# yzGuu830/efficient-speech-codec

Measured on AMD Instinct MI355X. Metric: audio-seconds/sec encode+decode, ESC-Base 9kbps 3s@16kHz, higher is better.
Workload: dtype f32 (fp32 storage and accumulation everywhere; the K = C contractions of the MLPs, of the attention's Q / K / V projections, of PatchMerge / PatchSplit and of the de-embedding run on the fp16 matrix cores with every fp32 operand split into two fp16 terms under power-of-two scales (range-safe by cons

## Files before the change

efficient-speech-codec_amd/csrc/escx_api.cpp:

```cpp
#include <hip/hip_runtime.h>

#include <algorithm>
#include <cmath>
#include <cstdlib>
#include <cstring>
#include <map>
#include <mutex>
#include <tuple>
#include <utility>
#include <vector>

#include "escx_internal.h"
#include "launchers.h"

using namespace escx;

static void part_layout(escx_handle_s* h, int B, int T, int* k, int* per, int* pass) {
    *k = std::min(n_parts(h, B), h->n_sets);
    *pass = std::max(1, std::min(pass_clips(h, B, T), h->sets[0].shp.B));
    *per = *k <= 1 ? B : (B + *k - 1) / *k;
}

template <class F>
static int run_halves(escx_handle_s* h, int B, int T, hipStream_t st, F part) {
// ... 311 lines not shown
        L.sub_x3 = nullptr; L.sub_x3s = nullptr;
        if (!want || !grab(&L.sub_x3_buf, rowgemm_x3_bytes(KP, Np))) continue;
        if (rowgemm_x3_pack(L.sub_wf, L.sub_x3_buf, KP, Np, st, nt, L.sub_g, L.sub_b, (L.scale == 1 ? 2 : 1) * L.C) == 0) L.sub_x3 = L.sub_x3_buf;
        if (L.scale == 2 && (L.Cp == 80 || L.Cp == 96 || L.Cp == 144) && L.Cp <= x3_max && grab(&L.sub_x3s_buf, mlp_x3_split_bytes(L.Cp, Np)) &&
            mlp_x3_split_pack(L.sub_wf, L.sub_x3s_buf, L.Cp, Np, st, nt, L.sub_g, L.sub_b, L.C) == 0) L.sub_x3s = L.sub_x3s_buf;
    }
    h->pvq_tab_stale = false;
    return launch_ok("derived images");
}

extern "C" int escx_set_precision(escx_handle h, int mode) {
    if (!h) ESCX_FAIL(ESCX_ERR_INVALID_ARG, "null handle");
    if (mode != ESCX_PRECISION_FP32 && mode != ESCX_PRECISION_BF16X3 && mode != ESCX_PRECISION_F16X2)
        ESCX_FAIL(ESCX_ERR_INVALID_ARG, "precision mode %d (0 = fp32 MFMA, 3 = three bf16 terms, 2 = two fp16 terms)", mode);
    if (mode != h->prec) { h->prec = mode; h->pvq_tab_stale = true; }
    return ESCX_OK;
}
extern "C" int escx_get_precision(escx_handle h) { return h ? h->prec : ESCX_ERR_INVALID_ARG; }

static float pvq_loss_scale(const escx_handle_s* h, const Quant& q, int Tq) {
    if (h->len) return 1.0f / ((float)q.d * h->cfg.group_size);
    return 1.0f / ((float)Tq * q.d * h->cfg.group_size);
}

static int run_pvq_encode(escx_handle_s* h, const Quant& q, const float* enc, const float* dec, int B, int W, long long* codes,
                          long long bstride, float* loss, hipStream_t st) {
    const escx_config& c = h->cfg;
    const int Tq = W / c.overlap, M = B * Tq;
    const int splits = pvq_down_splits(M, q.Kq, q.Cp);
    if ((size_t)splits * M * q.Nz > h->zpart_cap) ESCX_FAIL(ESCX_ERR_STATE, "split-K scratch too small");
    const double vec = (double)c.overlap * q.Hq * q.C;
    PROF("pvq_down_gemm", 2.0 * M * vec * q.d, (double)M * vec * (dec ? 2 : 1) * 4,
         gemm_pvq_down(enc, dec, B, q.Hq, W, q.Cp, c.overlap, q.wd, q.Nz, q.Kq, h->zpart, splits, st));
    int src_rc = 0;
    PROF("pvq_search", 2.0 * M * c.group_size * c.codebook_size * q.d, ((double)c.group_size * c.codebook_size * q.d + (double)M * c.group_size * q.d) * 4,
         src_rc = pvq_search(h->zpart, splits, M, q.Nz, q.cbn, q.c2, q.cbraw, c.group_size, c.codebook_size, q.d, q.dt, Tq, codes, bstride,
                             loss, pvq_loss_scale(h, q, Tq), c.l2norm, st));
    if (src_rc) ESCX_FAIL(ESCX_ERR_UNSUPPORTED, "codebook_dim %d unsupported by the search kernel", q.d);
    return launch_ok("pvq_encode");
}

static int run_pvq_decode(escx_handle_s* h, const Quant& q, const long long* codes, long long bstride, const float* dec, int B, int W,
                          float* out, hipStream_t st) {
    const escx_config& c = h->cfg;
    const double vec = (double)c.overlap * q.Hq * q.C, Mv = (double)B * (W / c.overlap);
    const bool special = h->pvq_up_kernel;
    if (q.tab && special) {
        PROF("pvq_tab_add", 0, Mv * vec * (dec ? 3 : 2) * 4,
             pvq_tab_add(codes, bstride, q.tab, q.gq, c.group_size, c.codebook_size, B, q.Hq, W, q.Cp, c.overlap, dec, out, st));
        return launch_ok("pvq_decode");
    }
    int urc = -1;
    if (special)
        PROF("pvq_up_gemm", 2.0 * Mv * vec * q.d, Mv * vec * (dec ? 2 : 1) * 4,
             urc = pvq_up(codes, bstride, q.cbraw, c.group_size, c.codebook_size, q.dt, B, q.Hq, W, q.Cp, c.overlap, q.wup, q.Kq, q.Kup, dec, out, st));
    if (urc != 0) {
        if (special && h->prof && !h->prof_recs.empty()) h->prof_recs.pop_back();
    PROF("pvq_up_gemm", 2.0 * Mv * vec * q.d, Mv * vec * (dec ? 2 : 1) * 4,
         gemm_pvq_up(codes, bstride, q.cbraw, c.group_size, c.codebook_size, q.dt, B, q.Hq, W, q.Cp, c.overlap, q.wup, q.Kq, q.Kup, dec, out, st));
    }
    return launch_ok("pvq_decode");
}

static int run_pvq_quantize(escx_handle_s* h, const Quant& q, const float* enc, const float* dec, int B, int W, long long* codes, long long bstride,
                            float* loss, float* out, hipStream_t st) {
    const escx_config& c = h->cfg;
    if (h->pvq_fused) {
        const int Tq = W / c.overlap, M = B * Tq;
        const double vec = (double)c.overlap * q.Hq * q.C;
        int frc = -1;
        PROF(out ? "pvq_fused" : "pvq_fused_codes", 2.0 * M * vec * q.d * (out ? 2 : 1) + 2.0 * M * c.group_size * c.codebook_size * q.d,
             (double)M * vec * ((dec ? 2 : 1) + (out ? (dec ? 2 : 1) : 0)) * 4,
             frc = pvq_fused(enc, dec, B, q.Hq, W, q.Cp, c.overlap, q.wdf, q.Nz, q.Kq, pvq_down_splits(M, q.Kq, q.Cp), pvq_down_bk(q.Cp), q.cbn, q.c2, q.cbraw,
                             c.group_size, c.codebook_size, q.d, q.dt, q.wup, q.tab, q.gq, out, codes, bstride, loss, pvq_loss_scale(h, q, Tq), c.l2norm, st));
        if (frc == 0) return launch_ok("pvq_quantize");
        if (h->prof && !h->prof_recs.empty()) h->prof_recs.pop_back();
    }
    int rc;
    if ((rc = run_pvq_encode(h, q, enc, dec, B, W, codes, bstride, loss, st))) return rc;
    if (out && (rc = run_pvq_decode(h, q, codes, bstride, dec, B, W, out, st))) return rc;
    return 0;
}

static int run_deembed(escx_handle_s* h, const float* tok, int B, int W, float* rspec, hipStream_t st) {
    const escx_config& c = h->cfg;
    const int H0 = c.in_freq / c.patch_f;
    if (h->len) {
        if (h->deembed_two_stage || c.in_dim * h->Q > 16) ESCX_FAIL(ESCX_ERR_UNSUPPORTED, "mixed-length batches run the composed de-embedding only (in_dim * patch area <= 16, ESCX_DEEMBED_TWO_STAGE unset)");
        const double tk = (double)B * H0 * W;
        PROF("deembed_zero_dead", 0, tk * h->C0p * 4, zero_dead_cols(const_cast<float*>(tok), h->len->d_W, B, H0, W, h->C0p, st));
        int hrc = -1;
        if (h->deembed_halo)
            PROF("deembed_composed7x7", 2.0 * tk * 49 * h->C0 * c.in_dim * h->Q, (tk * h->C0 + tk * c.in_dim * h->Q) * 4,
                 hrc = deembed7_fused(tok, B, H0, W, h->C0p, h->dch_w, h->dcc_b, rspec, c.patch_f, c.patch_t, c.in_dim, h->Fp, st, h->dch_x2));
        if (hrc != 0)
        PROF("deembed_composed7x7", 2.0 * tk * 49 * h->C0 * c.in_dim * h->Q, (tk * h->C0 + tk * c.in_dim * h->Q) * 4,
             gemm_deembed_composed(tok, B, H0, W, h->C0p, h->dcc_w, rspec, h->dcc_b, c.patch_f, c.patch_t, c.in_dim, h->Fp, st));
        int brc = 0;
        PROF("deembed_border_len", 0, 0,
             brc = deembed_border_len(tok, h->dcv_w, h->dcv_b, rspec, h->len->d_W, B, H0, W, h->C0, h->C0p, c.patch_f, c.patch_t, c.in_dim, h->Fp, st));
        if (brc != 0) ESCX_FAIL(ESCX_ERR_UNSUPPORTED, "mixed-length batches: no border kernel for %d de-embedding outputs", c.in_dim * h->Q);
        return launch_ok("patch_deembed");
    }
    if (!h->deembed_two_stage && c.in_dim * h->Q <= 16) {
        const double tk = (double)B * H0 * W;
        int hrc = -1;
        if (h->deembed_halo)
            PROF("deembed_composed7x7", 2.0 * tk * 49 * h->C0 * c.in_dim * h->Q, (tk * h->C0 + tk * c.in_dim * h->Q) * 4,
                 hrc = deembed7_fused(tok, B, H0, W, h->C0p, h->dch_w, h->dcc_b, rspec, c.patch_f, c.patch_t, c.in_dim, h->Fp, st, h->dch_x2));
        if (hrc != 0)
        PROF("deembed_composed7x7", 2.0 * tk * 49 * h->C0 * c.in_dim * h->Q, (tk * h->C0 + tk * c.in_dim * h->Q) * 4,
             gemm_deembed_composed(tok, B, H0, W, h->C0p, h->dcc_w, rspec, h->dcc_b, c.patch_f, c.patch_t, c.in_dim, h->Fp, st));
        int brc = 0;
        PROF("deembed_border", 0, 0,
             brc = deembed_border(tok, h->dcv_w, h->dcv_b, rspec, B, H0, W, h->C0, h->C0p, c.patch_f, c.patch_t, c.in_dim, h->Fp, st));
        if (brc == 0) return launch_ok("patch_deembed");
    }
    const double toks = (double)B * H0 * W, pix = toks * h->Q;
    PROF("deembed_conv5x5", 2.0 * toks * 25 * h->C0 * h->C0 * h->Q, (toks * h->C0 + pix * h->C0) * 4,
         gemm_conv_deembed1(tok, B, H0, W, h->C0p, h->dc1_w, h->Q * h->C0p, h->deemb, h->dc1_b, c.patch_f, c.patch_t, st));
    PROF("deembed_conv3x3", 2.0 * pix * 9 * h->C0 * c.in_dim, (pix * h->C0 + pix * c.in_dim) * 4,
         gemm_conv_spec(h->deemb, B, c.patch_t * W, c.patch_f * H0, h->C0p, h->dc2_w, rspec, h->dc2_b, h->Fp, c.in_dim, st));
    return launch_ok("patch_deembed");
}

static int run_istft(escx_handle_s* h, const float* rspec, int B, int T2, float* wave, hipStream_t st) {
    const escx_config& c = h->cfg;
    PROF("istft_idft_gemm", 2.0 * B * T2 * c.win_length * 2 * h->F, (double)B * T2 * (2 * h->F + c.win_length) * 4,
         gemm_store(rspec, c.in_dim * h->Fp, B * T2, h->idft_w, h->winP, c.in_dim * h->Fp, h->frames, h->winP, nullptr, st));
    if (h->len) {
        PROF("istft_overlap_add_len", 0, (double)B * T2 * c.win_length * 4 + (double)B * c.hop_length * (T2 - 1) * 4,
             istft_ola_len(h->frames, h->win2, wave, h->len->d_W, c.patch_t, B, T2, h->winP, c.win_length, c.hop_length, h->left, h->n_fft / 2, c.hop_length * (T2 - 1), st));
        return launch_ok("istft");
    }
    PROF("istft_overlap_add", 0, (double)B * T2 * c.win_length * 4 + (double)B * c.hop_length * (T2 - 1) * 4,
         istft_ola(h->frames, h->win2, wave, B, T2, h->winP, c.win_length, c.hop_length, h->left, h->n_fft / 2, c.hop_length * (T2 - 1), st));
    return launch_ok("istft");
}

static void spec_unpad(escx_handle_s* h, const float* src, float* dst, long long rows, hipStream_t st) {
    unpad_rows(src, dst, rows * h->cfg.in_dim, h->F, h->Fp, st);
}
static void spec_pad(escx_handle_s* h, const float* src, float* dst, long long rows, hipStream_t st) {
    pad_rows(src, dst, rows * h->cfg.in_dim, h->F, h->Fp, st);
}

extern "C" int escx_num_frames(escx_handle h, int n_samples) { return h ? 1 + n_samples / h->cfg.hop_length : 0; }
extern "C" int escx_output_samples(escx_handle h, int feat_w) { return h ? h->cfg.hop_length * (h->cfg.patch_t * feat_w - 1) : 0; }

static int rvq_encode(escx_handle_s* h, const float* wave, int B, int L, const int32_t* streams, int S, int64_t* codes, int* fh, int* fw, void* stream);
static int rvq_decode(escx_handle_s* h, const int64_t* codes, int B, int S, const int32_t* streams, int fh, int fw, float* wave_out, float* recon_feat, void* stream);
static int rvq_forward(escx_handle_s* h, const float* wave, const float* feat, int B, int LT, const int32_t* streams, int S, int64_t* codes, float* wave_out,
                       float* raw_feat, float* recon_feat, float* cm_loss, void* stream);

static int run_csvq_encode(escx_handle_s* h, const Shapes& s, int S, long long* codes, hipStream_t st) {
    const escx_config& c = h->cfg;
    const int n = h->n, G = c.group_size;
    const long long bstride = (long long)S * G * s.Tq, sstride = (long long)G * s.Tq;
    int rc, H = s.encH[n - 1], Hn;
    float* dec = h->decA; float* other = h->decB;
    if ((rc = run_pvq_quantize(h, h->quants[0], h->enc_hs[n - 1], nullptr, s.B, s.W, codes, bstride, nullptr, S == 1 ? nullptr : dec, st))) return rc;
    if (S == 1) return 0;
    for (int i = 0; i < S - 1; ++i) {
        const Quant& q = h->quants[i + 1];
        const bool last = (i + 2 == S);
        if ((rc = run_pvq_quantize(h, q, h->enc_hs[n - 1 - i], dec, s.B, s.W, codes + (i + 1) * sstride, bstride, nullptr, last ? nullptr : dec, st))) return rc;
        if (last) break;
        if ((rc = run_layer(h, h->layers[n + i], dec, other, s.B, H, s.W, &Hn, st))) return rc;
        std::swap(dec, other); H = Hn;
    }
    return 0;
}

extern "C" int escx_encode(escx_handle h, const float* wave, int B, int L, int S, int64_t* codes, int* fh, int* fw, void* stream) {
    if (h && h->kind == 1) return rvq_encode(h, wave, B, L, nullptr, S, codes, fh, fw, stream);
    int rc = check_ready(h); if (rc) return rc;
    if (!wave || !codes) ESCX_FAIL(ESCX_ERR_INVALID_ARG, "null pointer");
    if (S < 1 || S > h->cfg.max_streams) ESCX_FAIL(ESCX_ERR_INVALID_ARG, "num_streams=%d outside [1, %d]", S, h->cfg.max_streams);
    if (L <= h->n_fft / 2) ESCX_FAIL(ESCX_ERR_INVALID_ARG, "n_samples=%d too short for reflect padding of %d", L, h->n_fft / 2);
    Shapes s; if ((rc = ensure_ws(h, B, frames_of(h, L), &s))) return rc;
    const long long cstride = (long long)S * h->cfg.group_size * s.Tq;
    if ((rc = ensure_pvq_tables(h, (hipStream_t)stream))) return rc;
    rc = run_halves(h, B, s.T, (hipStream_t)stream, [&](int b0, int nb, hipStream_t st) -> int {
        Shapes sp = s; sp.B = nb; int r;
        if ((r = run_stft(h, wave + (size_t)b0 * L, nb, L, sp.T, h->spec, st))) return r;
        if ((r = run_encoder(h, sp, st))) return r;
        return run_csvq_encode(h, sp, S, (long long*)codes + b0 * cstride, st);
    });
    if (rc) return rc;
    if (fh) *fh = s.encH[h->n - 1];
    if (fw) *fw = s.W;
    return ESCX_OK;
}

static int run_csvq_decode(escx_handle_s* h, const long long* codes, int B, int S, int Hb, int W, float* rspec, hipStream_t st) {
    const escx_config& c = h->cfg;
    const int n = h->n, G = c.group_size, Tq = W / c.overlap;
    const long long bstride = (long long)S * G * Tq, sstride = (long long)G * Tq;
    int rc, H = Hb, Hn;
    float* dec = h->decA; float* other = h->decB;
    if ((rc = run_pvq_decode(h, h->quants[0], codes, bstride, nullptr, B, W, dec, st))) return rc;
    for (int i = 0; i + 1 < n; ++i) {
        if (i < S - 1 && (rc = run_pvq_decode(h, h->quants[i + 1], codes + (i + 1) * sstride, bstride, dec, B, W, dec, st))) return rc;
        if ((rc = run_layer(h, h->layers[n + i], dec, other, B, H, W, &Hn, st))) return rc;
        std::swap(dec, other); H = Hn;
    }
    if ((rc = run_layer(h, h->layers[2 * n - 1], dec, other, B, H, W, &Hn, st))) return rc;
    return run_deembed(h, other, B, W, rspec, st);
}

extern "C" int escx_decode(escx_handle h, const int64_t* codes, int B, int S, int fh, int fw, float* wave_out, float* recon_feat,
                           void* stream) {
    if (h && h->kind == 1) return rvq_decode(h, codes, B, S, nullptr, fh, fw, wave_out, recon_feat, stream);
    int rc = check_infer_ready(h); if (rc) return rc;
    if (!codes || !wave_out) ESCX_FAIL(ESCX_ERR_INVALID_ARG, "null pointer");
    const escx_config& c = h->cfg;
    if (S < 1 || S > c.max_streams) ESCX_FAIL(ESCX_ERR_INVALID_ARG, "codes.size(1)=%d outside [1, %d]", S, c.max_streams);
    if (fw < 1 || fw % c.overlap) ESCX_FAIL(ESCX_ERR_ASSERT, "Time dimension must be multiple of overlap");
    Shapes s; if ((rc = ensure_ws(h, B, frames_for_width(h, fw), &s))) return rc;
    if (s.W != fw || s.encH[h->n - 1] != fh) ESCX_FAIL(ESCX_ERR_INVALID_ARG, "feat_shape (%d,%d) does not match the model (%d,%d)", fh, fw, s.encH[h->n - 1], s.W);
    const int T2 = c.patch_t * fw, out_len = c.hop_length * (T2 - 1);
    const long long cstride = (long long)S * c.group_size * (fw / c.overlap);
    if ((rc = ensure_pvq_tables(h, (hipStream_t)stream))) return rc;
    rc = run_halves(h, B, s.T, (hipStream_t)stream, [&](int b0, int nb, hipStream_t st) -> int {
        int r;
        if ((r = run_csvq_decode(h, (const long long*)codes + b0 * cstride, nb, S, fh, fw, h->rspec, st))) return r;
        if ((r = run_istft(h, h->rspec, nb, T2, wave_out + (size_t)b0 * out_len, st))) return r;
        if (recon_feat) spec_unpad(h, h->rspec, recon_feat + (size_t)b0 * T2 * c.in_dim * h->F, (long long)nb * T2, st);
        return launch_ok("decode");
    });
    return rc;
}

static int forward_impl(escx_handle h, const float* wave, const float* feat, int B, int L, int T, int S, int64_t* codes, float* wave_out,
                        float* raw_feat, float* recon_feat, float* cm_loss, void* stream) {
    if (h && h->kind == 1) return rvq_forward(h, wave, feat, B, wave ? L : T, nullptr, S, codes, wave_out, raw_feat, recon_feat, cm_loss, stream);
    int rc = check_infer_ready(h); if (rc) return rc;
    if ((!wave && !feat) || !codes || !wave_out) ESCX_FAIL(ESCX_ERR_INVALID_ARG, "null pointer");
    const escx_config& c = h->cfg;
    if (S < 1 || S > c.max_streams) ESCX_FAIL(ESCX_ERR_INVALID_ARG, "num_streams=%d outside [1, %d]", S, c.max_streams);
    if (wave && L <= h->n_fft / 2) ESCX_FAIL(ESCX_ERR_INVALID_ARG, "n_samples=%d too short for reflect padding of %d", L, h->n_fft / 2);
    if (!wave && T < c.patch_t) ESCX_FAIL(ESCX_ERR_INVALID_ARG, "n_frames=%d shorter than one patch", T);
    if (wave) T = frames_of(h, L);
    Shapes s; if ((rc = ensure_ws(h, B, T, &s))) return rc;
    if (s.W % c.overlap) ESCX_FAIL(ESCX_ERR_ASSERT, "Time dimension must be multiple of overlap");
    const int n = h->n, G = c.group_size;
    const long long bstride = (long long)S * G * s.Tq, sstride = (long long)G * s.Tq;
    const int T2 = c.patch_t * s.W, out_len = c.hop_length * (T2 - 1);
    if ((rc = ensure_pvq_tables(h, (hipStream_t)stream))) return rc;
    return run_halves(h, B, s.T, (hipStream_t)stream, [&](int b0, int nb, hipStream_t st) -> int {
        Shapes sp = s; sp.B = nb; int r;
        long long* cd = (long long*)codes + b0 * bstride;
        if (wave) { if ((r = run_stft(h, wave + (size_t)b0 * L, nb, L, sp.T, h->spec, st))) return r; }
        else spec_pad(h, feat + (size_t)b0 * sp.T * c.in_dim * h->F, h->spec, (long long)nb * sp.T, st);
        if (raw_feat) spec_unpad(h, h->spec, raw_feat + (size_t)b0 * sp.T * c.in_dim * h->F, (long long)nb * sp.T, st);
        if ((r = run_encoder(h, sp, st))) return r;
        const size_t lslot = (size_t)G * nb * sp.Tq;
        float* loss = cm_loss ? h->loss_terms : nullptr;
        int n_slots = 1;
        int H = sp.encH[n - 1], Hn;
        float* dec = h->decA; float* other = h->decB;
        if ((r = run_pvq_quantize(h, h->quants[0], h->enc_hs[n - 1], nullptr, nb, sp.W, cd, bstride, loss, dec, st))) return r;
        for (int i = 0; i + 1 < n; ++i) {
            if (i < S - 1) {
                const Quant& q = h->quants[i + 1];
                if ((r = run_pvq_quantize(h, q, h->enc_hs[n - 1 - i], dec, nb, sp.W, cd + (i + 1) * sstride, bstride, loss ? loss + (size_t)(i + 1) * lslot : nullptr, dec, st))) return r;
                n_slots = i + 2;
            }
            if ((r = run_layer(h, h->layers[n + i], dec, other, nb, H, sp.W, &Hn, st))) return r;
            std::swap(dec, other); H = Hn;
        }
        if ((r = run_layer(h, h->layers[2 * n - 1], dec, other, nb, H, sp.W, &Hn, st))) return r;
        if ((r = run_deembed(h, other, nb, sp.W, h->rspec, st))) return r;
        if ((r = run_istft(h, h->rspec, nb, T2, wave_out + (size_t)b0 * out_len, st))) return r;
        if (recon_feat) spec_unpad(h, h->rspec, recon_feat + (size_t)b0 * T2 * c.in_dim * h->F, (long long)nb * T2, st);
        if (cm_loss) loss_reduce(loss, n_slots, G, nb * sp.Tq, sp.Tq, cm_loss + b0, st);
        return launch_ok("forward");
    });
}

extern "C" int escx_forward(escx_handle h, const float* wave, int B, int L, int S, int64_t* codes, float* wave_out, float* raw_feat,
                            float* recon_feat, float* cm_loss, void* stream) {
    if (!wave) ESCX_FAIL(ESCX_ERR_INVALID_ARG, "null pointer");
    return forward_impl(h, wave, nullptr, B, L, 0, S, codes, wave_out, raw_feat, recon_feat, cm_loss, stream);
}

extern "C" int escx_forward_feat(escx_handle h, const float* feat, int B, int T, int S, int64_t* codes, float* wave_out, float* recon_feat,
                                 float* cm_loss, void* stream) {
    if (!feat) ESCX_FAIL(ESCX_ERR_INVALID_ARG, "null pointer");
    return forward_impl(h, nullptr, feat, B, 0, T, S, codes, wave_out, nullptr, recon_feat, cm_loss, stream);
}

namespace {
struct MixPlan {
    int B = 0, Smax = 0;
    std::vector<int32_t> ints;
    const int32_t* S_ws() const { return ints.data() + 2 * B; }
};
}

static int check_streams(escx_handle_s* h, int B, const int32_t* streams, int* Smax) {
    if (!streams) ESCX_FAIL(ESCX_ERR_INVALID_ARG, "null streams pointer");
    if (B < 1) ESCX_FAIL(ESCX_ERR_INVALID_ARG, "batch=%d: the per-clip stream counts need at least one clip", B);
    int m = 0;
    for (int b = 0; b < B; ++b) {
        if (streams[b] < 1 || streams[b] > h->cfg.max_streams)
            ESCX_FAIL(ESCX_ERR_INVALID_ARG, "streams[%d]=%d outside [1, %d]", b, streams[b], h->cfg.max_streams);
        m = std::max(m, (int)streams[b]);
    }
    *Smax = m;
    return 0;
}

static void plan_streams(escx_handle_s* h, int B, int T, const int32_t* streams, int Smax, MixPlan* p) {
    int k, per, pass;
    part_layout(h, B, T, &k, &per, &pass);
    std::vector<std::pair<int, int>> groups;
    for (int off = 0; off < per; off += pass)
        for (int i = 0; i < std::max(k, 1); ++i) {
            const int b0 = i * per, nb = std::min(per, B - b0);
            if (nb <= off) continue;
            groups.push_back({b0 + off, std::min(pass, nb - off)});
        }
    std::vector<int> order(B);
    for (int b = 0; b < B; ++b) order[b] = b;
    std::stable_sort(order.begin(), order.end(), [&](int a, int b) { return streams[a] > streams[b]; });
    p->B = B; p->Smax = Smax;
    p->ints.assign((size_t)4 * B, 0);
    int32_t *ws2b = p->ints.data(), *b2ws = ws2b + B, *Sws = ws2b + 2 * B, *Sb = ws2b + 3 * B;
    int next = 0;
    for (int r = 0; next < B; ++r)
        for (const auto& g : groups)
            if (r < g.second && next < B) ws2b[g.first + r] = order[next++];
    for (int w = 0; w < B; ++w) { b2ws[ws2b[w]] = w; Sws[w] = streams[ws2b[w]]; }
    for (int b = 0; b < B; ++b) Sb[b] = streams[b];
}

namespace {
struct MixBufs {
    size_t used = 0;
    std::vector<std::pair<void**, size_t>> want;
    template <class T> void add(T** p, size_t n) { want.push_back({reinterpret_cast<void**>(p), n * sizeof(T)}); }
};
}
static int mix_alloc(escx_handle_s* h, MixBufs& m) {
    size_t total = 0;
    for (auto& w : m.want) total += (w.second + 255) / 256 * 256;
    if (total > h->mix_cap) {
        ESCX_HIP(hipDeviceSynchronize());
        if (h->mix_buf) { (void)hipFree(h->mix_buf); h->mix_buf = nullptr; h->mix_cap = 0; }
        ESCX_HIP(hipMalloc(&h->mix_buf, total));
        h->mix_cap = total;
    }
    char* base = static_cast<char*>(h->mix_buf);
    for (auto& w : m.want) { *w.first = w.second ? base : nullptr; base += (w.second + 255) / 256 * 256; }
    return 0;
}

static int upload_plan(escx_handle_s* h, const MixPlan& p, int32_t* dev, hipStream_t st) {
    ESCX_HIP(hipMemcpyAsync(dev, p.ints.data(), p.ints.size() * sizeof(int32_t), hipMemcpyHostToDevice, st));
    return 0;
}

static int clips_over(const int* S, int B, int j) { int c = 0; while (c < B && S[c] > j) ++c; return c; }

static int run_csvq_encode_streams(escx_handle_s* h, const Shapes& s, const int* S, long long* codes, long long bstride, hipStream_t st) {
    const int n = h->n;
    const long long sstride = (long long)h->cfg.group_size * s.Tq;
    int rc, H = s.encH[n - 1], Hn;
    float* dec = h->decA; float* other = h->decB;
    int nref = clips_over(S, s.B, 1);
    if ((rc = run_pvq_quantize(h, h->quants[0], h->enc_hs[n - 1], nullptr, s.B, s.W, codes, bstride, nullptr, nref ? dec : nullptr, st))) return rc;
    for (int i = 0; nref > 0; ++i) {
        const int nq = nref;
        nref = clips_over(S, nq, i + 2);
        if ((rc = run_pvq_quantize(h, h->quants[i + 1], h->enc_hs[n - 1 - i], dec, nq, s.W, codes + (i + 1) * sstride, bstride, nullptr, nref ? dec : nullptr, st))) return rc;
        if (!nref) break;
        if ((rc = run_layer(h, h->layers[n + i], dec, other, nref, H, s.W, &Hn, st))) return rc;
        std::swap(dec, other); H = Hn;
    }
    return 0;
}

static int run_csvq_decode_streams(escx_handle_s* h, const long long* codes, long long bstride, int B, const int* S, int Hb, int W, float* rspec, hipStream_t st) {
    const int n = h->n;
    const long long sstride = (long long)h->cfg.group_size * (W / h->cfg.overlap);
    int rc, H = Hb, Hn;
    float* dec = h->decA; float* other = h->decB;
    if ((rc = run_pvq_decode(h, h->quants[0], codes, bstride, nullptr, B, W, dec, st))) return rc;
    for (int i = 0; i + 1 < n; ++i) {
        const int nq = clips_over(S, B, i + 1);
        if (nq && (rc = run_pvq_decode(h, h->quants[i + 1], codes + (i + 1) * sstride, bstride, dec, nq, W, dec, st))) return rc;
        if ((rc = run_layer(h, h->layers[n + i], dec, other, B, H, W, &Hn, st))) return rc;
        std::swap(dec, other); H = Hn;
    }
    if ((rc = run_layer(h, h->layers[2 * n - 1], dec, other, B, H, W, &Hn, st))) return rc;
    return run_deembed(h, other, B, W, rspec, st);
}

extern "C" int escx_encode_streams(escx_handle h, const float* wave, int B, int L, const int32_t* streams, int64_t* codes, int* fh, int* fw,
                                   void* stream) {
    if (h && h->kind == 1) return rvq_encode(h, wave, B, L, streams, 0, codes, fh, fw, stream);
    int rc = check_ready(h); if (rc) return rc;
    if (!wave || !codes) ESCX_FAIL(ESCX_ERR_INVALID_ARG, "null pointer");
    int Smax = 0; if ((rc = check_streams(h, B, streams, &Smax))) return rc;
    if (L <= h->n_fft / 2) ESCX_FAIL(ESCX_ERR_INVALID_ARG, "n_samples=%d too short for reflect padding of %d", L, h->n_fft / 2);
    Shapes s; if ((rc = ensure_ws(h, B, frames_of(h, L), &s))) return rc;
    MixPlan p; plan_streams(h, B, s.T, streams, Smax, &p);
    const int GT = h->cfg.group_size * s.Tq;
    const long long cstride = (long long)Smax * GT;
    int32_t* maps; float* wave_ws; long long* codes_ws;
    MixBufs mb; mb.add(&maps, p.ints.size()); mb.add(&wave_ws, (size_t)B * L); mb.add(&codes_ws, (size_t)B * cstride);
    if ((rc = mix_alloc(h, mb))) return rc;
    hipStream_t st = (hipStream_t)stream;
    if ((rc = ensure_pvq_tables(h, st))) return rc;
    if ((rc = upload_plan(h, p, maps, st))) return rc;
    PROF("mix_gather", 0, 2.0 * B * L * 4, rows_permute(wave, wave_ws, maps, B, L, st));
    rc = run_halves(h, B, s.T, st, [&](int b0, int nb, hipStream_t sti) -> int {
        Shapes sp = s; sp.B = nb; int r;
        if ((r = run_stft(h, wave_ws + (size_t)b0 * L, nb, L, sp.T, h->spec, sti))) return r;
        if ((r = run_encoder(h, sp, sti))) return r;
        return run_csvq_encode_streams(h, sp, p.S_ws() + b0, codes_ws + b0 * cstride, cstride, sti);
    });
    if (rc) return rc;
    PROF("mix_scatter", 0, 2.0 * B * cstride * 8, codes_permute(codes_ws, cstride, (long long*)codes, maps + B, maps + 3 * B, B, Smax, GT, st));
    if ((rc = launch_ok("encode_streams"))) return rc;
    if (fh) *fh = s.encH[h->n - 1];
    if (fw) *fw = s.W;
    return ESCX_OK;
}

extern "C" int escx_decode_streams(escx_handle h, const int64_t* codes, int B, int Smax_in, const int32_t* streams, int fh, int fw, float* wave_out,
                                   float* recon_feat, void* stream) {
    if (h && h->kind == 1) return rvq_decode(h, codes, B, Smax_in, streams, fh, fw, wave_out, recon_feat, stream);
    int rc = check_infer_ready(h); if (rc) return rc;
    if (!codes || !wave_out) ESCX_FAIL(ESCX_ERR_INVALID_ARG, "null pointer");
    const escx_config& c = h->cfg;
    int Smax = 0; if ((rc = check_streams(h, B, streams, &Smax))) return rc;
    if (Smax_in < Smax || Smax_in > c.max_streams) ESCX_FAIL(ESCX_ERR_INVALID_ARG, "codes.size(1)=%d: must lie in [max(streams)=%d, %d]", Smax_in, Smax, c.max_streams);
    if (fw < 1 || fw % c.overlap) ESCX_FAIL(ESCX_ERR_ASSERT, "Time dimension must be multiple of overlap");
    Shapes s; if ((rc = ensure_ws(h, B, frames_for_width(h, fw), &s))) return rc;
    if (s.W != fw || s.encH[h->n - 1] != fh) ESCX_FAIL(ESCX_ERR_INVALID_ARG, "feat_shape (%d,%d) does not match the model (%d,%d)", fh, fw, s.encH[h->n - 1], s.W);
    MixPlan p; plan_streams(h, B, s.T, streams, Smax, &p);
    const int T2 = c.patch_t * fw, out_len = c.hop_length * (T2 - 1), GT = c.group_size * (fw / c.overlap);
    const long long in_stride = (long long)Smax_in * GT, cstride = (long long)Smax * GT, frow = (long long)T2 * c.in_dim * h->F;
    int32_t* maps; long long* codes_ws; float *wave_ws, *recon_ws = nullptr;
    MixBufs mb; mb.add(&maps, p.ints.size()); mb.add(&codes_ws, (size_t)B * cstride); mb.add(&wave_ws, (size_t)B * out_len);
    if (recon_feat) mb.add(&recon_ws, (size_t)B * frow);
    if ((rc = mix_alloc(h, mb))) return rc;
    hipStream_t st = (hipStream_t)stream;
    if ((rc = ensure_pvq_tables(h, st))) return rc;
    if ((rc = upload_plan(h, p, maps, st))) return rc;
    PROF("mix_gather", 0, 2.0 * B * cstride * 8, codes_permute((const long long*)codes, in_stride, codes_ws, maps, maps + 2 * B, B, Smax, GT, st));
    rc = run_halves(h, B, s.T, st, [&](int b0, int nb, hipStream_t sti) -> int {
        int r;
        if ((r = run_csvq_decode_streams(h, codes_ws + b0 * cstride, cstride, nb, p.S_ws() + b0, fh, fw, h->rspec, sti))) return r;
        if ((r = run_istft(h, h->rspec, nb, T2, wave_ws + (size_t)b0 * out_len, sti))) return r;
        if (recon_ws) spec_unpad(h, h->rspec, recon_ws + (size_t)b0 * frow, (long long)nb * T2, sti);
        return launch_ok("decode_streams");
    });
    if (rc) return rc;
    PROF("mix_scatter", 0, 2.0 * B * out_len * 4, rows_permute(wave_ws, wave_out, maps + B, B, out_len, st));
    if (recon_feat) PROF("mix_scatter", 0, 2.0 * B * frow * 4, rows_permute(recon_ws, recon_feat, maps + B, B, frow, st));
    return launch_ok("decode_streams");
}

extern "C" int escx_forward_streams(escx_handle h, const float* wave, const float* feat, int B, int LT, const int32_t* streams, int64_t* codes,
                                    float* wave_out, float* raw_feat, float* recon_feat, float* cm_loss, void* stream) {
    if (h && h->kind == 1) return rvq_forward(h, wave, feat, B, LT, streams, 0, codes, wave_out, raw_feat, recon_feat, cm_loss, stream);
    int rc = check_infer_ready(h); if (rc) return rc;
    if ((!wave == !feat) || !codes || !wave_out) ESCX_FAIL(ESCX_ERR_INVALID_ARG, "null pointer (exactly one of wave / feat, codes and wave_out are required)");
    const escx_config& c = h->cfg;
    int Smax = 0; if ((rc = check_streams(h, B, streams, &Smax))) return rc;
    const int L = wave ? LT : 0;
    int T = wave ? 0 : LT;
    if (wave && L <= h->n_fft / 2) ESCX_FAIL(ESCX_ERR_INVALID_ARG, "n_samples=%d too short for reflect padding of %d", L, h->n_fft / 2);
    if (!wave && T < c.patch_t) ESCX_FAIL(ESCX_ERR_INVALID_ARG, "n_frames=%d shorter than one patch", T);
    if (wave) T = frames_of(h, L);
    Shapes s; if ((rc = ensure_ws(h, B, T, &s))) return rc;
    if (s.W % c.overlap) ESCX_FAIL(ESCX_ERR_ASSERT, "Time dimension must be multiple of overlap");
    MixPlan p; plan_streams(h, B, s.T, streams, Smax, &p);
    const int n = h->n, G = c.group_size, GT = G * s.Tq;
    const long long cstride = (long long)Smax * GT, sstride = GT;
    const int T2 = c.patch_t * s.W, out_len = c.hop_length * (T2 - 1);
    const long long in_row = wave ? (long long)L : (long long)s.T * c.in_dim * h->F, raw_row = (long long)s.T * c.in_dim * h->F, rec_row = (long long)T2 * c.in_dim * h->F;
    int32_t* maps; float *in_ws, *wave_ws, *raw_ws = nullptr, *recon_ws = nullptr, *loss_ws = nullptr; long long* codes_ws;
    MixBufs mb; mb.add(&maps, p.ints.size()); mb.add(&in_ws, (size_t)B * in_row); mb.add(&codes_ws, (size_t)B * cstride); mb.add(&wave_ws, (size_t)B * out_len);
    if (raw_feat) mb.add(&raw_ws, (size_t)B * raw_row);
    if (recon_feat) mb.add(&recon_ws, (size_t)B * rec_row);
    if (cm_loss) mb.add(&loss_ws, (size_t)B);
    if ((rc = mix_alloc(h, mb))) return rc;
    hipStream_t st = (hipStream_t)stream;
    if ((rc = ensure_pvq_tables(h, st))) return rc;
    if ((rc = upload_plan(h, p, maps, st))) return rc;
    PROF("mix_gather", 0, 2.0 * B * in_row * 4, rows_permute(wave ? wave : feat, in_ws, maps, B, in_row, st));
    const int32_t* Sdev = maps + 2 * B;
    rc = run_halves(h, B, s.T, st, [&](int b0, int nb, hipStream_t st) -> int {
        Shapes sp = s; sp.B = nb; int r;
        const int* S = p.S_ws() + b0;
        long long* cd = codes_ws + b0 * cstride;
        if (wave) { if ((r = run_stft(h, in_ws + (size_t)b0 * L, nb, L, sp.T, h->spec, st))) return r; }
        else spec_pad(h, in_ws + (size_t)b0 * in_row, h->spec, (long long)nb * sp.T, st);
        if (raw_ws) spec_unpad(h, h->spec, raw_ws + (size_t)b0 * raw_row, (long long)nb * sp.T, st);
        if ((r = run_encoder(h, sp, st))) return r;
        const size_t lslot = (size_t)G * nb * sp.Tq;
        float* loss = cm_loss ? h->loss_terms : nullptr;
        int slot_clips[8] = {nb};
        int H = sp.encH[n - 1], Hn;
        float* dec = h->decA; float* other = h->decB;
        if ((r = run_pvq_quantize(h, h->quants[0], h->enc_hs[n - 1], nullptr, nb, sp.W, cd, cstride, loss, dec, st))) return r;
        for (int i = 0; i + 1 < n; ++i) {
            const int nq = clips_over(S, nb, i + 1);
            if (nq) {
                if ((r = run_pvq_quantize(h, h->quants[i + 1], h->enc_hs[n - 1 - i], dec, nq, sp.W, cd + (i + 1) * sstride, cstride, loss ? loss + (size_t)(i + 1) * lslot : nullptr, dec, st))) return r;
                slot_clips[i + 1] = nq;
            }
            if ((r = run_layer(h, h->layers[n + i], dec, other, nb, H, sp.W, &Hn, st))) return r;
            std::swap(dec, other); H = Hn;
        }
        if ((r = run_layer(h, h->layers[2 * n - 1], dec, other, nb, H, sp.W, &Hn, st))) return r;
        if ((r = run_deembed(h, other, nb, sp.W, h->rspec, st))) return r;
        if ((r = run_istft(h, h->rspec, nb, T2, wave_ws + (size_t)b0 * out_len, st))) return r;
        if (recon_ws) spec_unpad(h, h->rspec, recon_ws + (size_t)b0 * rec_row, (long long)nb * T2, st);
        if (cm_loss) PROF("loss_reduce_streams", 0, (double)nb * Smax * GT * 4, loss_reduce_streams(loss, (long long)lslot, Sdev + b0, n, slot_clips, G, sp.Tq, nb, loss_ws + b0, st));
        return launch_ok("forward_streams");
    });
    if (rc) return rc;
    PROF("mix_scatter", 0, 2.0 * B * cstride * 8, codes_permute(codes_ws, cstride, (long long*)codes, maps + B, maps + 3 * B, B, Smax, GT, st));
    PROF("mix_scatter", 0, 2.0 * B * out_len * 4, rows_permute(wave_ws, wave_out, maps + B, B, out_len, st));
    if (raw_feat) PROF("mix_scatter", 0, 2.0 * B * raw_row * 4, rows_permute(raw_ws, raw_feat, maps + B, B, raw_row, st));
    if (recon_feat) PROF("mix_scatter", 0, 2.0 * B * rec_row * 4, rows_permute(recon_ws, recon_feat, maps + B, B, rec_row, st));
    if (cm_loss) PROF("mix_scatter", 0, 8.0 * B, rows_permute(loss_ws, cm_loss, maps + B, B, 1, st));
    return launch_ok("forward_streams");
}

namespace {
struct LenGuard {
    escx_handle_s* h;
    LenGuard(escx_handle_s* h_, const LenCtx* c) : h(h_) { h->len = c; }
    ~LenGuard() { h->len = nullptr; }
};
}

static int len_common_checks(escx_handle_s* h, int B, const int32_t* v, const char* what) {
    if (h->kind == 1) ESCX_FAIL(ESCX_ERR_UNSUPPORTED, "mixed-length batches are not implemented for the rvq+swinT codec (RVQCodecs)");
    if (h->ws != 4) ESCX_FAIL(ESCX_ERR_UNSUPPORTED, "mixed-length batches are implemented for window_size 4 only (this model: %d)", h->ws);
    if (!v) ESCX_FAIL(ESCX_ERR_INVALID_ARG, "null %s pointer", what);
    if (B < 1) ESCX_FAIL(ESCX_ERR_INVALID_ARG, "batch=%d: the per-clip %s need at least one clip", B, what);
    return 0;
}

static int plan_lengths(escx_handle_s* h, int B, int Lx, const int32_t* lengths, LenCtx* lc, int* Lmax) {
    const escx_config& c = h->cfg;
    lc->B = B; lc->W.assign(B, 0); lc->Wmax = 0; *Lmax = 0;
    for (int b = 0; b < B; ++b) {
        const int L = lengths[b];
        if (L <= h->n_fft / 2 || L > Lx) ESCX_FAIL(ESCX_ERR_INVALID_ARG, "lengths[%d]=%d outside (%d, %d] (reflect padding of %d, row length %d)", b, L, h->n_fft / 2, Lx, h->n_fft / 2, Lx);
        const int W = frames_of(h, L) / c.patch_t;
        if (W < 1 || W % c.overlap) ESCX_FAIL(ESCX_ERR_ASSERT, "Time dimension must be multiple of overlap (clip %d: %d samples give %d latent frames)", b, L, W);
        lc->W[b] = W; lc->Wmax = std::max(lc->Wmax, W); *Lmax = std::max(*Lmax, L);
    }
    return 0;
}

static int upload_lengths(escx_handle_s* h, MixBufs& mb, LenCtx* lc, const int32_t* lengths, hipStream_t st) {
    int32_t* tab = nullptr;
    mb.add(&tab, (size_t)2 * lc->B);
    int rc = mix_alloc(h, mb); if (rc) return rc;
    ESCX_HIP(hipMemcpyAsync(tab, lc->W.data(), (size_t)lc->B * sizeof(int32_t), hipMemcpyHostToDevice, st));
    lc->d_W = tab;
    if (lengths) { ESCX_HIP(hipMemcpyAsync(tab + lc->B, lengths, (size_t)lc->B * sizeof(int32_t), hipMemcpyHostToDevice, st)); lc->d_L = tab + lc->B; }
    return 0;
}

extern "C" int escx_encode_lengths(escx_handle h, const float* wave, int B, int Lx, const int32_t* lengths, int S, int64_t* codes, int* fh, int* fw, void* stream) {
    int rc = check_ready(h); if (rc) return rc;
    if ((rc = len_common_checks(h, B, lengths, "lengths"))) return rc;
    if (!wave || !codes) ESCX_FAIL(ESCX_ERR_INVALID_ARG, "null pointer");
    const escx_config& c = h->cfg;
    if (S < 1 || S > c.max_streams) ESCX_FAIL(ESCX_ERR_INVALID_ARG, "num_streams=%d outside [1, %d]", S, c.max_streams);
    LenCtx lc; int Lmax = 0;
    if ((rc = plan_lengths(h, B, Lx, lengths, &lc, &Lmax))) return rc;
    Shapes s; if ((rc = ensure_ws(h, B, frames_of(h, Lmax), &s, B))) return rc;
    if (h->sets[0].shp.B < B || h->sets[0].shp.T < s.T) ESCX_FAIL(ESCX_ERR_STATE, "workspace set holds %d clips of %d frames, the batch needs %d of %d", h->sets[0].shp.B, h->sets[0].shp.T, B, s.T);
    hipStream_t st = (hipStream_t)stream;
    MixBufs mb; if ((rc = upload_lengths(h, mb, &lc, lengths, st))) return rc;
    if ((rc = ensure_pvq_tables(h, st))) return rc;
    use_set(h, 0);
    LenGuard guard(h, &lc);
    if ((rc = run_stft(h, wave, B, Lx, s.T, h->spec, st))) return rc;
    if ((rc = run_encoder(h, s, st))) return rc;
    if ((rc = run_csvq_encode(h, s, S, (long long*)codes, st))) return rc;
    PROF("codes_mask_len", 0, 8.0 * B * S * c.group_size * s.Tq, codes_mask_len((const long long*)codes, (long long*)codes, lc.d_W, c.overlap, B, S * c.group_size, s.Tq, -1, st));
    if ((rc = launch_ok("encode_lengths"))) return rc;
    if (fh) *fh = s.encH[h->n - 1];
    if (fw) *fw = s.W;
    return ESCX_OK;
}

static int plan_widths(escx_handle_s* h, int B, int fw, const int32_t* widths, LenCtx* lc) {
    lc->B = B; lc->W.assign(widths, widths + B); lc->Wmax = fw;
    for (int b = 0; b < B; ++b) {
        if (widths[b] < 1 || widths[b] > fw) ESCX_FAIL(ESCX_ERR_INVALID_ARG, "frame_lengths[%d]=%d outside [1, %d]", b, widths[b], fw);
        if (widths[b] % h->cfg.overlap) ESCX_FAIL(ESCX_ERR_ASSERT, "Time dimension must be multiple of overlap (clip %d: %d latent frames)", b, widths[b]);
    }
    return 0;
}

extern "C" int escx_decode_lengths(escx_handle h, const int64_t* codes, int B, int S, const int32_t* widths, int fh, int fw, float* wave_out, float* recon_feat,
                                   void* stream) {
    int rc = check_infer_ready(h); if (rc) return rc;
    if ((rc = len_common_checks(h, B, widths, "frame_lengths"))) return rc;
    if (!codes || !wave_out) ESCX_FAIL(ESCX_ERR_INVALID_ARG, "null pointer");
    const escx_config& c = h->cfg;
    if (S < 1 || S > c.max_streams) ESCX_FAIL(ESCX_ERR_INVALID_ARG, "codes.size(1)=%d outside [1, %d]", S, c.max_streams);
    if (fw < 1 || fw % c.overlap) ESCX_FAIL(ESCX_ERR_ASSERT, "Time dimension must be multiple of overlap");
    LenCtx lc;
    if ((rc = plan_widths(h, B, fw, widths, &lc))) return rc;
    Shapes s; if ((rc = ensure_ws(h, B, frames_for_width(h, fw), &s, B))) return rc;
    if (h->sets[0].shp.B < B || h->sets[0].shp.T < s.T) ESCX_FAIL(ESCX_ERR_STATE, "workspace set holds %d clips of %d frames, the batch needs %d of %d", h->sets[0].shp.B, h->sets[0].shp.T, B, s.T);
    if (s.W != fw || s.encH[h->n - 1] != fh) ESCX_FAIL(ESCX_ERR_INVALID_ARG, "feat_shape (%d,%d) does not match the model (%d,%d)", fh, fw, s.encH[h->n - 1], s.W);
    const int T2 = c.patch_t * fw, Tq = fw / c.overlap;
    hipStream_t st = (hipStream_t)stream;
    long long* codes_ws = nullptr;
    MixBufs mb; mb.add(&codes_ws, (size_t)B * S * c.group_size * Tq);
    if ((rc = upload_lengths(h, mb, &lc, nullptr, st))) return rc;
    if ((rc = ensure_pvq_tables(h, st))) return rc;
    use_set(h, 0);
    LenGuard guard(h, &lc);
    PROF("codes_mask_len", 0, 16.0 * B * S * c.group_size * Tq, codes_mask_len((const long long*)codes, codes_ws, lc.d_W, c.overlap, B, S * c.group_size, Tq, 0, st));
    if ((rc = run_csvq_decode(h, codes_ws, B, S, fh, fw, h->rspec, st))) return rc;
    if ((rc = run_istft(h, h->rspec, B, T2, wave_out, st))) return rc;
    if (recon_feat) PROF("unpad_len", 0, 2.0 * B * T2 * c.in_dim * h->F * 4, unpad_rows_len(h->rspec, recon_feat, lc.d_W, 1, c.patch_t, c.hop_length, B, T2, c.in_dim, h->F, h->Fp, st));
    return launch_ok("decode_lengths");
}

extern "C" int escx_forward_lengths(escx_handle h, const float* wave, int B, int Lx, const int32_t* lengths, int S, int64_t* codes, float* wave_out,
                                    float* raw_feat, float* recon_feat, float* cm_loss, void* stream) {
    int rc = check_infer_ready(h); if (rc) return rc;
    if ((rc = len_common_checks(h, B, lengths, "lengths"))) return rc;
    if (!wave || !codes || !wave_out) ESCX_FAIL(ESCX_ERR_INVALID_ARG, "null pointer");
    const escx_config& c = h->cfg;
    if (S < 1 || S > c.max_streams) ESCX_FAIL(ESCX_ERR_INVALID_ARG, "num_streams=%d outside [1, %d]", S, c.max_streams);
    LenCtx lc; int Lmax = 0;
    if ((rc = plan_lengths(h, B, Lx, lengths, &lc, &Lmax))) return rc;
    Shapes s; if ((rc = ensure_ws(h, B, frames_of(h, Lmax), &s, B))) return rc;
    if (h->sets[0].shp.B < B || h->sets[0].shp.T < s.T) ESCX_FAIL(ESCX_ERR_STATE, "workspace set holds %d clips of %d frames, the batch needs %d of %d", h->sets[0].shp.B, h->sets[0].shp.T, B, s.T);
    hipStream_t st = (hipStream_t)stream;
    MixBufs mb; if ((rc = upload_lengths(h, mb, &lc, lengths, st))) return rc;
    if ((rc = ensure_pvq_tables(h, st))) return rc;
    use_set(h, 0);
    LenGuard guard(h, &lc);
    const int n = h->n, G = c.group_size;
    const long long bstride = (long long)S * G * s.Tq, sstride = (long long)G * s.Tq;
    const int T2 = c.patch_t * s.W;
    long long* cd = (long long*)codes;
    if ((rc = run_stft(h, wave, B, Lx, s.T, h->spec, st))) return rc;
    if (raw_feat) PROF("unpad_len", 0, 2.0 * B * s.T * c.in_dim * h->F * 4, unpad_rows_len(h->spec, raw_feat, lc.d_L, 0, c.patch_t, c.hop_length, B, s.T, c.in_dim, h->F, h->Fp, st));
    if ((rc = run_encoder(h, s, st))) return rc;
    const size_t lslot = (size_t)G * B * s.Tq;
    float* loss = cm_loss ? h->loss_terms : nullptr;
    int n_slots = 1;
    int H = s.encH[n - 1], Hn;
    float* dec = h->decA; float* other = h->decB;
    if ((rc = run_pvq_quantize(h, h->quants[0], h->enc_hs[n - 1], nullptr, B, s.W, cd, bstride, loss, dec, st))) return rc;
    for (int i = 0; i + 1 < n; ++i) {
        if (i < S - 1) {
            if ((rc = run_pvq_quantize(h, h->quants[i + 1], h->enc_hs[n - 1 - i], dec, B, s.W, cd + (i + 1) * sstride, bstride, loss ? loss + (size_t)(i + 1) * lslot : nullptr, dec, st))) return rc;
            n_slots = i + 2;
        }
        if ((rc = run_layer(h, h->layers[n + i], dec, other, B, H, s.W, &Hn, st))) return rc;
        std::swap(dec, other); H = Hn;
    }
    if ((rc = run_layer(h, h->layers[2 * n - 1], dec, other, B, H, s.W, &Hn, st))) return rc;
    if ((rc = run_deembed(h, other, B, s.W, h->rspec, st))) return rc;
    if ((rc = run_istft(h, h->rspec, B, T2, wave_out, st))) return rc;
    if (recon_feat) PROF("unpad_len", 0, 2.0 * B * T2 * c.in_dim * h->F * 4, unpad_rows_len(h->rspec, recon_feat, lc.d_W, 1, c.patch_t, c.hop_length, B, T2, c.in_dim, h->F, h->Fp, st));
    if (cm_loss) PROF("loss_reduce_len", 0, (double)n_slots * lslot * 4, loss_reduce_len(loss, lc.d_W, c.overlap, n_slots, G, B, s.Tq, cm_loss, st));
    PROF("codes_mask_len", 0, 8.0 * B * bstride, codes_mask_len(cd, cd, lc.d_W, c.overlap, B, S * G, s.Tq, -1, st));
    return launch_ok("forward_lengths");
}

static int run_prvq(escx_handle_s* h, const float* enc, const long long* codes_in, int B, int W, long long* codes, long long bstride, const int* clip_S,
                    int S, float* loss, long long lslot, float* out, hipStream_t st) {
    const escx_config& c = h->cfg;
    const Quant& q = h->quants[0];
    const int Tq = W / c.overlap, M = B * Tq;
    const double vec = (double)c.overlap * q.Hq * q.C, G = c.group_size;
    int rc = -1;
    PROF(codes_in ? "prvq_decode" : (out ? "prvq_fused" : "prvq_fused_codes"),
         codes_in ? 2.0 * M * vec * q.d : 2.0 * M * vec * q.d * (out ? 2 : 1) + 2.0 * M * S * G * c.codebook_size * q.d,
         (double)M * vec * ((codes_in ? 0 : 1) + (out ? 1 : 0)) * 4,
         rc = prvq_fused(enc, codes_in, B, q.Hq, W, q.Cp, c.overlap, q.wdf, q.Nz, q.Kq, pvq_down_splits(M, q.Kq, q.Cp), pvq_down_bk(q.Cp), q.cbn, q.c2, q.cbraw,
                         c.group_size, c.codebook_size, q.d, q.dt, q.wup, codes, bstride, clip_S, S, S, loss, lslot, 1.0f / ((float)Tq * q.d * c.group_size),
                         c.l2norm, out, st));
    if (rc) ESCX_FAIL(ESCX_ERR_UNSUPPORTED, "rvq quantiser: geometry not covered (codebook_dim %d, %d groups)", q.d, c.group_size);
    return launch_ok("prvq");
}

static int run_plain_decoder(escx_handle_s* h, int B, int Hb, int W, float* rspec, hipStream_t st) {
    const int n = h->n;
    int rc, H = Hb, Hn;
    float* dec = h->decA; float* other = h->decB;
    for (int i = 0; i + 1 < n; ++i) {
        if ((rc = run_layer(h, h->layers[n + i], dec, other, B, H, W, &Hn, st))) return rc;
        std::swap(dec, other); H = Hn;
    }
    if ((rc = run_layer(h, h->layers[2 * n - 1], dec, other, B, H, W, &Hn, st))) return rc;
    return run_deembed(h, other, B, W, rspec, st);
}

static int rvq_counts(escx_handle_s* h, int B, const int32_t* streams, int S, int* Smax) {
    if (!streams) {
        if (S < 1 || S > h->num_rvqs) ESCX_FAIL(ESCX_ERR_INVALID_ARG, "num_streams=%d outside [1, %d] (num_rvqs)", S, h->num_rvqs);
        *Smax = S;
        return 0;
    }
    if (B < 1) ESCX_FAIL(ESCX_ERR_INVALID_ARG, "batch=%d: the per-clip stream counts need at least one clip", B);
    int m = 0;
    for (int b = 0; b < B; ++b) {
        if (streams[b] < 1 || streams[b] > h->num_rvqs) ESCX_FAIL(ESCX_ERR_INVALID_ARG, "streams[%d]=%d outside [1, %d] (num_rvqs)", b, streams[b], h->num_rvqs);
        m = std::max(m, (int)streams[b]);
    }
    *Smax = m;
    return 0;
}

static int rvq_upload(escx_handle_s* h, int B, const int32_t* streams, const int** dev, hipStream_t st) {
    *dev = nullptr;
    if (!streams) return 0;
    int32_t* d = nullptr;
    MixBufs mb; mb.add(&d, (size_t)B);
    int rc = mix_alloc(h, mb); if (rc) return rc;
    ESCX_HIP(hipMemcpyAsync(d, streams, (size_t)B * sizeof(int32_t), hipMemcpyHostToDevice, st));
    *dev = d;
    return 0;
}

static int rvq_encode(escx_handle_s* h, const float* wave, int B, int L, const int32_t* streams, int S, int64_t* codes, int* fh, int* fw, void* stream) {
    int rc = check_ready(h); if (rc) return rc;
    if (!wave || !codes) ESCX_FAIL(ESCX_ERR_INVALID_ARG, "null pointer");
    int Smax = 0; if ((rc = rvq_counts(h, B, streams, S, &Smax))) return rc;
    if (L <= h->n_fft / 2) ESCX_FAIL(ESCX_ERR_INVALID_ARG, "n_samples=%d too short for reflect padding of %d", L, h->n_fft / 2);
    Shapes s; if ((rc = ensure_ws(h, B, frames_of(h, L), &s))) return rc;
    hipStream_t st = (hipStream_t)stream;
    const int* Sdev; if ((rc = rvq_upload(h, B, streams, &Sdev, st))) return rc;
    if ((rc = ensure_pvq_tables(h, st))) return rc;
    const long long cstride = (long long)Smax * h->cfg.group_size * s.Tq;
    rc = run_halves(h, B, s.T, st, [&](int b0, int nb, hipStream_t sti) -> int {
        Shapes sp = s; sp.B = nb; int r;
        if ((r = run_stft(h, wave + (size_t)b0 * L, nb, L, sp.T, h->spec, sti))) return r;
// ... 66 lines not shown
    });
}

extern "C" int escx_spec_transform(escx_handle h, const float* wave, int B, int L, float* spec, void* stream) {
    int rc = check_ready(h); if (rc) return rc;
    if (!wave || !spec || B < 1) ESCX_FAIL(ESCX_ERR_INVALID_ARG, "bad argument");
    if (L <= h->n_fft / 2) ESCX_FAIL(ESCX_ERR_INVALID_ARG, "n_samples=%d too short for reflect padding of %d", L, h->n_fft / 2);
    const int T = frames_of(h, L);
    TmpBuf t; if (t.alloc((size_t)B * T * h->cfg.in_dim * h->Fp)) ESCX_FAIL(ESCX_ERR_HIP, "hipMalloc failed");
    hipStream_t st = (hipStream_t)stream;
    if ((rc = run_stft(h, wave, B, L, T, t.p, st))) return rc;
    spec_unpad(h, t.p, spec, (long long)B * T, st);
    return launch_ok("spec_transform");
}

extern "C" int escx_audio_reconstruct(escx_handle h, const float* spec, int B, int T, float* wave, void* stream) {
    int rc = check_ready(h); if (rc) return rc;
    if (!spec || !wave || B < 1 || T < 2) ESCX_FAIL(ESCX_ERR_INVALID_ARG, "bad argument (need at least 2 frames)");
    TmpBuf ts, tf;
    if (ts.alloc((size_t)B * T * h->cfg.in_dim * h->Fp) || tf.alloc((size_t)B * T * h->winP)) ESCX_FAIL(ESCX_ERR_HIP, "hipMalloc failed");
    hipStream_t st = (hipStream_t)stream;
    const escx_config& c = h->cfg;
    spec_pad(h, spec, ts.p, (long long)B * T, st);
    gemm_store(ts.p, c.in_dim * h->Fp, B * T, h->idft_w, h->winP, c.in_dim * h->Fp, tf.p, h->winP, nullptr, st);
    istft_ola(tf.p, h->win2, wave, B, T, h->winP, c.win_length, c.hop_length, h->left, h->n_fft / 2, c.hop_length * (T - 1), st);
    return launch_ok("audio_reconstruct");
}

extern "C" int escx_patch_embed(escx_handle h, const float* spec, int B, int T, float* tokens, void* stream) {
    int rc = check_ready(h); if (rc) return rc;
    const escx_config& c = h->cfg;
    const int W = T / c.patch_t, H0 = c.in_freq / c.patch_f;
    if (!spec || !tokens || B < 1 || W < 1) ESCX_FAIL(ESCX_ERR_INVALID_ARG, "bad argument");
    TmpBuf ts, tt;
    if (ts.alloc((size_t)B * T * c.in_dim * h->Fp) || tt.alloc((size_t)B * H0 * W * h->C0p)) ESCX_FAIL(ESCX_ERR_HIP, "hipMalloc failed");
    hipStream_t st = (hipStream_t)stream;
    spec_pad(h, spec, ts.p, (long long)B * T, st);
    if ((rc = run_patch_embed(h, ts.p, B, T, W, tt.p, st))) return rc;
    unpad_rows(tt.p, tokens, (long long)B * H0 * W, h->C0, h->C0p, st);
    return launch_ok("patch_embed");
}

static int stage_ws_for_w(escx_handle_s* h, int B, int W, Shapes* s) {
    int rc = ensure_ws(h, h->parts * B, frames_for_width(h, W), s, B);
    if (!rc) s->B = B;
    return rc;
}

extern "C" int escx_transformer_layer(escx_handle h, int layer_id, const float* x, int B, int H, int W, float* y, int* H_out, void* stream) {
    int rc = check_ready(h); if (rc) return rc;
    if (layer_id < 0 || layer_id >= 2 * h->n) ESCX_FAIL(ESCX_ERR_INVALID_ARG, "layer_id out of range");
    const Layer& L = h->layers[layer_id];
    Shapes s; if ((rc = stage_ws_for_w(h, B, W, &s))) return rc;
    if ((size_t)H > (size_t)2 * s.H0) ESCX_FAIL(ESCX_ERR_INVALID_ARG, "H too large for this model");
    hipStream_t st = (hipStream_t)stream;
    if ((rc = ensure_pvq_tables(h, st))) return rc;
    int Hn;
    const size_t need = (size_t)B * H * W * L.Cp, cap = std::max<size_t>((size_t)B * s.H0 * s.W * h->C0p, 1);
    size_t big = 0; for (int i = 0; i < h->n; ++i) big = std::max(big, (size_t)B * s.encH[i] * s.W * rup(h->cfg.h_dims[i], 16));
    if (need > std::max(cap, big)) ESCX_FAIL(ESCX_ERR_INVALID_ARG, "(H=%d, W=%d) is larger than any map of this layer", H, W);
    pad_rows(x, h->stageA, (long long)B * H * W, L.C, L.Cp, st);
    if ((rc = run_layer(h, L, h->stageA, h->stageB, B, H, W, &Hn, st))) return rc;
    unpad_rows(h->stageB, y, (long long)B * Hn * W, L.scale ? L.Cout : L.C, L.scale ? L.CoutP : L.Cp, st);
    if (H_out) *H_out = Hn;
    return launch_ok("transformer_layer");
}

extern "C" int escx_pvq_encode(escx_handle h, int sid, const float* enc, const float* dec, int B, int W, int64_t* codes, int64_t bstride,
                               void* stream) {
    int rc = check_ready(h); if (rc) return rc;
    if (h->kind != 0) ESCX_FAIL(ESCX_ERR_UNSUPPORTED, "escx_pvq_encode: the cross-scale quantisers do not exist on an rvq handle (escx_rvq_encode / escx_rvq_decode)");
    if (sid < 0 || sid >= h->cfg.max_streams) ESCX_FAIL(ESCX_ERR_INVALID_ARG, "stream_id out of range");
    if (W % h->cfg.overlap) ESCX_FAIL(ESCX_ERR_ASSERT, "Time dimension must be multiple of overlap");
    const Quant& q = h->quants[sid];
    Shapes s; if ((rc = stage_ws_for_w(h, B, W, &s))) return rc;
    hipStream_t st = (hipStream_t)stream;
    const long long rows = (long long)B * q.Hq * W;
    if ((rc = ensure_pvq_tables(h, st))) return rc;
    pad_rows(enc, h->stageA, rows, q.C, q.Cp, st);
    if (dec) pad_rows(dec, h->stageB, rows, q.C, q.Cp, st);
    return run_pvq_quantize(h, q, h->stageA, dec ? h->stageB : nullptr, B, W, (long long*)codes, bstride, nullptr, nullptr, st);
}

extern "C" int escx_pvq_decode(escx_handle h, int sid, const int64_t* codes, int64_t bstride, const float* dec, int B, int W, float* out,
                               void* stream) {
    int rc = check_ready(h); if (rc) return rc;
    if (h->kind != 0) ESCX_FAIL(ESCX_ERR_UNSUPPORTED, "escx_pvq_decode: the cross-scale quantisers do not exist on an rvq handle (escx_rvq_encode / escx_rvq_decode)");
    if (sid < 0 || sid >= h->cfg.max_streams) ESCX_FAIL(ESCX_ERR_INVALID_ARG, "stream_id out of range");
    if (W % h->cfg.overlap) ESCX_FAIL(ESCX_ERR_ASSERT, "Time dimension must be multiple of overlap");
    const Quant& q = h->quants[sid];
    Shapes s; if ((rc = stage_ws_for_w(h, B, W, &s))) return rc;
    hipStream_t st = (hipStream_t)stream;
    const long long rows = (long long)B * q.Hq * W;
    if ((rc = ensure_pvq_tables(h, st))) return rc;
    if (dec) pad_rows(dec, h->stageB, rows, q.C, q.Cp, st);
    if ((rc = run_pvq_decode(h, q, (const long long*)codes, bstride, dec ? h->stageB : nullptr, B, W, h->stageA, st))) return rc;
    unpad_rows(h->stageA, out, rows, q.C, q.Cp, st);
    return launch_ok("pvq_decode");
}

extern "C" int escx_rvq_encode(escx_handle h, const float* tokens, int B, int W, int S, int64_t* codes, float* zq_out, void* stream) {
    int rc = check_ready(h); if (rc) return rc;
    if (h->kind != 1) ESCX_FAIL(ESCX_ERR_UNSUPPORTED, "escx_rvq_encode needs an rvq handle (escx_create_rvq)");
    if (!tokens || !codes) ESCX_FAIL(ESCX_ERR_INVALID_ARG, "null pointer");
    if (B < 1 || W < 1) ESCX_FAIL(ESCX_ERR_INVALID_ARG, "batch and W must be positive");
    if (S < 1 || S > h->num_rvqs) ESCX_FAIL(ESCX_ERR_INVALID_ARG, "num_streams=%d outside [1, %d] (num_rvqs)", S, h->num_rvqs);
    if (W % h->cfg.overlap) ESCX_FAIL(ESCX_ERR_ASSERT, "Time dimension must be multiple of overlap");
    const Quant& q = h->quants[0];
    Shapes s; if ((rc = stage_ws_for_w(h, B, W, &s))) return rc;
    hipStream_t st = (hipStream_t)stream;
    const long long rows = (long long)B * q.Hq * W;
    pad_rows(tokens, h->stageA, rows, q.C, q.Cp, st);
    if ((rc = run_prvq(h, h->stageA, nullptr, B, W, (long long*)codes, (long long)S * h->cfg.group_size * (W / h->cfg.overlap), nullptr, S, nullptr, 0,
                       zq_out ? h->stageB : nullptr, st))) return rc;
    if (zq_out) unpad_rows(h->stageB, zq_out, rows, q.C, q.Cp, st);
    return launch_ok("rvq_encode");
}

extern "C" int escx_rvq_decode(escx_handle h, const int64_t* codes, int B, int S, int W, float* tokens_out, void* stream) {
    int rc = check_ready(h); if (rc) return rc;
    if (h->kind != 1) ESCX_FAIL(ESCX_ERR_UNSUPPORTED, "escx_rvq_decode needs an rvq handle (escx_create_rvq)");
    if (!codes || !tokens_out) ESCX_FAIL(ESCX_ERR_INVALID_ARG, "null pointer");
    if (B < 1 || W < 1) ESCX_FAIL(ESCX_ERR_INVALID_ARG, "batch and W must be positive");
    if (S < 1 || S > h->num_rvqs) ESCX_FAIL(ESCX_ERR_INVALID_ARG, "codes.size(1)=%d outside [1, %d] (num_rvqs)", S, h->num_rvqs);
    if (W % h->cfg.overlap) ESCX_FAIL(ESCX_ERR_ASSERT, "Time dimension must be multiple of overlap");
    const Quant& q = h->quants[0];
    Shapes s; if ((rc = stage_ws_for_w(h, B, W, &s))) return rc;
    hipStream_t st = (hipStream_t)stream;
    if ((rc = run_prvq(h, nullptr, (const long long*)codes, B, W, nullptr, (long long)S * h->cfg.group_size * (W / h->cfg.overlap), nullptr, S, nullptr, 0,
                       h->stageA, st))) return rc;
    unpad_rows(h->stageA, tokens_out, (long long)B * q.Hq * W, q.C, q.Cp, st);
    return launch_ok("rvq_decode");
}

extern "C" int escx_patch_deembed(escx_handle h, const float* tokens, int B, int W, float* spec, void* stream) {
    int rc = check_infer_ready(h); if (rc) return rc;
    Shapes s; if ((rc = stage_ws_for_w(h, B, W, &s))) return rc;
    hipStream_t st = (hipStream_t)stream;
    pad_rows(tokens, h->stageA, (long long)B * s.H0 * W, h->C0, h->C0p, st);
    if ((rc = run_deembed(h, h->stageA, B, W, h->rspec, st))) return rc;
    spec_unpad(h, h->rspec, spec, (long long)B * h->cfg.patch_t * W, st);
    return launch_ok("patch_deembed");
}

extern "C" int escx_debug_mlp_trace(unsigned long long* dev_buf) { mlp_set_trace(dev_buf); return 0; }
extern "C" int escx_test_fastdiv(int n, int d) { return test_fastdiv(n, d); }
extern "C" int escx_test_math(const float* x, float* y, int64_t n, int which, void* stream) {
    test_math(x, y, n, which, (hipStream_t)stream);
    return launch_ok("test_math");
}
extern "C" int escx_test_copy_rows(const float* src, float* dst, int64_t rows, int row_floats, void* stream) {
    if (!src || !dst || rows < 1 || row_floats < 4 || row_floats % 4) ESCX_FAIL(ESCX_ERR_INVALID_ARG, "bad argument");
    test_copy_rows(src, dst, rows, row_floats, (hipStream_t)stream);
    return launch_ok("test_copy_rows");
}
extern "C" int escx_codes_pack10(const int64_t* codes, uint8_t* out, int64_t n, void* stream) {
    if (!codes || !out || n < 0) ESCX_FAIL(ESCX_ERR_INVALID_ARG, "bad argument");
    codes_pack10((const long long*)codes, out, n, (hipStream_t)stream);
    return launch_ok("codes_pack10");
}
extern "C" int escx_codes_unpack10(const uint8_t* in, int64_t* codes, int64_t n, void* stream) {
    if (!codes || !in || n < 0) ESCX_FAIL(ESCX_ERR_INVALID_ARG, "bad argument");
    codes_unpack10(in, (long long*)codes, n, (hipStream_t)stream);
    return launch_ok("codes_unpack10");
}
static int ragged_offsets(int B, int Smax, int64_t gt, const int32_t* streams, hipStream_t st, const long long** off_dev, long long* n) {
// ... 38 lines not shown
```

efficient-speech-codec_amd/csrc/escx_internal.h:

```cpp
#pragma once
#include <hip/hip_runtime.h>
#include <cstdarg>
#include <cstdint>
#include <cstdio>
#include <map>
#include <string>
#include <tuple>
#include <vector>

#include "../../include/escx.h"

namespace escx {

inline int rup(int x, int m) { return (x + m - 1) / m * m; }

void set_error(const char* fmt, ...);

#define ESCX_FAIL(code, ...) do { ::escx::set_error(__VA_ARGS__); return (code); } while (0)
#define ESCX_HIP(expr) do { hipError_t _e = (expr); if (_e != hipSuccess) { \
        ::escx::set_error("%s failed: %s (%s:%d)", #expr, hipGetErrorString(_e), __FILE__, __LINE__); return ESCX_ERR_HIP; } } while (0)

struct Param { std::vector<float> data; std::vector<int64_t> shape; };

struct Arena {
// ... 25 lines not shown
    int scale;
    int Cout, CoutP;
    std::vector<BlockW> blocks;
    float *sub_g = nullptr, *sub_b = nullptr, *sub_w = nullptr;
    float *sub_wf = nullptr;
    void* sub_x3 = nullptr;
    void* sub_x3s = nullptr;
    void *sub_x3_buf = nullptr, *sub_x3s_buf = nullptr;
    float *sub_wT = nullptr;
};

struct Quant {
    std::string prefix;
    int C, Cp, Hq, d, dt, Nz, Kq, Kup;
    float *wd, *cbn, *c2, *cbraw, *wup;
    float *wdT = nullptr, *wupT = nullptr;
    float *wdf = nullptr, *gq = nullptr, *tab = nullptr;
    bool tab_ok = false;
    bool rvq = false;
    int stages = 1;
};

struct Shapes {
    int B = 0, L = 0, T = 0, W = 0, H0 = 0, Tq = 0;
    std::vector<int> encH;
};

struct WsFields {
    Arena ws;
    Shapes shp;
    float *spec = nullptr, *work = nullptr, *xn = nullptr, *qkv = nullptr, *obuf = nullptr, *hid = nullptr;
    float *decA = nullptr, *decB = nullptr, *zpart = nullptr, *deemb = nullptr, *rspec = nullptr, *frames = nullptr;
    float *stageA = nullptr, *stageB = nullptr, *loss = nullptr, *loss_terms = nullptr;
    long long* codes_tmp = nullptr;
    std::vector<float*> enc_hs;
    size_t zpart_cap = 0;
};

struct LenCtx {
    int B = 0, Wmax = 0;
    std::vector<int32_t> W;
    const int* d_W = nullptr;
    const int* d_L = nullptr;
};
struct LenMap { int* dev = nullptr; int n_windows = 0; };

}

struct escx_handle_s;
namespace escx {
int get_len_map(escx_handle_s* h, const LenCtx& lc, int H, int shift, LenMap* out);
int make_shapes(escx_handle_s* h, int B, int T, Shapes* out);
int check_infer_ready(escx_handle_s* h);
void free_train_state(escx_handle_s* h);
int get_map(escx_handle_s* h, int H, int W, int shift, const int** out);
int check_ready(escx_handle_s* h);
float* stream_scratch(hipStream_t st, int slot, size_t floats);
int launch_ok(const char* what);
int build_gather_map(escx_handle_s* h);
void use_set(escx_handle_s* h, int i);
int n_parts(escx_handle_s* h, int B);
int ensure_ws(escx_handle_s* h, int B, int T, Shapes* s, int min_set_clips = 0);
int pass_clips(escx_handle_s* h, int B, int T);
}

struct escx_handle_s : escx::WsFields {
    escx_config cfg;
    int kind = 0;
    int num_rvqs = 0;
    int device = 0;
    int n = 0;
    int F = 0, Fp = 0, n_fft = 0, left = 0, winP = 0, Kpe = 0, C0 = 0, C0p = 0, Q = 0;
    std::map<std::string, escx::Param> params;
    std::vector<std::string> required;
    bool finalized = false;
    bool use_fused = true;
    bool use_fused_attn = true;
    int prec = 2;
    int mlp_x3_max = 384, attn_x3_max = 384;
    bool rowgemm_x3 = true, pvq_table = true;
    int attn_gs_tokens = 600;
    bool mlp_split_fold = true;
    bool pvq_fused = true, pvq_up_kernel = true;
    bool prof_serial = false;
    int ws = 4;

    escx::Arena wts;
    std::vector<escx::Layer> layers;
    std::vector<escx::Quant> quants;
    float *pe_w = nullptr, *pe_b = nullptr, *pe_g = nullptr, *pe_beta = nullptr;
    float *dc1_w = nullptr, *dc1_b = nullptr, *dc2_w = nullptr, *dc2_b = nullptr;
    float *dft_w = nullptr, *idft_w = nullptr, *win2 = nullptr;
    float *dcc_w = nullptr, *dcc_b = nullptr, *dcv_w = nullptr, *dcv_b = nullptr;
    float* dch_w = nullptr;
    void* dch_x2 = nullptr;
    void* dch_x2_buf = nullptr;
    float *dc1_wT = nullptr, *idft_wT = nullptr;
    float* dft_wT = nullptr;
    double* dft_w64 = nullptr;

    std::vector<std::string> flat_keys;
    std::vector<size_t> flat_off, flat_numel;
    size_t flat_total = 0;
    int* gmap = nullptr;
    float* garena = nullptr;
    std::vector<std::pair<size_t, size_t>> grad_regions;
    long long* grad_seg = nullptr; int grad_nseg = 0; long long grad_seg_total = 0;
    escx::Arena tape;
    void* train_state = nullptr;
    bool train_x3_stale = true;
    bool pvq_tab_stale = true;
    long long* iota_codes = nullptr;
    bool composed_stale = false;
    bool deembed_halo = true;
    bool deembed_two_stage = false;

    static constexpr int MAX_PARTS = 4;
    escx::WsFields sets[MAX_PARTS];
    int n_sets = 1;
    int cap_clips = 0;
    int parts = 2;
    bool parts_forced = false;
    int chunk_frames = 10818;
    hipStream_t sx[MAX_PARTS] = {nullptr, nullptr, nullptr, nullptr};
    hipEvent_t ev_fork = nullptr, ev_join[MAX_PARTS] = {nullptr, nullptr, nullptr, nullptr};

    void* coll_buf = nullptr; size_t coll_cap = 0;
    void* mix_buf = nullptr; size_t mix_cap = 0;

    std::map<std::tuple<int, int, int>, int*> maps;
    const escx::LenCtx* len = nullptr;
    std::map<std::pair<std::vector<int32_t>, std::pair<int, int>>, escx::LenMap> len_maps;

    bool prof = false, prof_isolated = false;
    struct ProfRec { std::string name; double flops, bytes; hipEvent_t a, b; };
    std::vector<ProfRec> prof_recs;
    std::vector<hipEvent_t> prof_pool;
    std::string prof_json;
};

#include "launch_prof.h"
namespace escx {
hipEvent_t prof_event(escx_handle_s* h);
struct ProfScope {
    escx_handle_s* h; hipStream_t st; LaunchTimer lt; LaunchTimer* prev = nullptr; hipEvent_t m_start = nullptr;
    ProfScope(escx_handle_s* h_, hipStream_t s) : h(h_), st(s) {
        if (h->prof) { m_start = prof_event(h); (void)hipEventRecord(m_start, st); lt.start = prof_event(h); lt.stop = prof_event(h); prev = g_launch_timer; g_launch_timer = &lt; }
    }
    ~ProfScope() { if (lt.start && g_launch_timer == &lt) g_launch_timer = prev; }
    void end(const std::string& name, double flops, double bytes) {
        if (!lt.start) return;
        g_launch_timer = prev;
        if (lt.launches != 1) (void)hipEventRecord(lt.stop, st);
        const bool dispatch_timed = lt.launches >= 1;
        h->prof_recs.push_back({name, flops, bytes, dispatch_timed ? lt.start : m_start, lt.stop});
        h->prof_pool.push_back(dispatch_timed ? m_start : lt.start);
        lt.start = nullptr;
    }
};
}
#define PROF(name, flops, bytes, stmt) do { ::escx::ProfScope _ps(h, st); stmt; if (h->prof) _ps.end(name, flops, bytes); } while (0)
```

efficient-speech-codec_amd/csrc/escx_params.cpp:

```cpp
#include <hip/hip_runtime.h>

#include <algorithm>
#include <cmath>
#include <cstdlib>
#include <cstring>
#include <map>
#include <mutex>
#include <tuple>

#include "escx_internal.h"
#include "launchers.h"

using namespace escx;

namespace escx {
static thread_local std::string g_err;
void set_error(const char* fmt, ...) {
    char buf[1024];
    va_list ap; va_start(ap, fmt); vsnprintf(buf, sizeof(buf), fmt, ap); va_end(ap);
    g_err = buf;
}
}

extern "C" const char* escx_last_error(void) { return g_err.c_str(); }
// ... 51 lines not shown
    for (int j = 0; j + 1 < n; ++j)
        if ((rc = make_layer("decoder.blocks." + std::to_string(j) + ".", c.h_dims[n - 1 - j], c.swin_heads[n - 2 - j], 2,
                             c.h_dims[n - 2 - j]))) return rc;
    if ((rc = make_layer("decoder.post_nn.", c.h_dims[0], c.swin_heads[0], 0, c.h_dims[0]))) return rc;

    const int H0 = c.in_freq / c.patch_f;
    if (h->kind == 1) {
        Quant q; q.prefix = "quantizers."; q.rvq = true; q.stages = h->num_rvqs;
        q.C = c.h_dims[n - 1]; q.Cp = rup(q.C, 16);
        q.Hq = H0 >> (n - 1);
        if (q.Hq < 1) ESCX_FAIL(ESCX_ERR_UNSUPPORTED, "the bottleneck quantiser has in_freq 0");
        q.d = c.codebook_dims[0]; q.dt = roundup4(q.d);
        q.Nz = rup(c.group_size * q.dt, 16); q.Kup = q.Nz;
        q.Kq = c.overlap * q.Hq * q.Cp;
        const int D = c.overlap * q.Hq * q.C;
        for (int g = 0; g < c.group_size; ++g) {
            const int dg = g + 1 < c.group_size ? D / c.group_size : D - (D / c.group_size) * (c.group_size - 1);
            if (dg == q.d) ESCX_FAIL(ESCX_ERR_UNSUPPORTED, "rvq group %d has width %d == codebook_dim: the reference skips the projections there", g, dg);
            if (dg < 1) ESCX_FAIL(ESCX_ERR_UNSUPPORTED, "rvq group %d is empty", g);
        }
        if (!prvq_geometry_ok(q.Nz, q.dt, c.group_size, q.Kq, q.Cp, pvq_down_splits(0, q.Kq, q.Cp), pvq_down_bk(q.Cp)))
            ESCX_FAIL(ESCX_ERR_UNSUPPORTED, "rvq quantiser: codebook_dim %d with %d groups (bottleneck vector %d) is not covered by the fused kernel "
                                            "(fused_prvq.h: codebook_dim 5..8 with 3 or 4 groups, codebook_dim <= 4 with up to 4 groups)", q.d, c.group_size, D);
        h->quants.push_back(q);
    }
    for (int s = 0; s < c.max_streams && h->kind == 0; ++s) {
        Quant q; q.prefix = "quantizers." + std::to_string(s) + ".";
        q.C = c.h_dims[n - 1 - std::max(s - 1, 0)]; q.Cp = rup(q.C, 16);
        q.Hq = (s == 0) ? H0 >> (c.max_streams - 1) : H0 >> (c.max_streams - s);
        if (q.Hq < 1) ESCX_FAIL(ESCX_ERR_UNSUPPORTED, "quantizer %d has in_freq 0", s);
        q.d = c.codebook_dims[s]; q.dt = roundup4(q.d);
        if (q.d < 1 || q.dt > 64) ESCX_FAIL(ESCX_ERR_UNSUPPORTED, "codebook_dim %d unsupported", q.d);
        q.Nz = rup(c.group_size * q.dt, 16); q.Kup = q.Nz;
        q.Kq = c.overlap * q.Hq * q.Cp;
        h->quants.push_back(q);
    }

    auto& K = h->required;
    if (h->kind == 1)
        for (int g = 0; g < c.group_size; ++g) {
            const std::string p = "quantizers.vqs." + std::to_string(g) + ".";
            K.push_back(p + "proj_down.weight");
            K.push_back(p + "proj_up.weight");
            for (int i = 0; i < h->num_rvqs; ++i) K.push_back(p + "vqs." + std::to_string(i) + ".embedding.weight");
        }
    for (int s = 0; s < c.max_streams && h->kind == 0; ++s)
        for (int g = 0; g < c.group_size; ++g) {
            const std::string p = "quantizers." + std::to_string(s) + ".";
            K.push_back(p + "vqs." + std::to_string(g) + ".embedding.weight");
            K.push_back(p + "down_projs." + std::to_string(g) + ".weight");
            K.push_back(p + "up_projs." + std::to_string(g) + ".weight");
        }
    for (const char* k : {"proj.weight", "proj.bias", "norm.weight", "norm.bias"}) K.push_back(std::string("encoder.patch_embed.") + k);
    for (const Layer& L : h->layers) {
        for (int j = 0; j < c.swin_depth; ++j) add_block_keys(K, L.prefix + "swint_blocks." + std::to_string(j) + ".");
        if (L.scale) {
            K.push_back(L.prefix + "subsample.norm.weight"); K.push_back(L.prefix + "subsample.norm.bias");
            K.push_back(L.prefix + (L.scale == 1 ? "subsample.down.weight" : "subsample.up.weight"));
        }
    }
    for (const char* k : {"de_proj1.weight", "de_proj1.bias", "de_proj2.weight", "de_proj2.bias"})
        K.push_back(std::string("decoder.patch_deembed.") + k);
    return 0;
}

static int env_defaults(escx_handle_s* h) {
    auto flag = [](const char* name, bool dflt) { const char* e = getenv(name); return (e && e[0]) ? e[0] == '1' : dflt; };
    auto off = [](const char* name) { const char* e = getenv(name); return e && e[0] == '0'; };
    auto num = [](const char* name, int dflt) { const char* e = getenv(name); return (e && e[0]) ? atoi(e) : dflt; };
    h->use_fused = !flag("ESCX_NO_FUSED", false);
    h->use_fused_attn = !flag("ESCX_NO_FUSED_ATTN", false);
    h->deembed_two_stage = flag("ESCX_DEEMBED_TWO_STAGE", false);
    h->deembed_halo = !flag("ESCX_DEEMBED_GEMM", false);
    if (getenv("ESCX_STREAMS") && getenv("ESCX_STREAMS")[0]) { h->parts = std::min(std::max(num("ESCX_STREAMS", 2), 1), (int)escx_handle_s::MAX_PARTS); h->parts_forced = true; }
    h->chunk_frames = num("ESCX_CHUNK_FRAMES", h->chunk_frames);
    h->mlp_x3_max = num("ESCX_MLP_X3", h->mlp_x3_max);
    h->attn_x3_max = num("ESCX_ATTN_X3", h->attn_x3_max);
    h->rowgemm_x3 = !off("ESCX_ROWGEMM_X3");
    h->pvq_table = !off("ESCX_PVQ_TABLE");
    h->attn_gs_tokens = num("ESCX_ATTN_GS_TOKENS", h->attn_gs_tokens);
    h->mlp_split_fold = !off("ESCX_MLP_SPLIT_FOLD");
    h->pvq_fused = !off("ESCX_PVQ_FUSED");
    h->pvq_up_kernel = !off("ESCX_PVQ_UP_KERNEL");
    h->prof_serial = flag("ESCX_PROF_SERIAL", false);
    if (num("ESCX_X3_TERMS", 2) == 3) h->prec = 3;
    if (const char* e = getenv("ESCX_PRECISION")) {
        if (e[0]) {
            const std::string v(e);
            if (v == "fp32" || v == "0") h->prec = 0; else if (v == "bf16x3" || v == "3") h->prec = 3; else if (v == "f16x2" || v == "2") h->prec = 2;
            else ESCX_FAIL(ESCX_ERR_INVALID_ARG, "ESCX_PRECISION=%s (fp32 | bf16x3 | f16x2)", e);
        }
    }
    return 0;
}

static int create_impl(const escx_config* cfg, int kind, int num_rvqs, int device, escx_handle* out) {
    int ndev = 0;
    ESCX_HIP(hipGetDeviceCount(&ndev));
    if (device < 0 || device >= ndev) ESCX_FAIL(ESCX_ERR_INVALID_ARG, "device %d out of range (%d visible)", device, ndev);
    escx_handle_s* h = new escx_handle_s();
    h->cfg = *cfg; h->device = device;
    h->kind = kind; h->num_rvqs = num_rvqs;
    int erc = env_defaults(h);
    if (erc) { delete h; return erc; }
    int rc = build_geometry(h);
    if (rc) { delete h; return rc; }
    *out = h;
    return ESCX_OK;
}

extern "C" int escx_create(const escx_config* cfg, int device, escx_handle* out) {
    if (!cfg || !out) ESCX_FAIL(ESCX_ERR_INVALID_ARG, "null argument");
    return create_impl(cfg, 0, 0, device, out);
}

extern "C" int escx_create_rvq(const escx_rvq_config* cfg, int device, escx_handle* out) {
    if (!cfg || !out) ESCX_FAIL(ESCX_ERR_INVALID_ARG, "null argument");
    if (cfg->num_rvqs < 1 || cfg->num_rvqs > 16) ESCX_FAIL(ESCX_ERR_UNSUPPORTED, "num_rvqs=%d outside [1, 16]", cfg->num_rvqs);
    if (cfg->codebook_dim < 1 || cfg->codebook_dim > 64) ESCX_FAIL(ESCX_ERR_UNSUPPORTED, "codebook_dim=%d outside [1, 64]", cfg->codebook_dim);
    escx_config c = cfg->base;
    for (int i = 0; i < ESCX_MAX_SCALES; ++i) c.codebook_dims[i] = cfg->codebook_dim;
    return create_impl(&c, 1, cfg->num_rvqs, device, out);
}

extern "C" int escx_quantizer_kind(escx_handle h) { return h ? h->kind : ESCX_ERR_INVALID_ARG; }

extern "C" void escx_destroy(escx_handle h) {
    if (!h) return;
    (void)hipSetDevice(h->device);
    if (h->wts.base) (void)hipFree(h->wts.base);
    for (auto& S : h->sets) if (S.ws.base) (void)hipFree(S.ws.base);
    for (int i = 0; i < escx_handle_s::MAX_PARTS; ++i) {
        if (h->sx[i]) (void)hipStreamDestroy(h->sx[i]);
        if (h->ev_join[i]) (void)hipEventDestroy(h->ev_join[i]);
    }
    if (h->ev_fork) (void)hipEventDestroy(h->ev_fork);
    for (auto& kv : h->maps) (void)hipFree(kv.second);
    for (auto& kv : h->len_maps) (void)hipFree(kv.second.dev);
    if (h->coll_buf) (void)hipFree(h->coll_buf);
    if (h->mix_buf) (void)hipFree(h->mix_buf);
    for (Quant& q : h->quants) if (q.tab) (void)hipFree(q.tab);
    for (Layer& L : h->layers) { if (L.sub_x3_buf) (void)hipFree(L.sub_x3_buf); if (L.sub_x3s_buf) (void)hipFree(L.sub_x3s_buf); }
    if (h->dch_x2_buf) (void)hipFree(h->dch_x2_buf);
    for (Layer& L : h->layers) for (BlockW& bw : L.blocks) { if (bw.x3w_buf) (void)hipFree(bw.x3w_buf); if (bw.x3a_buf) (void)hipFree(bw.x3a_buf); if (bw.x3w_train) (void)hipFree(bw.x3w_train); }
    if (h->iota_codes) (void)hipFree(h->iota_codes);
    if (h->gmap) (void)hipFree(h->gmap);
    if (h->garena) (void)hipFree(h->garena);
    if (h->grad_seg) (void)hipFree(h->grad_seg);
    if (h->tape.base) (void)hipFree(h->tape.base);
    if (h->dft_w64) (void)hipFree(h->dft_w64);
    free_train_state(h);
    delete h;
}

extern "C" int escx_num_required_keys(escx_handle h) { return h ? (int)h->required.size() : 0; }
extern "C" const char* escx_required_key(escx_handle h, int i) {
    return (h && i >= 0 && i < (int)h->required.size()) ? h->required[i].c_str() : nullptr;
}

extern "C" int escx_set_param(escx_handle h, const char* key, const float* host, const int64_t* shape, int ndim) {
    if (!h || !key || !host || (ndim > 0 && !shape)) ESCX_FAIL(ESCX_ERR_INVALID_ARG, "null argument");
    Param p; size_t n = 1;
    for (int i = 0; i < ndim; ++i) { p.shape.push_back(shape[i]); n *= (size_t)shape[i]; }
    p.data.assign(host, host + n);
    h->params[key] = std::move(p);
    h->finalized = false;
// ... 729 lines not shown
```

efficient-speech-codec_amd/csrc/fused_pvq.h:

```cpp
#pragma once
#include <hip/hip_runtime.h>
#include "gemm_engine.h"
#include "kernels.h"

namespace escx {

struct PvqFusedArgs {
    const float* enc; const float* dec;
    const float* wd;
    const float* cbn; const float* c2; const float* cbraw;
    const float* wup;
    const float* tab; const float* gq;
    float* out;
    long long* codes; long long bstride;
    float* loss; float loss_scale;
    int M, Tq, Hq, Wd, Cp, ov, Kq, k_per_z, splits;
    int G, Ksz, d, l2norm;
    unsigned long long* trace;
};

constexpr int PVQF_WAVES = 16;
constexpr int PVQF_GMAX = 4;
template <int NT> constexpr int pvqf_lds_floats() { return PVQF_WAVES * 16 * (16 * NT + 4); }

// ... 6 lines not shown
    const int kbeg = wave * k_per_z, kend = min(Kq, kbeg + k_per_z);
    if (wave < splits && kbeg < kend) {
        const int nch = (kend - kbeg) >> 4;
        const float* wfrag = wd + (size_t)lane * 4;
        f32x4 er[PF], dr[PF], wr[PF][NT];
        auto issue = [&](int ci, f32x4& e, f32x4& dd, f32x4 (&wf)[NT]) {
            const int k0 = kbeg + 16 * min(ci, nch - 1);
            const int oh = k0 / Cp, cc = k0 - oh * Cp, o = oh / Hq, h = oh - o * Hq;
            const size_t idx = vecbase + (size_t)(h * Wd + o) * Cp + cc;
            e = ld4(enc + idx);
            if constexpr (DEC) dd = ld4(dec + idx);
#pragma unroll
            for (int n = 0; n < NT; ++n) wf[n] = ld4(wfrag + ((size_t)(k0 >> 4) * NT + n) * 256);
        };
        f32x4 acc[NT];
#pragma unroll
        for (int n = 0; n < NT; ++n) acc[n] = zero4();
        auto consume = [&](const f32x4& e, const f32x4& dd, const f32x4 (&wf)[NT]) {
            f32x4 af = e;
            if constexpr (DEC) af -= dd;
            if (!live) af = zero4();
#pragma unroll
            for (int r = 0; r < 4; ++r)
#pragma unroll
                for (int n = 0; n < NT; ++n) acc[n] = __builtin_amdgcn_mfma_f32_16x16x4f32(wf[n][r], af[r], acc[n], 0, 0, 0);
        };
#pragma unroll
        for (int j = 0; j < PF; ++j) issue(j, er[j], dr[j], wr[j]);
        const int rounds = nch / PF, tail = nch - rounds * PF;
        for (int rd = 0; rd < rounds; ++rd) {
#pragma unroll
            for (int j = 0; j < PF; ++j) {
                consume(er[j], dr[j], wr[j]);
                issue((rd + 1) * PF + j, er[j], dr[j], wr[j]);
            }
        }
#pragma unroll
        for (int j = 0; j < PF - 1; ++j)
            if (j < tail) consume(er[j], dr[j], wr[j]);
        float* pr = part + ((size_t)wave * 16 + (lane & 15)) * NPS + 4 * (lane >> 4);
#pragma unroll
        for (int n = 0; n < NT; ++n) st4(pr + 16 * n, acc[n]);
    }
}

template <int NT>
__device__ __forceinline__ void pvq_sum_slices(const float* part, int splits, int tid, float (&zs)[16][16 * NT + 1]) {
#pragma clang fp contract(off)
    constexpr int NP = 16 * NT, NPS = NP + 4;
    for (int e = tid; e < 16 * NP; e += 64 * PVQF_WAVES) {
        const int r = e / NP, n = e - r * NP;
        float z = 0.f;
#pragma unroll
        for (int s = 0; s < 16; ++s) z += (s < splits) ? part[((size_t)s * 16 + r) * NPS + n] : 0.f;
        zs[r][n] = z;
    }
}

template <int NT, int STEPS>
__device__ __forceinline__ void pvq_normalise(const float (&zs)[16][16 * NT + 1], int tid, int G, int d, int l2norm,
                                              float (&zn2)[PVQF_GMAX][16][4 * STEPS], float (&asum)[PVQF_GMAX][16]) {
#pragma clang fp contract(off)
    constexpr int DT = 4 * STEPS;
    if (tid < 16 * G) {
        const int g = tid >> 4, vi = tid & 15;
        float zr[DT];
#pragma unroll
        for (int j = 0; j < DT; ++j) zr[j] = zs[vi][g * DT + j];
        float ss = 0.f;
#pragma unroll
        for (int j = 0; j < DT; ++j) ss = (j < d) ? __builtin_fmaf(zr[j], zr[j], ss) : ss;
        const float den = l2norm ? fmaxf(sqrtf(ss), 1e-12f) : 1.0f;
        float s2 = 0.f;
#pragma unroll
        for (int j = 0; j < DT; ++j) {
            const float zn = (j < d) ? zr[j] / den : 0.f;
            s2 = __builtin_fmaf(zn, zn, s2);
            zn2[g][vi][j] = 2.0f * zn;
        }
        asum[g][vi] = s2;
    }
}

template <int STEPS>
__device__ __forceinline__ void pvq_search_group(const float* cb, const float* c2, int Ksz, int g, int wave, int l15, int lg,
                                                 const float (&zn2)[PVQF_GMAX][16][4 * STEPS], const float (&asum)[PVQF_GMAX][16],
                                                 float (&bestd)[PVQF_WAVES][PVQF_GMAX][16], int (&besti)[PVQF_WAVES][PVQF_GMAX][16]) {
#pragma clang fp contract(off)
    constexpr int TB = 4, DT = 4 * STEPS;
    const int per_wave = ((Ksz + PVQF_WAVES - 1) / PVQF_WAVES + 15) & ~15;
    const int cbeg = wave * per_wave, cend = min(Ksz, cbeg + per_wave);
    float zf[STEPS];
#pragma unroll
    for (int r = 0; r < STEPS; ++r) zf[r] = zn2[g][l15][STEPS * lg + r];
    const float av = asum[g][l15];
    float bd = __builtin_inff();
    int bi = 0x7fffffff;
    bool have = false;
    for (int cb0 = cbeg; cb0 < cend; cb0 += 16 * TB) {
        float cf[TB][STEPS], c2v[TB][4];
#pragma unroll
        for (int u = 0; u < TB; ++u) {
            const int c0 = cb0 + 16 * u;
            const float* p = cb + (size_t)min(c0 + l15, Ksz - 1) * DT + STEPS * lg;
#pragma unroll
            for (int r = 0; r < STEPS; ++r) cf[u][r] = p[r];
#pragma unroll
            for (int r = 0; r < 4; ++r) c2v[u][r] = c2[min(c0 + 4 * lg + r, Ksz - 1)];
        }
#pragma unroll
        for (int u = 0; u < TB; ++u) {
            const int c0 = cb0 + 16 * u;
            f32x4 dot = zero4();
#pragma unroll
            for (int r = 0; r < STEPS; ++r) dot = __builtin_amdgcn_mfma_f32_16x16x4f32(cf[u][r], zf[r], dot, 0, 0, 0);
#pragma unroll
            for (int r = 0; r < 4; ++r) {
                const int code = c0 + 4 * lg + r;
                const float dist = (av - dot[r]) + c2v[u][r];
                const bool in = code < cend;
                const bool take = in & (!have | (!(dist >= bd) & (bd == bd)));
                bd = take ? dist : bd; bi = take ? code : bi; have = have | in;
            }
        }
    }
#pragma unroll
    for (int o = 16; o <= 32; o <<= 1) {
        const float od = __shfl_xor(bd, o);
        const int oi = __shfl_xor(bi, o);
        const bool better = arg_better_sel(od, oi, bd, bi);
        bd = better ? od : bd; bi = better ? oi : bi;
    }
    if (lg == 0) { bestd[wave][g][l15] = bd; besti[wave][g][l15] = bi; }
}

__device__ __forceinline__ int pvq_combine_waves(const float (&bestd)[PVQF_WAVES][PVQF_GMAX][16], const int (&besti)[PVQF_WAVES][PVQF_GMAX][16], int g, int vi) {
#pragma clang fp contract(off)
    float wd_[PVQF_WAVES]; int wi_[PVQF_WAVES];
#pragma unroll
    for (int w = 0; w < PVQF_WAVES; ++w) { wd_[w] = bestd[w][g][vi]; wi_[w] = besti[w][g][vi]; }
    float d0 = wd_[0]; int i0 = wi_[0];
#pragma unroll
    for (int w = 1; w < PVQF_WAVES; ++w) {
        const bool better = arg_better_sel(wd_[w], wi_[w], d0, i0);
        d0 = better ? wd_[w] : d0; i0 = better ? wi_[w] : i0;
    }
    return i0;
}

template <int NT, bool DEC>
__device__ __forceinline__ void pvq_up_mfma(const f32x4 (&zf)[NT], const float* wup, const float* dec, float* out, size_t vecbase, bool live,
                                            int wave, int l15, int lg, int Kq, int Hq, int Wd, int Cp) {
#pragma clang fp contract(off)
    constexpr int NP = 16 * NT, KC = NT;
    constexpr int UNR = KC >= 6 ? 2 : (KC >= 4 ? 3 : (KC == 3 ? 4 : 6));
    const int NTo = Kq / 16;
    const float* wrow = wup + (size_t)l15 * NP + 4 * lg;
    for (int nt0 = wave * UNR; nt0 < NTo; nt0 += PVQF_WAVES * UNR) {
        f32x4 wf[UNR][KC], dv[UNR];
        size_t idx[UNR];
#pragma unroll
        for (int u = 0; u < UNR; ++u) {
            const int nt = min(nt0 + u, NTo - 1);
#pragma unroll
            for (int c = 0; c < KC; ++c) wf[u][c] = ld4(wrow + (size_t)(16 * nt) * NP + 16 * c);
            const int n0 = 16 * nt, oh = n0 / Cp, c0 = n0 - oh * Cp, o = oh / Hq, h = oh - o * Hq;
            idx[u] = vecbase + (size_t)(h * Wd + o) * Cp + c0;
            if constexpr (DEC) dv[u] = ld4(dec + idx[u]);
        }
#pragma unroll
        for (int u = 0; u < UNR; ++u) {
            f32x4 acc = zero4();
#pragma unroll
            for (int c = 0; c < KC; ++c)
#pragma unroll
                for (int r = 0; r < 4; ++r) acc = __builtin_amdgcn_mfma_f32_16x16x4f32(wf[u][c][r], zf[c][r], acc, 0, 0, 0);
            if constexpr (DEC) acc += dv[u];
            if (live && nt0 + u < NTo) st4(out + idx[u], acc);
        }
    }
}

template <int NT, int STEPS, bool DEC>
__global__ __launch_bounds__(64 * PVQF_WAVES) void pvq_fused_kernel(PvqFusedArgs a) {
#pragma clang fp contract(off)
    ESCX_SET_PRIO_SMALL();
    constexpr int NP = 16 * NT, DT = 4 * STEPS, KC = NT;
    extern __shared__ __attribute__((aligned(16))) float pvqf_part[];
    __shared__ float zs[16][NP + 1];
    __shared__ float zn2[PVQF_GMAX][16][DT];
    __shared__ float asum[PVQF_GMAX][16];
    __shared__ float bestd[PVQF_WAVES][PVQF_GMAX][16];
    __shared__ int besti[PVQF_WAVES][PVQF_GMAX][16];
    __shared__ int code_s[PVQF_GMAX][16];
    const int tid = threadIdx.x;
    const int lane = tid & 63, l15 = lane & 15, lg = lane >> 4;
    const int wave = __builtin_amdgcn_readfirstlane(tid >> 6);
    const int m0 = blockIdx.x * 16;
    const int m = m0 + l15;
    const bool live = m < a.M;
    const int b = live ? m / a.Tq : 0, t = live ? m - b * a.Tq : 0;
    const size_t vecbase = ((size_t)b * a.Hq * a.Wd + (size_t)a.ov * t) * a.Cp + 4 * lg;
#ifdef ESCX_PVQ_TRACE
#define PVQ_TS(i) if (a.trace && tid == 0) { __builtin_amdgcn_sched_barrier(0); a.trace[(size_t)blockIdx.x * 8 + (i)] = __builtin_amdgcn_s_memtime(); __builtin_amdgcn_sched_barrier(0); }
#else
#define PVQ_TS(i)
#endif
    PVQ_TS(0)

    pvq_down_slice<NT, DEC>(a.enc, a.dec, a.wd, vecbase, live, lane, wave, a.Kq, a.k_per_z, a.splits, a.Hq, a.Wd, a.Cp, pvqf_part);
    __syncthreads();
    PVQ_TS(1)
    pvq_sum_slices<NT>(pvqf_part, a.splits, tid, zs);
    __syncthreads();
    pvq_normalise<NT, STEPS>(zs, tid, a.G, a.d, a.l2norm, zn2, asum);
    __syncthreads();
    PVQ_TS(2)
    for (int g = 0; g < a.G; ++g)
        pvq_search_group<STEPS>(a.cbn + (size_t)g * a.Ksz * DT, a.c2 + (size_t)g * a.Ksz, a.Ksz, g, wave, l15, lg, zn2, asum, bestd, besti);
    __syncthreads();
    PVQ_TS(3)
    if (tid < 16 * a.G) {
        const int g = tid >> 4, vi = tid & 15;
        const int i0 = pvq_combine_waves(bestd, besti, g, vi);
        code_s[g][vi] = i0;
        const int mm = m0 + vi;
        if (mm < a.M) {
            const int bb = mm / a.Tq, tt = mm - bb * a.Tq;
            a.codes[(size_t)bb * a.bstride + (size_t)g * a.Tq + tt] = (long long)i0;
            if (a.loss) {
                const float* q = a.cbraw + ((size_t)g * a.Ksz + i0) * DT;
                float e = 0.f;
                for (int j = 0; j < a.d; ++j) { const float df = q[j] - zs[vi][g * DT + j]; e = __builtin_fmaf(df, df, e); }
                a.loss[(size_t)g * a.M + mm] = e * a.loss_scale;
            }
        }
    }
    if (!a.out) return;
    __syncthreads();
    PVQ_TS(4)

    if (a.tab) {
        constexpr int UNR = 8;
        const int NTo = a.Kq / 16;
        const int tabw = a.ov * a.Ksz;
        int cs[PVQF_GMAX];
#pragma unroll
        for (int g = 0; g < PVQF_GMAX; ++g) cs[g] = code_s[g < a.G ? g : 0][l15];
        for (int nt0 = wave * UNR; nt0 < NTo; nt0 += PVQF_WAVES * UNR) {
            f32x4 tv[UNR], dv[UNR];
            size_t idx[UNR];
            int gsel[UNR];
#pragma unroll
            for (int u = 0; u < UNR; ++u) {
                const int nt = min(nt0 + u, NTo - 1);
                const int n0 = 16 * nt, oh = n0 / a.Cp, c0 = n0 - oh * a.Cp, o = oh / a.Hq, h = oh - o * a.Hq;
                idx[u] = vecbase + (size_t)(h * a.Wd + o) * a.Cp + c0;
                gsel[u] = (int)a.gq[(n0 >> 2) + lg];
                const int gg = gsel[u] < 0 ? 0 : gsel[u];
                const int code = gg == 0 ? cs[0] : (gg == 1 ? cs[1] : (gg == 2 ? cs[2] : cs[3]));
                tv[u] = ld4(a.tab + ((size_t)h * tabw + (size_t)a.ov * code + o) * a.Cp + c0 + 4 * lg);
                if constexpr (DEC) dv[u] = ld4(a.dec + idx[u]);
            }
#pragma unroll
            for (int u = 0; u < UNR; ++u) {
                f32x4 v = gsel[u] >= 0 ? tv[u] : zero4();
                if constexpr (DEC) v += dv[u];
                if (live && nt0 + u < NTo) st4(a.out + idx[u], v);
            }
        }
        PVQ_TS(5)
        return;
    }
    f32x4 zf[KC];
#pragma unroll
    for (int c = 0; c < KC; ++c) {
        const int k = 16 * c + 4 * lg, g = k / DT;
        zf[c] = zero4();
        if (live && g < a.G) zf[c] = ld4(a.cbraw + ((size_t)g * a.Ksz + (size_t)code_s[g][l15]) * DT + (k - g * DT));
    }
    pvq_up_mfma<NT, DEC>(zf, a.wup, a.dec, a.out, vecbase, live, wave, l15, lg, a.Kq, a.Hq, a.Wd, a.Cp);
    PVQ_TS(5)
#undef PVQ_TS
}

struct PvqTabAddArgs {
    const long long* codes; long long bstride; const float* tab; const float* gq; const float* dec; float* out;
    int G, Ksz, Tq, Hq, Wd, Cp, ov; long long n4;
};
__global__ __launch_bounds__(256) void pvq_tab_add_kernel(PvqTabAddArgs a) {
    ESCX_SET_PRIO_SMALL();
    const long long i = (long long)blockIdx.x * 256 + threadIdx.x;
    if (i >= a.n4) return;
    const int c4 = a.Cp >> 2;
    const long long row = i / c4; const int c = (int)(i - row * c4) * 4;
    const int w = (int)(row % a.Wd); const long long bh = row / a.Wd; const int h = (int)(bh % a.Hq); const int b = (int)(bh / a.Hq);
    const int t = w / a.ov, o = w - t * a.ov;
    const int g = (int)a.gq[(((o * a.Hq + h) * a.Cp) + c) >> 2];
    f32x4 v = zero4();
    if (g >= 0) {
        long long code = a.codes[(size_t)b * a.bstride + (size_t)g * a.Tq + t];
        code = code < 0 ? 0 : (code >= a.Ksz ? a.Ksz - 1 : code);
        v = ld4(a.tab + ((size_t)h * a.ov * a.Ksz + (size_t)a.ov * code + o) * a.Cp + c);
    }
    if (a.dec) v += ld4(a.dec + i * 4);
    st4(a.out + i * 4, v);
}

}
```

efficient-speech-codec_amd/csrc/kernels_misc.hip:

```cpp
#include <algorithm>
#include <cstdint>

#include "kernels.h"
#include "fused_pvq.h"
#include "fused_prvq.h"
#include "train_prvq.h"
#include <atomic>
#include "launchers.h"

namespace escx {

static inline int grid_for(long long work_items, int per_block, int cap = 4096) {
    long long g = (work_items + per_block - 1) / per_block;
    if (g < 1) g = 1;
    if (g > cap) g = cap;
    return (int)g;
}

void ln_rows(int mode, const float* src, float* dst, const float* gamma, const float* beta, const int* map, int rows_per_clip,
             int src_rows_per_clip, int total_rows, int C, int Cp, hipStream_t s) {
    const int grid = grid_for(total_rows, 16, 8192);
    const float eps = 1e-5f;
    if (mode == 0)
        ESCX_LAUNCH((ln_rows_kernel<1, 0>), dim3(grid), dim3(256), 0, s, src, dst, gamma, beta, map, rows_per_clip,
// ... 1 lines not shown
    else if (mode == 1)
        ESCX_LAUNCH((ln_rows_kernel<1, 1>), dim3(grid), dim3(256), 0, s, src, dst, gamma, beta, map, rows_per_clip,
                           src_rows_per_clip, total_rows, C, Cp, eps);
    else
        ESCX_LAUNCH((ln_rows_kernel<2, 2>), dim3(grid), dim3(256), 0, s, src, dst, gamma, beta, map, rows_per_clip,
                           src_rows_per_clip, total_rows, C, Cp, eps);
}

int window_attention(const float* qkv, const float* bias, float* out, int total_windows, int nH, int hdp, int ldq, int ldo, int nWh,
                     int nWw, int shifted, hipStream_t s) {
    const long long pairs = (long long)total_windows * nH;
    const int grid = grid_for(pairs, 4, 16384);
#define ESCX_ATT(S) case S: ESCX_LAUNCH((window_attention_kernel<S>), dim3(grid), dim3(256), 0, s, qkv, bias, out, (int)pairs, \
                                               nH, ldq, ldo, nWh, nWw, shifted); return 0;
    switch (hdp / 4) {
        ESCX_ATT(1) ESCX_ATT(2) ESCX_ATT(3) ESCX_ATT(4) ESCX_ATT(5) ESCX_ATT(6) ESCX_ATT(7) ESCX_ATT(8)
        ESCX_ATT(12) ESCX_ATT(16)
        default: return -1;
    }
#undef ESCX_ATT
}

int window_attention_any(const float* qkv, const float* bias, float* out, int total_windows, int ws, int nH, int hd, int hdp, int ldq, int ldo, int nWh, int nWw,
                         int shift, hipStream_t s) {
    if (total_windows < 1 || nH < 1 || nH > 65535 || ws < 1) return -1;
    ESCX_LAUNCH(window_attention_any_kernel, dim3((unsigned)total_windows, (unsigned)nH), dim3(64), 0, s, qkv, bias, out, nH, hd, hdp, ldq, ldo, ws, nWh, nWw, shift);
    return 0;
}

int pvq_search(const float* zpart, int splits, int M, int ldz, const float* cbn, const float* c2, const float* cbraw, int G, int Ksz,
               int d, int dt, int Tq, long long* codes, long long bstride, float* loss, float loss_scale, int l2norm, hipStream_t s) {
    SearchArgs a{zpart, splits, M, ldz, cbn, c2, cbraw, Ksz, d, Tq, codes, bstride, loss, loss_scale, l2norm};
    dim3 grid((M + 15) / 16, G);
#define ESCX_SRCH(S) case S: ESCX_LAUNCH((pvq_search_kernel<S>), grid, dim3(256), 0, s, a); return 0;
    switch (dt / 4) {
        ESCX_SRCH(1) ESCX_SRCH(2) ESCX_SRCH(3) ESCX_SRCH(4) ESCX_SRCH(5) ESCX_SRCH(6) ESCX_SRCH(7) ESCX_SRCH(8)
        ESCX_SRCH(12) ESCX_SRCH(16)
        default: return -1;
    }
#undef ESCX_SRCH
}

void loss_reduce(const float* terms, int n_slots, int G, int M, int Tq, float* out, hipStream_t s) {
    ESCX_LAUNCH(loss_reduce_kernel, dim3(M / Tq), dim3(64), 0, s, terms, n_slots, G, M, Tq, out);
}

static bool pvq_slices(int Kq, int splits, int bk, int* k_per_z) {
    if (bk < 16 || bk % 16 || Kq % bk || splits < 1 || splits > PVQF_WAVES) return false;
    const int kIters = Kq / bk, per = (kIters + splits - 1) / splits;
    if ((kIters + per - 1) / per != splits) return false;
    *k_per_z = per * bk;
    return true;
}
static bool pvq_geometry(int Np, int dt, int G, int Kq, int Cp, int splits, int bk, int* k_per_z) {
    return !(Np % 16 || Kq % 16 || Cp % 16 || dt % 4 || G < 1 || G > PVQF_GMAX || G * dt > Np) && pvq_slices(Kq, splits, bk, k_per_z);
}

template <int NT, int STEPS, bool DEC>
static void launch_pvq_fused_d(const PvqFusedArgs& a, hipStream_t s) {
    auto kern = pvq_fused_kernel<NT, STEPS, DEC>;
    constexpr int lds = pvqf_lds_floats<NT>() * (int)sizeof(float);
    if constexpr (lds > 48 * 1024) {
        static std::atomic<unsigned> done{0};
        int dev = 0; (void)hipGetDevice(&dev);
        const unsigned bit = 1u << (dev & 31);
        if (!(done.load(std::memory_order_relaxed) & bit)) {
            (void)hipFuncSetAttribute((const void*)kern, hipFuncAttributeMaxDynamicSharedMemorySize, lds);
            done.fetch_or(bit, std::memory_order_relaxed);
        }
    }
    ESCX_LAUNCH(kern, dim3((a.M + 15) / 16), dim3(64 * PVQF_WAVES), lds, s, a);
}
template <int NT, int STEPS>
static void launch_pvq_fused(const PvqFusedArgs& a, hipStream_t s) {
    if (a.dec) launch_pvq_fused_d<NT, STEPS, true>(a, s); else launch_pvq_fused_d<NT, STEPS, false>(a, s);
}

void pvq_tab_add(const long long* codes, long long bstride, const float* tab, const float* gq, int G, int Ksz, int B, int Hq, int Wd, int Cp, int ov,
                 const float* dec, float* out, hipStream_t s) {
    PvqTabAddArgs a{codes, bstride, tab, gq, dec, out, G, Ksz, Wd / ov, Hq, Wd, Cp, ov, (long long)B * Hq * Wd * (Cp / 4)};
    ESCX_LAUNCH(pvq_tab_add_kernel, dim3((unsigned)((a.n4 + 255) / 256)), dim3(256), 0, s, a);
}

int pvq_fused(const float* enc, const float* dec, int B, int Hq, int Wd, int Cp, int ov, const float* wd, int Np, int Kq, int splits, int bk,
              const float* cbn, const float* c2, const float* cbraw, int G, int Ksz, int d, int dt, const float* wup, const float* tab, const float* gq,
              float* out, long long* codes, long long bstride, float* loss, float loss_scale, int l2norm, hipStream_t s) {
    const int Tq = Wd / ov, M = B * Tq;
    int k_per_z = 0;
    if (!pvq_geometry(Np, dt, G, Kq, Cp, splits, bk, &k_per_z) || Ksz < 1) return -1;
    PvqFusedArgs a{enc, dec, wd, cbn, c2, cbraw, wup, tab, gq, out, codes, bstride, loss, loss_scale, M, Tq, Hq, Wd, Cp, ov, Kq, k_per_z, splits, G, Ksz, d, l2norm, nullptr};
#ifdef ESCX_PVQ_TRACE
    {
        static unsigned long long* last = nullptr; static int n = 0;
        unsigned long long* p = debug_trace_buffer();
        if (p != last) { last = p; n = 0; }
        a.trace = p ? p + (size_t)(n++ % 16) * 4096 * 8 : nullptr;
    }
#endif
    const int NT = Np / 16, STEPS = dt / 4;
    if (NT == 6 && STEPS == 8) { launch_pvq_fused<6, 8>(a, s); return 0; }
    if (NT == 3 && STEPS == 4) { launch_pvq_fused<3, 4>(a, s); return 0; }
    if (NT == 3 && STEPS == 3) { launch_pvq_fused<3, 3>(a, s); return 0; }
    if (NT == 2 && STEPS == 2) { launch_pvq_fused<2, 2>(a, s); return 0; }
    if (NT == 1 && STEPS == 1) { launch_pvq_fused<1, 1>(a, s); return 0; }
    return -1;
}

int pvq_up(const long long* codes, long long bstride, const float* cbraw, int G, int Ksz, int dt, int B, int Hq, int Wd, int Cp, int ov,
           const float* W, int Np, int Kp, const float* dec, float* out, hipStream_t s) {
    const int Tq = Wd / ov, M = B * Tq;
    if (Np % 16 || Kp % 16 || Cp % 16 || dt % 4) return -1;
    PvqUpArgs a{codes, bstride, cbraw, W, dec, out, G, Ksz, dt, Tq, M, Hq, Wd, Cp, ov, Kp, Np / 16, 0};
    const int mt = (M + 15) / 16;
    int per = 16;
    while (per < a.NT && (long long)mt * ((a.NT + per - 1) / per) > 2048) per += 16;
    a.nt_per_wg = per;
    const dim3 grid(mt, (a.NT + per - 1) / per);
    switch (Kp / 16) {
        case 1: ESCX_LAUNCH(pvq_up_kernel<1>, grid, dim3(256), 0, s, a); return 0;
        case 2: ESCX_LAUNCH(pvq_up_kernel<2>, grid, dim3(256), 0, s, a); return 0;
        case 3: ESCX_LAUNCH(pvq_up_kernel<3>, grid, dim3(256), 0, s, a); return 0;
        case 4: ESCX_LAUNCH(pvq_up_kernel<4>, grid, dim3(256), 0, s, a); return 0;
        case 6: ESCX_LAUNCH(pvq_up_kernel<6>, grid, dim3(256), 0, s, a); return 0;
        default: return -1;
    }
}

void istft_ola(const float* frames, const float* win2, float* wave, int B, int T, int ldf, int win, int hop, int left, int half,
               int out_len, hipStream_t s) {
    const long long n = (long long)B * out_len;
    ESCX_LAUNCH(istft_ola_kernel, dim3((unsigned)((n + 255) / 256)), dim3(256), 0, s, frames, win2, wave, B, T, ldf, win, hop,
                       left, half, out_len);
}

void pad_rows(const float* src, float* dst, long long rows, int C, int Cp, hipStream_t s) {
    const long long n = rows * Cp;
    ESCX_LAUNCH(pad_rows_kernel, dim3((unsigned)((n + 255) / 256)), dim3(256), 0, s, src, dst, rows, C, Cp);
}
void unpad_rows(const float* src, float* dst, long long rows, int C, int Cp, hipStream_t s) {
    const long long n = rows * C;
    ESCX_LAUNCH(unpad_rows_kernel, dim3((unsigned)((n + 255) / 256)), dim3(256), 0, s, src, dst, rows, C, Cp);
}
int deembed_border(const float* x, const float* wv, const float* bv, float* out, int B, int H, int W, int C, int Cp, int pf, int pt,
                   int in_dim, int Fp, hipStream_t s) {
    const int per_clip = 2 * W + 2 * (H > 2 ? H - 2 : 0);
    const long long waves = (long long)B * per_clip;
    const unsigned grid = (unsigned)((waves + 3) / 4);
    const int NO = in_dim * pf * pt;
    if (NO == 12) ESCX_LAUNCH((deembed_border_kernel<12>), dim3(grid), dim3(256), 0, s, x, wv, bv, out, B, H, W, C, Cp, pf, pt, in_dim, Fp);
    else if (NO == 8) ESCX_LAUNCH((deembed_border_kernel<8>), dim3(grid), dim3(256), 0, s, x, wv, bv, out, B, H, W, C, Cp, pf, pt, in_dim, Fp);
    else if (NO == 6) ESCX_LAUNCH((deembed_border_kernel<6>), dim3(grid), dim3(256), 0, s, x, wv, bv, out, B, H, W, C, Cp, pf, pt, in_dim, Fp);
    else if (NO == 4) ESCX_LAUNCH((deembed_border_kernel<4>), dim3(grid), dim3(256), 0, s, x, wv, bv, out, B, H, W, C, Cp, pf, pt, in_dim, Fp);
    else return -1;
    return 0;
}

void codes_pack10(const long long* in, unsigned char* out, long long n, hipStream_t s) {
    const long long q = (n + 3) / 4;
    ESCX_LAUNCH(codes_pack10_kernel, dim3((unsigned)((q + 255) / 256)), dim3(256), 0, s, in, out, n);
}
void codes_unpack10(const unsigned char* in, long long* out, long long n, hipStream_t s) {
    const long long q = (n + 3) / 4;
    ESCX_LAUNCH(codes_unpack10_kernel, dim3((unsigned)((q + 255) / 256)), dim3(256), 0, s, in, out, n);
}
void test_math(const float* x, float* y, long long n, int which, hipStream_t s) {
    ESCX_LAUNCH(test_math_kernel, dim3((unsigned)((n + 255) / 256)), dim3(256), 0, s, x, y, n, which);
}
void test_copy_rows(const float* src, float* dst, long long rows, int Cp, hipStream_t s) {
    ESCX_LAUNCH(test_copy_rows_kernel, dim3(4096), dim3(256), 0, s, src, dst, rows, Cp);
}
void rows_permute(const float* src, float* dst, const int* map, int rows, long long row_len, hipStream_t s) {
    const int vec = (row_len % 4 == 0 && (reinterpret_cast<uintptr_t>(src) | reinterpret_cast<uintptr_t>(dst)) % 16 == 0) ? 1 : 0;
    const long long per_row = vec ? row_len / 4 : row_len;
    const unsigned gx = (unsigned)std::max<long long>(1, std::min<long long>((per_row + 255) / 256, 1024));
    ESCX_LAUNCH(rows_permute_kernel, dim3(gx, (unsigned)std::min(rows, 65535)), dim3(256), 0, s, src, dst, map, rows, row_len, vec);
}
void codes_permute(const long long* src, long long src_stride, long long* dst, const int* map, const int* S, int rows, int Smax, int GT, hipStream_t s) {
    const long long n = (long long)rows * Smax * GT;
    ESCX_LAUNCH(codes_permute_kernel, dim3((unsigned)((n + 255) / 256)), dim3(256), 0, s, src, src_stride, dst, map, S, rows, Smax, GT);
}
void loss_reduce_streams(const float* terms, long long lslot, const int* S, int cap, const int* slot_clips, int G, int Tq, int B, float* out, hipStream_t s) {
    SlotRows r{};
    for (int j = 0; j < cap && j < 8; ++j) r.m[j] = slot_clips[j] * Tq;
    ESCX_LAUNCH(loss_reduce_streams_kernel, dim3(B), dim3(64), 0, s, terms, lslot, S, cap, r, G, Tq, out);
}
void codes_pack10_streams(const long long* in, unsigned char* out, const long long* off, int B, long long clip_stride, long long n, hipStream_t s) {
    const long long q = (n + 3) / 4;
    if (q > 0) ESCX_LAUNCH(codes_pack10_streams_kernel, dim3((unsigned)((q + 255) / 256)), dim3(256), 0, s, in, out, off, B, clip_stride);
// ... 73 lines not shown
```

efficient-speech-codec_amd/csrc/launchers.h:

```cpp
#pragma once
#include <hip/hip_runtime.h>

namespace escx {

void gemm_qkv(const float* A, int lda, int M, const float* W, int Np, int Kp, float* out, const float* bias,
              int nq, float scale, hipStream_t s);
void gemm_proj_scatter(const float* A, int lda, int M, const float* W, int Np, int Kp, float* out, const float* shortcut,
                       const float* bias, const int* map, int slots, int tokens, hipStream_t s);
void gemm_gelu(const float* A, int lda, int M, const float* W, int Np, int Kp, float* out, const float* bias, hipStream_t s);
void gemm_residual(const float* A, int lda, int M, const float* W, int Np, int Kp, float* out, const float* bias,
                   const float* res, hipStream_t s);
void gemm_store(const float* A, int lda, int M, const float* W, int Np, int Kp, float* out, int ldo, const float* bias, hipStream_t s);
void gemm_split(const float* A, int lda, int M, const float* W, int Np, int Kp, float* out, int H, int Wd, int C2p, hipStream_t s);

#ifndef ESCX_MLP_OCC4
#define ESCX_MLP_OCC4 96
#endif
#ifndef ESCX_ATTN_TMW2_MAX
#define ESCX_ATTN_TMW2_MAX 48
#endif
constexpr int attn_windows_per_wave(int Cp) { return Cp <= ESCX_ATTN_TMW2_MAX ? 2 : 1; }

constexpr int ESCX_COMB_UNSUPPORTED = -3;
struct MlpSplit { const float* wf; const float* gamma; const float* beta; float* out; int NT, H, W, C2p; };
int mlp_fused(float* x, int M, int C, int Cp, const float* gamma, const float* beta, const float* w1f, const float* b1,
              const float* w2f, const float* b2, const float* wcf, int hiddenP, int variant, int* hs_io, float* partial, hipStream_t s,
              float* out = nullptr,
              const MlpSplit* split = nullptr);
unsigned long long* debug_trace_buffer();
size_t mlp_x3_bytes(int Cp, int hiddenP, int nt = 3);
int mlp_x3_pack(const float* w1, const float* w2, void* image, int Cp, int hiddenP, hipStream_t s, int nt = 3, const float* gamma = nullptr, const float* beta = nullptr,
                const float* b1 = nullptr, int C = 0);
struct MlpSplit;
int mlp_x3(float* x, int M, int C, int Cp, const float* gamma, const float* beta, const float* b1, const float* b2, const void* image, int hiddenP, int nw, int* hs_io, float* partial,
           hipStream_t s, const MlpSplit* split = nullptr, int nt = 3, float* out = nullptr);
size_t mlp_x3_split_bytes(int Cp, int Np);
int mlp_x3_split_pack(const float* wf, void* image, int Cp, int Np, hipStream_t s, int nt = 3, const float* gamma = nullptr, const float* beta = nullptr, int C = 0);
void rows_combine(float* dst, const float* src, const float* partial, const float* bias, long long M, int Cp, int n, hipStream_t s);

int rowgemm_fused(int segs, const float* x, float* out, const float* gamma, const float* beta, const float* wf, const int* map, int M,
                  int rows_per_clip, int src_rows_per_clip, int C, int Cp, int Np, int split, int H, int W, int C2p, hipStream_t s,
                  const void* x3_wf = nullptr, int x3_nt = 3);
size_t rowgemm_x3_bytes(int KP, int Np);
int rowgemm_x3_pack(const float* wf, void* image, int KP, int Np, hipStream_t s, int nt = 3, const float* gamma = nullptr, const float* beta = nullptr, int C = 0);
void loss_reduce(const float* terms, int n_slots, int G, int M, int Tq, float* out, hipStream_t s);
void mlp_set_trace(unsigned long long* p);
int test_fastdiv(int n, int d);
int deembed7_fused(const float* tok, int B, int H, int W, int Cp, const float* wfrag, const float* bias, float* out, int pf, int pt,
                   int in_dim, int Fp, hipStream_t s, const void* x2_image = nullptr);
size_t deembed7_x2_image_bytes(int Cp);
int deembed7_x2_pack(const float* wfrag, void* image, int Cp, hipStream_t s);
int attn_fused(const float* src, float* dst, int Cp, int C, int mode, int n_groups, const float* gamma, const float* beta,
               const float* wf, const float* bqkv, const float* bias_tab, const float* bproj, const int* map, int slots, int tokens,
               int n_windows, int nWh, int nWw, int shifted, float scale, int nw, int* gs_io, float* partial, int rows, hipStream_t s,
               const struct AttnTape* tape = nullptr,
               const void* x3_wf = nullptr, int x3_nt = 3,
               bool len_tables = false);
size_t attn_x3_bytes(int Cp, int mode, int n_groups);
int attn_x3_pack(const float* waf, void* image, int Cp, int mode, int n_groups, hipStream_t s, int nt = 3, const float* gamma = nullptr, const float* beta = nullptr, int C = 0, const float* bqkv = nullptr);
struct AttnTape { float* xn; float* qkv; float* o; int ldq, ldo, hdp, nH; };

void gemm_frames(const float* wave, int B, int L, int T, int hop, int off, const float* W, int Np, int Kp, float* out, hipStream_t s);
void gemm_patch(const float* spec, int B, int T, int in_dim, int Fp, int H, int Wd, int pf, int pt, const float* W, int Np, int Kp,
                float* out, const float* bias, hipStream_t s);
void gemm_conv_deembed1(const float* x, int B, int H, int Wd, int Cp, const float* W, int Np, float* out, const float* bias,
                        int pf, int pt, hipStream_t s);
void gemm_conv_spec(const float* x, int B, int T, int F, int Cp, const float* W, float* out, const float* bias, int Fp, int in_dim,
                    hipStream_t s);
void gemm_deembed_composed(const float* x, int B, int H, int Wd, int Cp, const float* W, float* out, const float* bias, int pf, int pt,
                           int in_dim, int Fp, hipStream_t s);
int deembed_border(const float* x, const float* wv, const float* bv, float* out, int B, int H, int W, int C, int Cp, int pf, int pt,
                   int in_dim, int Fp, hipStream_t s);
void gemm_pvq_down(const float* enc, const float* dec, int B, int Hq, int Wd, int Cp, int ov, const float* W, int Np, int Kp,
                   float* zpart, int splits, hipStream_t s);
int pvq_down_splits(int M, int Kp, int Cp);
void gemm_pvq_up(const long long* codes, long long bstride, const float* cbraw, int G, int Ksz, int dt, int B, int Hq, int Wd, int Cp,
                 int ov, const float* W, int Np, int Kp, const float* dec, float* out, hipStream_t s);

void ln_rows(int mode, const float* src, float* dst, const float* gamma, const float* beta, const int* map, int rows_per_clip,
             int src_rows_per_clip, int total_rows, int C, int Cp, hipStream_t s);
int window_attention(const float* qkv, const float* bias, float* out, int total_windows, int nH, int hdp, int ldq, int ldo, int nWh,
                     int nWw, int shifted, hipStream_t s);
int window_attention_any(const float* qkv, const float* bias, float* out, int total_windows, int ws, int nH, int hd, int hdp, int ldq, int ldo, int nWh, int nWw,
                         int shift, hipStream_t s);
int pvq_fused(const float* enc, const float* dec, int B, int Hq, int Wd, int Cp, int ov, const float* wdf, int Np, int Kq, int splits, int bk,
              const float* cbn, const float* c2, const float* cbraw, int G, int Ksz, int d, int dt, const float* wup, const float* tab, const float* gq,
              float* out, long long* codes, long long bstride, float* loss, float loss_scale, int l2norm, hipStream_t s);
bool prvq_geometry_ok(int Np, int dt, int G, int Kq, int Cp, int splits, int bk);
int prvq_fused(const float* enc, const long long* codes_in, int B, int Hq, int Wd, int Cp, int ov, const float* wdf, int Np, int Kq, int splits, int bk,
               const float* cbn, const float* c2, const float* cbraw, int G, int Ksz, int d, int dt, const float* wup,
               long long* codes, long long bstride, const int* clip_S, int S, int Smax, float* loss, long long lslot, float loss_scale, int l2norm,
               float* out, hipStream_t s);
int prvq_train_fwd(const float* enc, int B, int Hq, int Wd, int Cp, int ov, const float* wdf, int Np, int Kq, int splits, int bk, const float* cbn, const float* c2,
                   const float* cbraw, int G, int Ksz, int d, int dt, const float* wup, long long* codes, long long bstride, int S, int R, int freeze, float* ze,
                   float* zq, float* terms, long long lslot, float loss_scale, int l2norm, float* out, hipStream_t s);
void pvq_tab_add(const long long* codes, long long bstride, const float* tab, const float* gq, int G, int Ksz, int B, int Hq, int Wd, int Cp, int ov,
                 const float* dec, float* out, hipStream_t s);
int pvq_down_bk(int Cp);
int pvq_up(const long long* codes, long long bstride, const float* cbraw, int G, int Ksz, int dt, int B, int Hq, int Wd, int Cp, int ov,
           const float* W, int Np, int Kp, const float* dec, float* out, hipStream_t s);
int pvq_search(const float* zpart, int splits, int M, int ldz, const float* cbn, const float* c2, const float* cbraw, int G, int Ksz,
               int d, int dt, int Tq, long long* codes, long long bstride, float* loss, float loss_scale, int l2norm, hipStream_t s);
void istft_ola(const float* frames, const float* win2, float* wave, int B, int T, int ldf, int win, int hop, int left, int half,
               int out_len, hipStream_t s);
void pad_rows(const float* src, float* dst, long long rows, int C, int Cp, hipStream_t s);
void unpad_rows(const float* src, float* dst, long long rows, int C, int Cp, hipStream_t s);
void codes_pack10(const long long* in, unsigned char* out, long long n, hipStream_t s);
void codes_unpack10(const unsigned char* in, long long* out, long long n, hipStream_t s);
void test_math(const float* x, float* y, long long n, int which, hipStream_t s);
void test_copy_rows(const float* src, float* dst, long long rows, int Cp, hipStream_t s);
void rows_permute(const float* src, float* dst, const int* map, int rows, long long row_len, hipStream_t s);
void codes_permute(const long long* src, long long src_stride, long long* dst, const int* map, const int* S, int rows, int Smax, int GT, hipStream_t s);
void loss_reduce_streams(const float* terms, long long lslot, const int* S, int cap, const int* slot_clips, int G, int Tq, int B, float* out, hipStream_t s);
void codes_pack10_streams(const long long* in, unsigned char* out, const long long* off, int B, long long clip_stride, long long n, hipStream_t s);
void codes_unpack10_streams(const unsigned char* in, long long* out, const long long* off, int B, long long clip_stride, hipStream_t s);
void gemm_frames_len(const float* wave, const int* len, int B, int L, int T, int hop, int off, const float* W, int Np, int Kp, float* out, hipStream_t s);
int window_attention_len(const float* qkv, const float* bias, float* out, int total_windows, int nH, int hdp, int ldq, int ldo, const int* flags, int shifted,
                         hipStream_t s);
void zero_dead_cols(float* x, const int* wlen, int B, int H, int W, int Cp, hipStream_t s);
int deembed_border_len(const float* x, const float* wv, const float* bv, float* out, const int* wlen, int B, int H, int W, int C, int Cp, int pf, int pt,
                       int in_dim, int Fp, hipStream_t s);
void istft_ola_len(const float* frames, const float* win2, float* wave, const int* wlen, int pt, int B, int T, int ldf, int win, int hop, int left, int half,
                   int out_len, hipStream_t s);
void loss_reduce_len(const float* terms, const int* wlen, int ov, int n_slots, int G, int B, int Tq, float* out, hipStream_t s);
void codes_mask_len(const long long* src, long long* dst, const int* wlen, int ov, int B, int rows, int Tq, long long fill, hipStream_t s);
void unpad_rows_len(const float* src, float* dst, const int* len, int per_w, int pt, int hop, int B, int T, int segs, int C, int Cp, hipStream_t s);
void codes_narrow(const long long* in, short* out, long long n, hipStream_t s);
void codes_widen(const short* in, long long* out, long long n, hipStream_t s);

}
```

efficient-speech-codec_amd/esc/_native.py:

```python
import ctypes
import os
from ctypes import POINTER, Structure, byref, c_char_p, c_double, c_float, c_int, c_int16, c_int32, c_int64, c_void_p

_LIB_TAG = os.environ.get("ESCX_LIB_TAG", "")
_LIB_PATH = os.path.join(os.path.dirname(os.path.abspath(__file__)), "lib", "libescx" + ("_" + _LIB_TAG if _LIB_TAG else "") + ".so")
MAX_SCALES = 8


class EscxConfig(Structure):
    _fields_ = [
        ("in_dim", c_int32), ("in_freq", c_int32), ("n_scales", c_int32), ("h_dims", c_int32 * MAX_SCALES),
        ("max_streams", c_int32), ("win_length", c_int32), ("hop_length", c_int32), ("patch_f", c_int32),
        ("patch_t", c_int32), ("swin_heads", c_int32 * MAX_SCALES), ("swin_depth", c_int32), ("window_size", c_int32),
        ("mlp_ratio", c_float), ("overlap", c_int32), ("group_size", c_int32), ("codebook_size", c_int32),
        ("codebook_dims", c_int32 * MAX_SCALES), ("l2norm", c_int32),
    ]


class EscxRvqConfig(Structure):
    _fields_ = [("base", EscxConfig), ("num_rvqs", c_int32), ("codebook_dim", c_int32)]


class EscxDiscConfig(Structure):
    _fields_ = [("sample_rate", c_int32), ("n_rates", c_int32), ("n_periods", c_int32), ("periods", c_int32 * 8), ("n_ffts", c_int32),
                ("fft_sizes", c_int32 * 8), ("n_bands", c_int32), ("bands", (c_float * 2) * 8), ("rates", c_int32 * 8)]


class EscxSpecLossConfig(Structure):
    _fields_ = [("n_scales", c_int32), ("window", c_int32 * 16), ("n_mels", c_int32 * 16), ("filterbank", c_void_p * 16), ("clamp_eps", c_float), ("pow", c_float),
                ("mag_weight", c_float), ("log_weight", c_float)]


class EscxDacConfig(Structure):
    _fields_ = [("encoder_dim", c_int32), ("n_encoder_rates", c_int32), ("encoder_rates", c_int32 * 8), ("latent_dim", c_int32),
                ("decoder_dim", c_int32), ("n_decoder_rates", c_int32), ("decoder_rates", c_int32 * 8), ("n_codebooks", c_int32),
                ("codebook_size", c_int32), ("codebook_dim", c_int32), ("sample_rate", c_int32)]


SIGNATURES = {
    "escx_last_error": (c_char_p, []),
    "escx_version": (c_char_p, []),
    "escx_create": (c_int, [POINTER(EscxConfig), c_int, POINTER(c_void_p)]),
    "escx_create_rvq": (c_int, [POINTER(EscxRvqConfig), c_int, POINTER(c_void_p)]),
    "escx_quantizer_kind": (c_int, [c_void_p]),
    "escx_destroy": (None, [c_void_p]),
    "escx_set_param": (c_int, [c_void_p, c_char_p, c_void_p, POINTER(c_int64), c_int]),
    "escx_finalize_params": (c_int, [c_void_p]),
    "escx_num_required_keys": (c_int, [c_void_p]),
    "escx_required_key": (c_char_p, [c_void_p, c_int]),
    "escx_reserve": (c_int, [c_void_p, c_int, c_int]),
    "escx_workspace_bytes": (c_int64, [c_void_p]),
    "escx_set_precision": (c_int, [c_void_p, c_int]),
    "escx_get_precision": (c_int, [c_void_p]),
    "escx_encode": (c_int, [c_void_p, c_void_p, c_int, c_int, c_int, c_void_p, POINTER(c_int), POINTER(c_int), c_void_p]),
    "escx_decode": (c_int, [c_void_p, c_void_p, c_int, c_int, c_int, c_int, c_void_p, c_void_p, c_void_p]),
    "escx_forward": (c_int, [c_void_p, c_void_p, c_int, c_int, c_int, c_void_p, c_void_p, c_void_p, c_void_p, c_void_p, c_void_p]),
    "escx_forward_feat": (c_int, [c_void_p, c_void_p, c_int, c_int, c_int, c_void_p, c_void_p, c_void_p, c_void_p, c_void_p]),
    "escx_encode_streams": (c_int, [c_void_p, c_void_p, c_int, c_int, POINTER(c_int32), c_void_p, POINTER(c_int), POINTER(c_int), c_void_p]),
    "escx_decode_streams": (c_int, [c_void_p, c_void_p, c_int, c_int, POINTER(c_int32), c_int, c_int, c_void_p, c_void_p, c_void_p]),
    "escx_forward_streams": (c_int, [c_void_p, c_void_p, c_void_p, c_int, c_int, POINTER(c_int32), c_void_p, c_void_p, c_void_p, c_void_p, c_void_p, c_void_p]),
    "escx_encode_lengths": (c_int, [c_void_p, c_void_p, c_int, c_int, POINTER(c_int32), c_int, c_void_p, POINTER(c_int), POINTER(c_int), c_void_p]),
    "escx_decode_lengths": (c_int, [c_void_p, c_void_p, c_int, c_int, POINTER(c_int32), c_int, c_int, c_void_p, c_void_p, c_void_p]),
    "escx_forward_lengths": (c_int, [c_void_p, c_void_p, c_int, c_int, POINTER(c_int32), c_int, c_void_p, c_void_p, c_void_p, c_void_p, c_void_p, c_void_p]),
    "escx_num_frames": (c_int, [c_void_p, c_int]),
    "escx_output_samples": (c_int, [c_void_p, c_int]),
    "escx_spec_transform": (c_int, [c_void_p, c_void_p, c_int, c_int, c_void_p, c_void_p]),
    "escx_audio_reconstruct": (c_int, [c_void_p, c_void_p, c_int, c_int, c_void_p, c_void_p]),
    "escx_patch_embed": (c_int, [c_void_p, c_void_p, c_int, c_int, c_void_p, c_void_p]),
    "escx_transformer_layer": (c_int, [c_void_p, c_int, c_void_p, c_int, c_int, c_int, c_void_p, POINTER(c_int), c_void_p]),
    "escx_pvq_encode": (c_int, [c_void_p, c_int, c_void_p, c_void_p, c_int, c_int, c_void_p, c_int64, c_void_p]),
    "escx_pvq_decode": (c_int, [c_void_p, c_int, c_void_p, c_int64, c_void_p, c_int, c_int, c_void_p, c_void_p]),
    "escx_rvq_encode": (c_int, [c_void_p, c_void_p, c_int, c_int, c_int, c_void_p, c_void_p, c_void_p]),
    "escx_rvq_decode": (c_int, [c_void_p, c_void_p, c_int, c_int, c_int, c_void_p, c_void_p]),
    "escx_patch_deembed": (c_int, [c_void_p, c_void_p, c_int, c_int, c_void_p, c_void_p]),
    "escx_profile_enable": (c_int, [c_void_p, c_int]),
    "escx_profile_report": (c_char_p, [c_void_p]),
    "escx_debug_mlp_trace": (c_int, [c_void_p]),
    "escx_test_math": (c_int, [c_void_p, c_void_p, c_int64, c_int, c_void_p]),
    "escx_test_fastdiv": (c_int, [c_int, c_int]),
    "escx_test_copy_rows": (c_int, [c_void_p, c_void_p, c_int64, c_int, c_void_p]),
    "escx_codes_pack10": (c_int, [c_void_p, c_void_p, c_int64, c_void_p]),
    "escx_codes_unpack10": (c_int, [c_void_p, c_void_p, c_int64, c_void_p]),
    "escx_codes_pack10_streams": (c_int, [c_void_p, c_int, c_int, c_int64, POINTER(c_int32), c_void_p, c_void_p]),
    "escx_codes_unpack10_streams": (c_int, [c_void_p, c_int, c_int, c_int64, POINTER(c_int32), c_void_p, c_void_p]),
    "escx_codes_narrow": (c_int, [c_void_p, c_void_p, c_int64, c_void_p]),
    "escx_codes_widen": (c_int, [c_void_p, c_void_p, c_int64, c_void_p]),
    "escx_flat_param_count": (c_int, [c_void_p]),
    "escx_flat_param_key": (c_char_p, [c_void_p, c_int]),
    "escx_flat_param_offset": (c_int64, [c_void_p, c_int]),
    "escx_flat_param_numel": (c_int64, [c_void_p, c_int]),
    "escx_flat_param_total": (c_int64, [c_void_p]),
    "escx_load_flat_params": (c_int, [c_void_p, c_void_p, c_int, c_void_p]),
    "escx_train_forward": (c_int, [c_void_p, c_void_p, c_void_p, c_int, c_int, c_int, c_int, c_void_p, c_void_p, c_void_p, c_void_p, c_void_p, c_void_p, c_void_p]),
    "escx_train_forward_feat": (c_int, [c_void_p, c_void_p, c_void_p, c_int, c_int, c_int, c_int, c_void_p, c_void_p, c_void_p, c_void_p, c_void_p, c_void_p]),
    "escx_train_backward": (c_int, [c_void_p, c_void_p, c_void_p, c_void_p, c_void_p, c_void_p, c_void_p]),
    "escx_train_backward_ex": (c_int, [c_void_p, c_void_p, c_void_p, c_void_p, c_void_p, c_void_p, c_void_p, c_void_p, c_void_p]),
    "escx_rvq_train_forward": (c_int, [c_void_p, c_void_p, c_void_p, c_void_p, c_int, c_int, c_int, c_int, c_void_p, c_void_p, c_void_p, c_void_p, c_void_p, c_void_p, c_void_p]),
    "escx_rvq_train_backward": (c_int, [c_void_p, c_void_p, c_void_p, c_void_p, c_void_p, c_void_p, c_void_p, c_void_p, c_void_p]),
    "escx_train_tape_bytes": (c_int64, [c_void_p]),
    "escx_train_tape_generation": (c_int64, [c_void_p]),
    "escx_stft_loss": (c_int, [c_void_p, c_void_p, c_int, c_int64, c_void_p, c_void_p, c_void_p]),
    "escx_mel_loss": (c_int, [c_void_p, c_void_p, c_int, c_int, c_int, c_void_p, c_void_p, c_void_p]),
    "escx_stft_loss_ex": (c_int, [c_void_p, c_void_p, c_int, c_int64, c_void_p, c_void_p, c_void_p, c_void_p]),
    "escx_mel_loss_ex": (c_int, [c_void_p, c_void_p, c_int, c_int, c_int, c_void_p, c_void_p, c_void_p, c_void_p]),
    "escx_scale_rows": (c_int, [c_void_p, c_void_p, c_void_p, c_int, c_int64, c_void_p]),
    "escx_grad_norm_clip": (c_int, [c_void_p, c_int64, c_float, c_void_p, c_void_p]),
    "escx_adamw_step": (c_int, [c_void_p, c_void_p, c_void_p, c_void_p, c_int64, c_int, c_double, c_double, c_double, c_double, c_double, c_void_p, c_void_p]),
    "escx_disc_create": (c_int, [POINTER(EscxDiscConfig), c_int, POINTER(c_void_p)]),
    "escx_disc_destroy": (None, [c_void_p]),
    "escx_disc_param_count": (c_int, [c_void_p]),
    "escx_disc_param_key": (c_char_p, [c_void_p, c_int]),
    "escx_disc_param_offset": (c_int64, [c_void_p, c_int]),
    "escx_disc_param_numel": (c_int64, [c_void_p, c_int]),
    "escx_disc_param_total": (c_int64, [c_void_p]),
    "escx_disc_num_fmaps": (c_int, [c_void_p, c_int]),
    "escx_disc_fmap_shape": (c_int, [c_void_p, c_int, c_int] + [POINTER(c_int)] * 7),
    "escx_disc_forward": (c_int, [c_void_p, c_void_p, c_int64, c_void_p, c_int, c_int, POINTER(c_void_p), c_void_p]),
    "escx_disc_backward": (c_int, [c_void_p, c_void_p, c_int64, c_void_p, c_int, c_int, POINTER(c_void_p), POINTER(c_void_p), c_void_p, c_void_p, c_void_p]),
    "escx_gan_term": (c_int, [c_void_p, c_void_p, c_void_p, c_int, c_int, c_int, c_int, c_int, c_int, c_int, c_float, c_void_p, c_int, c_void_p]),
    "escx_gan_term_grad": (c_int, [c_void_p, c_void_p, c_void_p, c_void_p, c_int, c_int, c_int, c_int, c_int, c_int, c_int, c_float, c_void_p]),
    "escx_disc_set_precision": (c_int, [c_void_p, c_int]),
    "escx_disc_get_precision": (c_int, [c_void_p]),
    "escx_disc_profile_enable": (c_int, [c_int]),
    "escx_disc_profile_report": (c_char_p, []),
    "escx_dac_create": (c_int, [POINTER(EscxDacConfig), c_int, POINTER(c_void_p)]),
    "escx_dac_destroy": (None, [c_void_p]),
    "escx_dac_param_count": (c_int, [c_void_p]),
    "escx_dac_param_key": (c_char_p, [c_void_p, c_int]),
    "escx_dac_param_offset": (c_int64, [c_void_p, c_int]),
    "escx_dac_param_numel": (c_int64, [c_void_p, c_int]),
    "escx_dac_param_total": (c_int64, [c_void_p]),
    "escx_dac_num_frames": (c_int, [c_void_p, c_int]),
    "escx_dac_output_samples": (c_int, [c_void_p, c_int]),
    "escx_dac_encode": (c_int, [c_void_p, c_void_p, c_int64, c_void_p, c_int, c_int, c_int, c_void_p, c_void_p, c_void_p, c_void_p, c_void_p]),
    "escx_dac_encode_ex": (c_int, [c_void_p, c_void_p, c_int64, c_void_p, c_int, c_int, c_int, POINTER(c_int32), POINTER(c_int32), c_int, c_void_p, c_void_p, c_void_p,
                                   c_void_p, c_void_p, c_void_p]),
    "escx_dac_from_codes": (c_int, [c_void_p, c_void_p, c_int64, c_void_p, c_int, c_int, c_int, c_void_p, c_void_p, c_void_p]),
    "escx_dac_from_codes_ex": (c_int, [c_void_p, c_void_p, c_int64, c_void_p, c_int, c_int, c_int, POINTER(c_int32), c_void_p, c_void_p, c_void_p]),
    "escx_dac_decode": (c_int, [c_void_p, c_void_p, c_int64, c_void_p, c_int, c_int, c_void_p, c_void_p]),
    "escx_dac_encode_lengths": (c_int, [c_void_p, c_void_p, c_int64, c_void_p, c_int, c_int, POINTER(c_int32), c_int, c_int, POINTER(c_int32), c_void_p, c_void_p,
                                        c_void_p, c_void_p, c_void_p]),
    "escx_dac_from_codes_lengths": (c_int, [c_void_p, c_void_p, c_int64, c_void_p, c_int, c_int, c_int, POINTER(c_int32), POINTER(c_int32), c_void_p, c_void_p,
                                            c_void_p]),
    "escx_dac_decode_lengths": (c_int, [c_void_p, c_void_p, c_int64, c_void_p, c_int, c_int, POINTER(c_int32), POINTER(c_int32), c_void_p, c_void_p]),
    "escx_dac_set_snake_maps": (c_int, [c_void_p, c_int]),
    "escx_dac_get_snake_maps": (c_int, [c_void_p]),
    "escx_dac_set_precision": (c_int, [c_void_p, c_int]),
    "escx_dac_get_precision": (c_int, [c_void_p]),
    "escx_dac_set_grad_precision": (c_int, [c_void_p, c_int]),
    "escx_dac_get_grad_precision": (c_int, [c_void_p]),
    "escx_dac_set_param_grad_precision": (c_int, [c_void_p, c_int]),
    "escx_dac_get_param_grad_precision": (c_int, [c_void_p]),
    "escx_dac_set_padding": (c_int, [c_void_p, c_int]),
    "escx_dac_get_padding": (c_int, [c_void_p]),
# ... 91 lines not shown
```

include/escx.h:

```cpp
#ifndef ESCX_H
#define ESCX_H

#include <stdint.h>

#ifdef __cplusplus
extern "C" {
#endif

#define ESCX_MAX_SCALES 8

typedef enum {
    ESCX_OK = 0,
    ESCX_ERR_INVALID_ARG = -1,
    ESCX_ERR_UNSUPPORTED = -2,
    ESCX_ERR_HIP = -3,
    ESCX_ERR_STATE = -4,
    ESCX_ERR_ASSERT = -5
} escx_status;

typedef struct {
    int32_t in_dim;
    int32_t in_freq;
    int32_t n_scales;
    int32_t h_dims[ESCX_MAX_SCALES];
    int32_t max_streams;
    int32_t win_length;
    int32_t hop_length;
    int32_t patch_f, patch_t;
    int32_t swin_heads[ESCX_MAX_SCALES];
    int32_t swin_depth;
    int32_t window_size;
    float   mlp_ratio;
    int32_t overlap;
    int32_t group_size;
    int32_t codebook_size;
    int32_t codebook_dims[ESCX_MAX_SCALES];
    int32_t l2norm;
} escx_config;

typedef struct escx_handle_s* escx_handle;

typedef struct {
    escx_config base;
    int32_t num_rvqs;
    int32_t codebook_dim;
} escx_rvq_config;

const char* escx_last_error(void);
const char* escx_version(void);
int escx_create(const escx_config* cfg, int device, escx_handle* out);
int escx_create_rvq(const escx_rvq_config* cfg, int device, escx_handle* out);
int escx_quantizer_kind(escx_handle h);
void escx_destroy(escx_handle h);

int escx_set_param(escx_handle h, const char* key, const float* host_data, const int64_t* shape, int ndim);
int escx_finalize_params(escx_handle h);
int escx_num_required_keys(escx_handle h);
const char* escx_required_key(escx_handle h, int i);

int escx_reserve(escx_handle h, int batch, int n_samples);
int64_t escx_workspace_bytes(escx_handle h);

#define ESCX_PRECISION_FP32   0
#define ESCX_PRECISION_F16X2  2
#define ESCX_PRECISION_BF16X3 3
int escx_set_precision(escx_handle h, int mode);
int escx_get_precision(escx_handle h);

int escx_encode(escx_handle h, const float* wave_dev, int batch, int n_samples, int num_streams,
                int64_t* codes_dev, int* feat_h, int* feat_w, void* stream);
int escx_decode(escx_handle h, const int64_t* codes_dev, int batch, int num_streams, int feat_h, int feat_w,
                float* wave_out_dev, float* recon_feat_dev, void* stream);
int escx_forward(escx_handle h, const float* wave_dev, int batch, int n_samples, int num_streams,
                 int64_t* codes_dev, float* wave_out_dev, float* raw_feat_dev, float* recon_feat_dev,
                 float* cm_loss_dev, void* stream);
int escx_forward_feat(escx_handle h, const float* feat_dev, int batch, int n_frames, int num_streams,
                      int64_t* codes_dev, float* wave_out_dev, float* recon_feat_dev, float* cm_loss_dev, void* stream);
int escx_encode_streams(escx_handle h, const float* wave_dev, int batch, int n_samples, const int32_t* streams,
                        int64_t* codes_dev, int* feat_h, int* feat_w, void* stream);
int escx_decode_streams(escx_handle h, const int64_t* codes_dev, int batch, int smax, const int32_t* streams, int feat_h, int feat_w,
                        float* wave_out_dev, float* recon_feat_dev, void* stream);
int escx_forward_streams(escx_handle h, const float* wave_dev, const float* feat_dev, int batch, int n_samples_or_frames, const int32_t* streams,
                         int64_t* codes_dev, float* wave_out_dev, float* raw_feat_dev, float* recon_feat_dev, float* cm_loss_dev, void* stream);
int escx_encode_lengths(escx_handle h, const float* wave_dev, int batch, int row_len, const int32_t* lengths, int num_streams,
                        int64_t* codes_dev, int* feat_h, int* feat_w, void* stream);
int escx_decode_lengths(escx_handle h, const int64_t* codes_dev, int batch, int num_streams, const int32_t* widths, int feat_h, int feat_w,
                        float* wave_out_dev, float* recon_feat_dev, void* stream);
int escx_forward_lengths(escx_handle h, const float* wave_dev, int batch, int row_len, const int32_t* lengths, int num_streams,
                         int64_t* codes_dev, float* wave_out_dev, float* raw_feat_dev, float* recon_feat_dev, float* cm_loss_dev, void* stream);
int escx_num_frames(escx_handle h, int n_samples);
int escx_output_samples(escx_handle h, int feat_w);

int escx_spec_transform(escx_handle h, const float* wave_dev, int batch, int n_samples, float* spec_dev, void* stream);
int escx_audio_reconstruct(escx_handle h, const float* spec_dev, int batch, int n_frames, float* wave_dev, void* stream);
int escx_patch_embed(escx_handle h, const float* spec_dev, int batch, int n_frames, float* tokens_dev, void* stream);
int escx_transformer_layer(escx_handle h, int layer_id, const float* x_dev, int batch, int H, int W,
                           float* y_dev, int* H_out, void* stream);
int escx_pvq_encode(escx_handle h, int stream_id, const float* enc_dev, const float* dec_dev, int batch, int W,
                    int64_t* codes_dev, int64_t code_batch_stride, void* stream);
int escx_pvq_decode(escx_handle h, int stream_id, const int64_t* codes_dev, int64_t code_batch_stride,
                    const float* dec_dev, int batch, int W, float* out_dev, void* stream);
int escx_rvq_encode(escx_handle h, const float* tokens_dev, int batch, int W, int num_streams, int64_t* codes_dev, float* zq_out_dev, void* stream);
int escx_rvq_decode(escx_handle h, const int64_t* codes_dev, int batch, int num_streams, int W, float* tokens_out_dev, void* stream);
int escx_patch_deembed(escx_handle h, const float* tokens_dev, int batch, int W, float* spec_dev, void* stream);

int escx_profile_enable(escx_handle h, int enable);
const char* escx_profile_report(escx_handle h);

int escx_debug_mlp_trace(unsigned long long* dev_buf);
int escx_test_math(const float* x_dev, float* y_dev, int64_t n, int which, void* stream);
int escx_test_copy_rows(const float* src_dev, float* dst_dev, int64_t rows, int row_floats, void* stream);
int escx_test_fastdiv(int n, int d);

int escx_codes_pack10(const int64_t* codes_dev, uint8_t* out_dev, int64_t n, void* stream);
int escx_codes_unpack10(const uint8_t* in_dev, int64_t* codes_dev, int64_t n, void* stream);
int escx_codes_pack10_streams(const int64_t* codes_dev, int batch, int smax, int64_t gt, const int32_t* streams, uint8_t* out_dev, void* stream);
int escx_codes_unpack10_streams(const uint8_t* in_dev, int batch, int smax, int64_t gt, const int32_t* streams, int64_t* codes_dev, void* stream);
int escx_codes_narrow(const int64_t* codes_dev, int16_t* out_dev, int64_t n, void* stream);
int escx_codes_widen(const int16_t* in_dev, int64_t* codes_dev, int64_t n, void* stream);

int escx_flat_param_count(escx_handle h);
const char* escx_flat_param_key(escx_handle h, int i);
int64_t escx_flat_param_offset(escx_handle h, int i);
int64_t escx_flat_param_numel(escx_handle h, int i);
int64_t escx_flat_param_total(escx_handle h);
int escx_load_flat_params(escx_handle h, const float* flat_params_dev, int full, void* stream);
int escx_train_forward(escx_handle h, const float* flat_params_dev, const float* wave_dev, int batch, int n_samples, int num_streams,
                       int freeze_codebook, int64_t* codes_dev, float* wave_out_dev, float* raw_feat_dev, float* recon_feat_dev,
                       float* cm_loss_dev, float* cb_loss_dev, void* stream);
int escx_train_forward_feat(escx_handle h, const float* flat_params_dev, const float* feat_dev, int batch, int n_frames, int num_streams, int freeze_codebook,
                            int64_t* codes_dev, float* wave_out_dev, float* recon_feat_dev, float* cm_loss_dev, float* cb_loss_dev, void* stream);
int escx_train_backward(escx_handle h, const float* d_wave_dev, const float* d_recon_feat_dev, const float* d_cm_loss_dev,
                        const float* d_cb_loss_dev, float* grad_flat_dev, void* stream);
int escx_train_backward_ex(escx_handle h, const float* d_wave_dev, const float* d_recon_feat_dev, const float* d_raw_feat_dev,
                           const float* d_cm_loss_dev, const float* d_cb_loss_dev, float* grad_flat_dev, float* d_input_dev, void* stream);
int escx_rvq_train_forward(escx_handle h, const float* flat_params_dev, const float* wave_dev, const float* feat_dev, int batch, int n_samples_or_frames,
                           int num_streams, int freeze_codebook, int64_t* codes_dev, float* wave_out_dev, float* raw_feat_dev, float* recon_feat_dev,
                           float* cm_loss_dev, float* cb_loss_dev, void* stream);
int escx_rvq_train_backward(escx_handle h, const float* d_wave_dev, const float* d_recon_feat_dev, const float* d_raw_feat_dev,
                            const float* d_cm_loss_dev, const float* d_cb_loss_dev, float* grad_flat_dev, float* d_input_dev, void* stream);
int64_t escx_train_tape_bytes(escx_handle h);
int64_t escx_train_tape_generation(escx_handle h);
int escx_stft_loss(const float* raw_feat_dev, const float* recon_feat_dev, int batch, int64_t per_clip, float* loss_dev,
                   float* d_recon_feat_dev, void* stream);
int escx_stft_loss_ex(const float* raw_feat_dev, const float* recon_feat_dev, int batch, int64_t per_clip, float* loss_dev,
                      float* d_recon_feat_dev, float* d_raw_feat_dev, void* stream);
int escx_mel_loss(const float* raw_wave_dev, const float* recon_wave_dev, int batch, int n_samples, int sample_rate, float* loss_dev,
                  float* d_recon_wave_dev, void* stream);
int escx_mel_loss_ex(const float* raw_wave_dev, const float* recon_wave_dev, int batch, int n_samples, int sample_rate, float* loss_dev,
                     float* d_recon_wave_dev, float* d_raw_wave_dev, void* stream);
int escx_scale_rows(const float* x_dev, const float* g_dev, float* out_dev, int rows, int64_t per_row, void* stream);
int escx_grad_norm_clip(const float* grad_flat_dev, int64_t n, float max_norm, float* norm_out_dev, void* stream);
int escx_adamw_step(float* param_flat_dev, const float* grad_flat_dev, float* exp_avg_dev, float* exp_avg_sq_dev, int64_t n, int step,
                    double lr, double beta1, double beta2, double eps, double weight_decay, const float* clip_dev, void* stream);

typedef struct {
    int32_t sample_rate;
    int32_t n_rates;
    int32_t n_periods; int32_t periods[8];
    int32_t n_ffts; int32_t fft_sizes[8];
    int32_t n_bands; float bands[8][2];
    int32_t rates[8];
} escx_disc_config;
typedef struct escx_disc_s* escx_disc;
int escx_disc_create(const escx_disc_config* cfg, int device, escx_disc* out);
void escx_disc_destroy(escx_disc d);
int escx_disc_param_count(escx_disc d);
const char* escx_disc_param_key(escx_disc d, int i);
int64_t escx_disc_param_offset(escx_disc d, int i);
int64_t escx_disc_param_numel(escx_disc d, int i);
int64_t escx_disc_param_total(escx_disc d);
int escx_disc_num_fmaps(escx_disc d, int n_samples);
int escx_disc_fmap_shape(escx_disc d, int n_samples, int i, int* sub, int* C, int* Cp, int* D0, int* D1, int* P1, int* off1);
int escx_disc_forward(escx_disc d, const float* flat_params_dev, int64_t params_version, const float* wave_dev, int batch, int n_samples,
                      float* const* fmaps_dev, void* stream);
int escx_disc_backward(escx_disc d, const float* flat_params_dev, int64_t params_version, const float* wave_dev, int batch, int n_samples,
                       float* const* fmaps_dev, const float* const* d_fmaps_dev, float* grad_flat_dev, float* d_wave_dev, void* stream);
int escx_disc_set_precision(escx_disc d, int mode);
int escx_disc_get_precision(escx_disc d);
int escx_gan_term(const float* x_dev, const float* ref_dev, float* grad_dev, int batch, int C, int Cp, int D0, int D1, int P1, int mode, float target,
                  float* loss_dev, int accumulate, void* stream);
int escx_gan_term_grad(const float* x_dev, const float* ref_dev, const float* g_dev, float* grad_dev, int batch, int C, int Cp, int D0, int D1, int P1, int mode,
                       float target, void* stream);
int escx_disc_profile_enable(int enable);
// ... 111 lines not shown
```

Measured before the change: 12600.

## Fuse the first two PVQ quantisers into one paired kernel for encode and decode

Adds a paired fused PVQ kernel that quantises stream 0 and stream 1 of the same coarsest scale in a single launch, feeding stream 0's reconstruction directly to stream 1. Decode gets a matching table-lookup kernel that adds both streams' codebook contributions in one pass. All encode, decode and forward paths route their first two quantisers through these paired helpers, falling back to the separate calls when shapes differ or ESCX_PVQ_PAIR is off. The aim is to save a launch and a round trip of the intermediate decoded tensor through global memory. The cost is a larger kernel that may have different register and LDS pressure.

```diff
diff --git a/efficient-speech-codec_amd/csrc/escx_api.cpp b/efficient-speech-codec_amd/csrc/escx_api.cpp
--- a/efficient-speech-codec_amd/csrc/escx_api.cpp
+++ b/efficient-speech-codec_amd/csrc/escx_api.cpp
@@ -417,6 +417,51 @@
     return 0;
 }
 
+static int run_pvq_quantize_pair(escx_handle_s* h, const float* enc, int B0, int B1, int W, long long* codes0, long long* codes1, long long bstride,
+                                 float* loss0, float* loss1, float* dec, float* out1, hipStream_t st) {
+    const escx_config& c = h->cfg;
+    const Quant& q0 = h->quants[0];
+    if (B1 > 0 && h->pvq_pair && h->pvq_fused && B1 == B0 && dec && c.max_streams > 1) {
+        const Quant& q1 = h->quants[1];
+        const int Tq = W / c.overlap, M = B0 * Tq;
+        if (q0.Nz == q1.Nz && q0.dt == q1.dt && q0.d == q1.d && q0.Kq == q1.Kq && q0.Cp == q1.Cp && q0.Hq == q1.Hq && q0.C == q1.C) {
+            const double vec = (double)c.overlap * q0.Hq * q0.C, srch = 2.0 * M * c.group_size * c.codebook_size * q0.d;
+            const PvqPairStream s0{q0.wdf, q0.cbn, q0.c2, q0.cbraw, q0.wup, q0.tab, q0.gq, codes0, loss0, pvq_loss_scale(h, q0, Tq)};
+            const PvqPairStream s1{q1.wdf, q1.cbn, q1.c2, q1.cbraw, q1.wup, q1.tab, q1.gq, codes1, loss1, pvq_loss_scale(h, q1, Tq)};
+            int frc = -1;
+            PROF("pvq_fused_pair", (2.0 * M * vec * q0.d * 2 + srch) + (2.0 * M * vec * q0.d * (out1 ? 2 : 1) + srch),
+                 (double)M * vec * (2 + 2 + (out1 ? 2 : 0)) * 4,
+                 frc = pvq_fused_pair(enc, B0, q0.Hq, W, q0.Cp, c.overlap, q0.Nz, q0.Kq, pvq_down_splits(M, q0.Kq, q0.Cp), pvq_down_bk(q0.Cp), c.group_size,
+                                      c.codebook_size, q0.d, q0.dt, s0, s1, dec, out1, bstride, c.l2norm, st));
+            if (frc == 0) return launch_ok("pvq_quantize_pair");
+            if (h->prof && !h->prof_recs.empty()) h->prof_recs.pop_back();
+        }
+    }
+    int rc;
+    if ((rc = run_pvq_quantize(h, q0, enc, nullptr, B0, W, codes0, bstride, loss0, dec, st))) return rc;
+    if (B1 > 0 && (rc = run_pvq_quantize(h, h->quants[1], enc, dec, B1, W, codes1, bstride, loss1, out1, st))) return rc;
+    return 0;
+}
+
+static int run_pvq_decode_pair(escx_handle_s* h, const long long* codes0, const long long* codes1, long long bstride, int B0, int B1, int W, float* dec,
+                               hipStream_t st) {
+    const escx_config& c = h->cfg;
+    const Quant& q0 = h->quants[0];
+    if (B1 > 0 && B1 == B0 && h->pvq_pair && h->pvq_up_kernel && c.max_streams > 1) {
+        const Quant& q1 = h->quants[1];
+        if (q0.tab && q1.tab && q0.Cp == q1.Cp && q0.Hq == q1.Hq && q0.C == q1.C) {
+            const double vec = (double)c.overlap * q0.Hq * q0.C, Mv = (double)B0 * (W / c.overlap);
+            PROF("pvq_tab_add2", 0, Mv * vec * 3 * 4,
+                 pvq_tab_add2(codes0, codes1, bstride, q0.tab, q0.gq, q1.tab, q1.gq, c.group_size, c.codebook_size, B0, q0.Hq, W, q0.Cp, c.overlap, dec, st));
+            return launch_ok("pvq_decode_pair");
+        }
+    }
+    int rc;
+    if ((rc = run_pvq_decode(h, q0, codes0, bstride, nullptr, B0, W, dec, st))) return rc;
+    if (B1 > 0 && (rc = run_pvq_decode(h, h->quants[1], codes1, bstride, dec, B1, W, dec, st))) return rc;
+    return 0;
+}
+
 static int run_deembed(escx_handle_s* h, const float* tok, int B, int W, float* rspec, hipStream_t st) {
     const escx_config& c = h->cfg;
     const int H0 = c.in_freq / c.patch_f;
@@ -494,12 +539,12 @@
     const long long bstride = (long long)S * G * s.Tq, sstride = (long long)G * s.Tq;
     int rc, H = s.encH[n - 1], Hn;
     float* dec = h->decA; float* other = h->decB;
-    if ((rc = run_pvq_quantize(h, h->quants[0], h->enc_hs[n - 1], nullptr, s.B, s.W, codes, bstride, nullptr, S == 1 ? nullptr : dec, st))) return rc;
-    if (S == 1) return 0;
+    if (S == 1) return run_pvq_quantize(h, h->quants[0], h->enc_hs[n - 1], nullptr, s.B, s.W, codes, bstride, nullptr, nullptr, st);
+    if ((rc = run_pvq_quantize_pair(h, h->enc_hs[n - 1], s.B, s.B, s.W, codes, codes + sstride, bstride, nullptr, nullptr, dec, S == 2 ? nullptr : dec, st))) return rc;
     for (int i = 0; i < S - 1; ++i) {
         const Quant& q = h->quants[i + 1];
         const bool last = (i + 2 == S);
-        if ((rc = run_pvq_quantize(h, q, h->enc_hs[n - 1 - i], dec, s.B, s.W, codes + (i + 1) * sstride, bstride, nullptr, last ? nullptr : dec, st))) return rc;
+        if (i > 0 && (rc = run_pvq_quantize(h, q, h->enc_hs[n - 1 - i], dec, s.B, s.W, codes + (i + 1) * sstride, bstride, nullptr, last ? nullptr : dec, st))) return rc;
         if (last) break;
         if ((rc = run_layer(h, h->layers[n + i], dec, other, s.B, H, s.W, &Hn, st))) return rc;
         std::swap(dec, other); H = Hn;
@@ -534,9 +579,9 @@
     const long long bstride = (long long)S * G * Tq, sstride = (long long)G * Tq;
     int rc, H = Hb, Hn;
     float* dec = h->decA; float* other = h->decB;
-    if ((rc = run_pvq_decode(h, h->quants[0], codes, bstride, nullptr, B, W, dec, st))) return rc;
+    if ((rc = run_pvq_decode_pair(h, codes, codes + sstride, bstride, B, S > 1 && n > 1 ? B : 0, W, dec, st))) return rc;
     for (int i = 0; i + 1 < n; ++i) {
-        if (i < S - 1 && (rc = run_pvq_decode(h, h->quants[i + 1], codes + (i + 1) * sstride, bstride, dec, B, W, dec, st))) return rc;
+        if (i > 0 && i < S - 1 && (rc = run_pvq_decode(h, h->quants[i + 1], codes + (i + 1) * sstride, bstride, dec, B, W, dec, st))) return rc;
         if ((rc = run_layer(h, h->layers[n + i], dec, other, B, H, W, &Hn, st))) return rc;
         std::swap(dec, other); H = Hn;
     }
@@ -595,11 +640,11 @@
         int n_slots = 1;
         int H = sp.encH[n - 1], Hn;
         float* dec = h->decA; float* other = h->decB;
-        if ((r = run_pvq_quantize(h, h->quants[0], h->enc_hs[n - 1], nullptr, nb, sp.W, cd, bstride, loss, dec, st))) return r;
+        if ((r = run_pvq_quantize_pair(h, h->enc_hs[n - 1], nb, S > 1 ? nb : 0, sp.W, cd, cd + sstride, bstride, loss, loss ? loss + lslot : nullptr, dec, dec, st))) return r;
         for (int i = 0; i + 1 < n; ++i) {
             if (i < S - 1) {
                 const Quant& q = h->quants[i + 1];
-                if ((r = run_pvq_quantize(h, q, h->enc_hs[n - 1 - i], dec, nb, sp.W, cd + (i + 1) * sstride, bstride, loss ? loss + (size_t)(i + 1) * lslot : nullptr, dec, st))) return r;
+                if (i > 0 && (r = run_pvq_quantize(h, q, h->enc_hs[n - 1 - i], dec, nb, sp.W, cd + (i + 1) * sstride, bstride, loss ? loss + (size_t)(i + 1) * lslot : nullptr, dec, st))) return r;
                 n_slots = i + 2;
             }
             if ((r = run_layer(h, h->layers[n + i], dec, other, nb, H, sp.W, &Hn, st))) return r;
@@ -705,11 +750,12 @@
     int rc, H = s.encH[n - 1], Hn;
     float* dec = h->decA; float* other = h->decB;
     int nref = clips_over(S, s.B, 1);
-    if ((rc = run_pvq_quantize(h, h->quants[0], h->enc_hs[n - 1], nullptr, s.B, s.W, codes, bstride, nullptr, nref ? dec : nullptr, st))) return rc;
+    if (!nref) return run_pvq_quantize(h, h->quants[0], h->enc_hs[n - 1], nullptr, s.B, s.W, codes, bstride, nullptr, nullptr, st);
+    if ((rc = run_pvq_quantize_pair(h, h->enc_hs[n - 1], s.B, nref, s.W, codes, codes + sstride, bstride, nullptr, nullptr, dec, clips_over(S, nref, 2) ? dec : nullptr, st))) return rc;
     for (int i = 0; nref > 0; ++i) {
         const int nq = nref;
         nref = clips_over(S, nq, i + 2);
-        if ((rc = run_pvq_quantize(h, h->quants[i + 1], h->enc_hs[n - 1 - i], dec, nq, s.W, codes + (i + 1) * sstride, bstride, nullptr, nref ? dec : nullptr, st))) return rc;
+        if (i > 0 && (rc = run_pvq_quantize(h, h->quants[i + 1], h->enc_hs[n - 1 - i], dec, nq, s.W, codes + (i + 1) * sstride, bstride, nullptr, nref ? dec : nullptr, st))) return rc;
         if (!nref) break;
         if ((rc = run_layer(h, h->layers[n + i], dec, other, nref, H, s.W, &Hn, st))) return rc;
         std::swap(dec, other); H = Hn;
@@ -722,10 +768,10 @@
     const long long sstride = (long long)h->cfg.group_size * (W / h->cfg.overlap);
     int rc, H = Hb, Hn;
     float* dec = h->decA; float* other = h->decB;
-    if ((rc = run_pvq_decode(h, h->quants[0], codes, bstride, nullptr, B, W, dec, st))) return rc;
+    if ((rc = run_pvq_decode_pair(h, codes, codes + sstride, bstride, B, n > 1 ? clips_over(S, B, 1) : 0, W, dec, st))) return rc;
     for (int i = 0; i + 1 < n; ++i) {
         const int nq = clips_over(S, B, i + 1);
-        if (nq && (rc = run_pvq_decode(h, h->quants[i + 1], codes + (i + 1) * sstride, bstride, dec, nq, W, dec, st))) return rc;
+        if (i > 0 && nq && (rc = run_pvq_decode(h, h->quants[i + 1], codes + (i + 1) * sstride, bstride, dec, nq, W, dec, st))) return rc;
         if ((rc = run_layer(h, h->layers[n + i], dec, other, B, H, W, &Hn, st))) return rc;
         std::swap(dec, other); H = Hn;
     }
@@ -843,11 +889,11 @@
         int slot_clips[8] = {nb};
         int H = sp.encH[n - 1], Hn;
         float* dec = h->decA; float* other = h->decB;
-        if ((r = run_pvq_quantize(h, h->quants[0], h->enc_hs[n - 1], nullptr, nb, sp.W, cd, cstride, loss, dec, st))) return r;
+        if ((r = run_pvq_quantize_pair(h, h->enc_hs[n - 1], nb, n > 1 ? clips_over(S, nb, 1) : 0, sp.W, cd, cd + sstride, cstride, loss, loss ? loss + lslot : nullptr, dec, dec, st))) return r;
         for (int i = 0; i + 1 < n; ++i) {
             const int nq = clips_over(S, nb, i + 1);
             if (nq) {
-                if ((r = run_pvq_quantize(h, h->quants[i + 1], h->enc_hs[n - 1 - i], dec, nq, sp.W, cd + (i + 1) * sstride, cstride, loss ? loss + (size_t)(i + 1) * lslot : nullptr, dec, st))) return r;
+                if (i > 0 && (r = run_pvq_quantize(h, h->quants[i + 1], h->enc_hs[n - 1 - i], dec, nq, sp.W, cd + (i + 1) * sstride, cstride, loss ? loss + (size_t)(i + 1) * lslot : nullptr, dec, st))) return r;
                 slot_clips[i + 1] = nq;
             }
             if ((r = run_layer(h, h->layers[n + i], dec, other, nb, H, sp.W, &Hn, st))) return r;
@@ -998,10 +1044,10 @@
     int n_slots = 1;
     int H = s.encH[n - 1], Hn;
     float* dec = h->decA; float* other = h->decB;
-    if ((rc = run_pvq_quantize(h, h->quants[0], h->enc_hs[n - 1], nullptr, B, s.W, cd, bstride, loss, dec, st))) return rc;
+    if ((rc = run_pvq_quantize_pair(h, h->enc_hs[n - 1], B, S > 1 ? B : 0, s.W, cd, cd + sstride, bstride, loss, loss ? loss + lslot : nullptr, dec, dec, st))) return rc;
     for (int i = 0; i + 1 < n; ++i) {
         if (i < S - 1) {
-            if ((rc = run_pvq_quantize(h, h->quants[i + 1], h->enc_hs[n - 1 - i], dec, B, s.W, cd + (i + 1) * sstride, bstride, loss ? loss + (size_t)(i + 1) * lslot : nullptr, dec, st))) return rc;
+            if (i > 0 && (rc = run_pvq_quantize(h, h->quants[i + 1], h->enc_hs[n - 1 - i], dec, B, s.W, cd + (i + 1) * sstride, bstride, loss ? loss + (size_t)(i + 1) * lslot : nullptr, dec, st))) return rc;
             n_slots = i + 2;
         }
         if ((rc = run_layer(h, h->layers[n + i], dec, other, B, H, s.W, &Hn, st))) return rc;
@@ -1234,6 +1280,42 @@
     return run_pvq_quantize(h, q, h->stageA, dec ? h->stageB : nullptr, B, W, (long long*)codes, bstride, nullptr, nullptr, st);
 }
 
+extern "C" int escx_pvq_encode_pair(escx_handle h, const float* enc, int B, int W, int64_t* codes, int64_t bstride, float* out, void* stream) {
+    int rc = check_ready(h); if (rc) return rc;
+    if (h->kind != 0) ESCX_FAIL(ESCX_ERR_UNSUPPORTED, "escx_pvq_encode_pair: the cross-scale quantisers do not exist on an rvq handle (escx_rvq_encode / escx_rvq_decode)");
+    if (h->cfg.max_streams < 2) ESCX_FAIL(ESCX_ERR_INVALID_ARG, "escx_pvq_encode_pair needs a model with at least two streams");
+    if (!enc || !codes) ESCX_FAIL(ESCX_ERR_INVALID_ARG, "null pointer");
+    if (W % h->cfg.overlap) ESCX_FAIL(ESCX_ERR_ASSERT, "Time dimension must be multiple of overlap");
+    const Quant& q = h->quants[0];
+    Shapes s; if ((rc = stage_ws_for_w(h, B, W, &s))) return rc;
+    hipStream_t st = (hipStream_t)stream;
+    const long long rows = (long long)B * q.Hq * W;
+    if ((rc = ensure_pvq_tables(h, st))) return rc;
+    pad_rows(enc, h->stageA, rows, q.C, q.Cp, st);
+    long long* cd = (long long*)codes;
+    if ((rc = run_pvq_quantize_pair(h, h->stageA, B, B, W, cd, cd + (long long)h->cfg.group_size * (W / h->cfg.overlap), bstride, nullptr, nullptr,
+                                    h->stageB, out ? h->stageB : nullptr, st))) return rc;
+    if (out) unpad_rows(h->stageB, out, rows, q.C, q.Cp, st);
+    return launch_ok("pvq_encode_pair");
+}
+
+extern "C" int escx_pvq_decode_pair(escx_handle h, const int64_t* codes, int64_t bstride, int B, int W, float* out, void* stream) {
+    int rc = check_ready(h); if (rc) return rc;
+    if (h->kind != 0) ESCX_FAIL(ESCX_ERR_UNSUPPORTED, "escx_pvq_decode_pair: the cross-scale quantisers do not exist on an rvq handle (escx_rvq_encode / escx_rvq_decode)");
+    if (h->cfg.max_streams < 2) ESCX_FAIL(ESCX_ERR_INVALID_ARG, "escx_pvq_decode_pair needs a model with at least two streams");
+    if (!codes || !out) ESCX_FAIL(ESCX_ERR_INVALID_ARG, "null pointer");
+    if (W % h->cfg.overlap) ESCX_FAIL(ESCX_ERR_ASSERT, "Time dimension must be multiple of overlap");
+    const Quant& q = h->quants[0];
+    Shapes s; if ((rc = stage_ws_for_w(h, B, W, &s))) return rc;
+    hipStream_t st = (hipStream_t)stream;
+    const long long rows = (long long)B * q.Hq * W;
+    if ((rc = ensure_pvq_tables(h, st))) return rc;
+    const long long* cd = (const long long*)codes;
+    if ((rc = run_pvq_decode_pair(h, cd, cd + (long long)h->cfg.group_size * (W / h->cfg.overlap), bstride, B, B, W, h->stageA, st))) return rc;
+    unpad_rows(h->stageA, out, rows, q.C, q.Cp, st);
+    return launch_ok("pvq_decode_pair");
+}
+
 extern "C" int escx_pvq_decode(escx_handle h, int sid, const int64_t* codes, int64_t bstride, const float* dec, int B, int W, float* out,
                                void* stream) {
     int rc = check_ready(h); if (rc) return rc;
diff --git a/efficient-speech-codec_amd/csrc/escx_internal.h b/efficient-speech-codec_amd/csrc/escx_internal.h
--- a/efficient-speech-codec_amd/csrc/escx_internal.h
+++ b/efficient-speech-codec_amd/csrc/escx_internal.h
@@ -131,6 +131,7 @@
     int attn_gs_tokens = 600;
     bool mlp_split_fold = true;
     bool pvq_fused = true, pvq_up_kernel = true;
+    bool pvq_pair = true;
     bool prof_serial = false;
     int ws = 4;
 
diff --git a/efficient-speech-codec_amd/csrc/escx_params.cpp b/efficient-speech-codec_amd/csrc/escx_params.cpp
--- a/efficient-speech-codec_amd/csrc/escx_params.cpp
+++ b/efficient-speech-codec_amd/csrc/escx_params.cpp
@@ -157,6 +157,7 @@
     h->mlp_split_fold = !off("ESCX_MLP_SPLIT_FOLD");
     h->pvq_fused = !off("ESCX_PVQ_FUSED");
     h->pvq_up_kernel = !off("ESCX_PVQ_UP_KERNEL");
+    h->pvq_pair = !off("ESCX_PVQ_PAIR");
     h->prof_serial = flag("ESCX_PROF_SERIAL", false);
     if (num("ESCX_X3_TERMS", 2) == 3) h->prec = 3;
     if (const char* e = getenv("ESCX_PRECISION")) {
diff --git a/efficient-speech-codec_amd/csrc/fused_pvq.h b/efficient-speech-codec_amd/csrc/fused_pvq.h
--- a/efficient-speech-codec_amd/csrc/fused_pvq.h
+++ b/efficient-speech-codec_amd/csrc/fused_pvq.h
@@ -112,13 +112,63 @@
     }
 }
 
+constexpr int PVQF_TB = 4;
+__device__ __forceinline__ int pvq_search_per_wave(int Ksz) { return ((Ksz + PVQF_WAVES - 1) / PVQF_WAVES + 15) & ~15; }
+
+template <int STEPS, int TBH>
+__device__ __forceinline__ void pvq_search_fetch(const float* cb, const float* c2, int Ksz, int cb0, int l15, int lg,
+                                                 float (&cf)[TBH][STEPS], float (&c2v)[TBH][4]) {
+    constexpr int DT = 4 * STEPS;
+#pragma unroll
+    for (int u = 0; u < TBH; ++u) {
+        const int c0 = cb0 + 16 * u;
+        const float* p = cb + (size_t)min(c0 + l15, Ksz - 1) * DT + STEPS * lg;
+#pragma unroll
+        for (int r = 0; r < STEPS; ++r) cf[u][r] = p[r];
+#pragma unroll
+        for (int r = 0; r < 4; ++r) c2v[u][r] = c2[min(c0 + 4 * lg + r, Ksz - 1)];
+    }
+}
+
+template <int STEPS, int TBH>
+__device__ __forceinline__ void pvq_search_chain(const float (&cf)[TBH][STEPS], const float (&c2v)[TBH][4], const float (&zf)[STEPS], float av,
+                                                 int cb0, int cend, int lg, float& bd, int& bi, bool& have) {
+#pragma clang fp contract(off)
+#pragma unroll
+    for (int u = 0; u < TBH; ++u) {
+        const int c0 = cb0 + 16 * u;
+        f32x4 dot = zero4();
+#pragma unroll
+        for (int r = 0; r < STEPS; ++r) dot = __builtin_amdgcn_mfma_f32_16x16x4f32(cf[u][r], zf[r], dot, 0, 0, 0);
+#pragma unroll
+        for (int r = 0; r < 4; ++r) {
+            const int code = c0 + 4 * lg + r;
+            const float dist = (av - dot[r]) + c2v[u][r];
+            const bool in = code < cend;
+            const bool take = in & (!have | (!(dist >= bd) & (bd == bd)));
+            bd = take ? dist : bd; bi = take ? code : bi; have = have | in;
+        }
+    }
+}
+
+__device__ __forceinline__ void pvq_search_wave_best(float bd, int bi, int g, int wave, int l15, int lg,
+                                                     float (&bestd)[PVQF_WAVES][PVQF_GMAX][16], int (&besti)[PVQF_WAVES][PVQF_GMAX][16]) {
+#pragma unroll
+    for (int o = 16; o <= 32; o <<= 1) {
+        const float od = __shfl_xor(bd, o);
+        const int oi = __shfl_xor(bi, o);
+        const bool better = arg_better_sel(od, oi, bd, bi);
+        bd = better ? od : bd; bi = better ? oi : bi;
+    }
+    if (lg == 0) { bestd[wave][g][l15] = bd; besti[wave][g][l15] = bi; }
+}
+
 template <int STEPS>
 __device__ __forceinline__ void pvq_search_group(const float* cb, const float* c2, int Ksz, int g, int wave, int l15, int lg,
                                                  const float (&zn2)[PVQF_GMAX][16][4 * STEPS], const float (&asum)[PVQF_GMAX][16],
                                                  float (&bestd)[PVQF_WAVES][PVQF_GMAX][16], int (&besti)[PVQF_WAVES][PVQF_GMAX][16]) {
 #pragma clang fp contract(off)
-    constexpr int TB = 4, DT = 4 * STEPS;
-    const int per_wave = ((Ksz + PVQF_WAVES - 1) / PVQF_WAVES + 15) & ~15;
+    const int per_wave = pvq_search_per_wave(Ksz);
     const int cbeg = wave * per_wave, cend = min(Ksz, cbeg + per_wave);
     float zf[STEPS];
 #pragma unroll
@@ -127,42 +177,89 @@
     float bd = __builtin_inff();
     int bi = 0x7fffffff;
     bool have = false;
-    for (int cb0 = cbeg; cb0 < cend; cb0 += 16 * TB) {
-        float cf[TB][STEPS], c2v[TB][4];
-#pragma unroll
-        for (int u = 0; u < TB; ++u) {
-            const int c0 = cb0 + 16 * u;
-            const float* p = cb + (size_t)min(c0 + l15, Ksz - 1) * DT + STEPS * lg;
-#pragma unroll
-            for (int r = 0; r < STEPS; ++r) cf[u][r] = p[r];
-#pragma unroll
-            for (int r = 0; r < 4; ++r) c2v[u][r] = c2[min(c0 + 4 * lg + r, Ksz - 1)];
-        }
-#pragma unroll
-        for (int u = 0; u < TB; ++u) {
-            const int c0 = cb0 + 16 * u;
-            f32x4 dot = zero4();
-#pragma unroll
-            for (int r = 0; r < STEPS; ++r) dot = __builtin_amdgcn_mfma_f32_16x16x4f32(cf[u][r], zf[r], dot, 0, 0, 0);
-#pragma unroll
-            for (int r = 0; r < 4; ++r) {
-                const int code = c0 + 4 * lg + r;
-                const float dist = (av - dot[r]) + c2v[u][r];
-                const bool in = code < cend;
-                const bool take = in & (!have | (!(dist >= bd) & (bd == bd)));
-                bd = take ? dist : bd; bi = take ? code : bi; have = have | in;
-            }
-        }
-    }
-#pragma unroll
-    for (int o = 16; o <= 32; o <<= 1) {
-        const float od = __shfl_xor(bd, o);
-        const int oi = __shfl_xor(bi, o);
-        const bool better = arg_better_sel(od, oi, bd, bi);
-        bd = better ? od : bd; bi = better ? oi : bi;
-    }
-    if (lg == 0) { bestd[wave][g][l15] = bd; besti[wave][g][l15] = bi; }
-}
+    for (int cb0 = cbeg; cb0 < cend; cb0 += 16 * PVQF_TB) {
+        float cf[PVQF_TB][STEPS], c2v[PVQF_TB][4];
+        pvq_search_fetch<STEPS, PVQF_TB>(cb, c2, Ksz, cb0, l15, lg, cf, c2v);
+        pvq_search_chain<STEPS, PVQF_TB>(cf, c2v, zf, av, cb0, cend, lg, bd, bi, have);
+    }
+    pvq_search_wave_best(bd, bi, g, wave, l15, lg, bestd, besti);
+}
+
+template <int STEPS>
+struct PvqSearchAhead {
+    static constexpr int DT = 4 * STEPS, TBH = STEPS >= 3 ? 2 : PVQF_TB, NU = PVQF_TB / TBH;
+    unsigned cfo[PVQF_TB], c2o[PVQF_TB][4];
+    float cf[TBH][STEPS], c2v[TBH][4];
+    int cbeg, cend;
+
+    __device__ __forceinline__ void init(int Ksz, int wave, int l15, int lg) {
+        const int per_wave = pvq_search_per_wave(Ksz);
+        cbeg = wave * per_wave; cend = min(Ksz, cbeg + per_wave);
+#pragma unroll
+        for (int u = 0; u < PVQF_TB; ++u) {
+            const int c0 = cbeg + 16 * u;
+            cfo[u] = (unsigned)min(c0 + l15, Ksz - 1) * DT + STEPS * lg;
+#pragma unroll
+            for (int r = 0; r < 4; ++r) c2o[u][r] = (unsigned)min(c0 + 4 * lg + r, Ksz - 1);
+        }
+    }
+    template <int HU>
+    __device__ __forceinline__ void fetch_unit(const float* cb, const float* c2, float (&f)[TBH][STEPS], float (&v)[TBH][4]) const {
+#pragma unroll
+        for (int u = 0; u < TBH; ++u) {
+            const float* p = cb + cfo[HU * TBH + u];
+#pragma unroll
+            for (int r = 0; r < STEPS; ++r) f[u][r] = p[r];
+#pragma unroll
+            for (int r = 0; r < 4; ++r) v[u][r] = c2[c2o[HU * TBH + u][r]];
+        }
+    }
+    __device__ __forceinline__ void start(const float* cbn, const float* c2) { fetch_unit<0>(cbn, c2, cf, c2v); }
+
+    __device__ __forceinline__ void run(const float* cbn, const float* c2, int Ksz, int G, int wave, int l15, int lg,
+                                        const float (&zn2)[PVQF_GMAX][16][4 * STEPS], const float (&asum)[PVQF_GMAX][16],
+                                        float (&bestd)[PVQF_WAVES][PVQF_GMAX][16], int (&besti)[PVQF_WAVES][PVQF_GMAX][16]) {
+#pragma clang fp contract(off)
+        for (int g = 0; g < G; ++g) {
+            const float* cb = cbn + (size_t)g * Ksz * DT; const float* cc = c2 + (size_t)g * Ksz;
+            const int gn = min(g + 1, G - 1);
+            const float* cbx = cbn + (size_t)gn * Ksz * DT; const float* ccx = c2 + (size_t)gn * Ksz;
+            float zf[STEPS];
+#pragma unroll
+            for (int r = 0; r < STEPS; ++r) zf[r] = zn2[g][l15][STEPS * lg + r];
+            const float av = asum[g][l15];
+            float bd = __builtin_inff();
+            int bi = 0x7fffffff;
+            bool have = false;
+            int cbeg = this->cbeg, cend = this->cend;
+            asm volatile("" : "+s"(cbeg), "+s"(cend));
+            float nf[TBH][STEPS], nv[TBH][4];
+            if constexpr (NU == 2) {
+                fetch_unit<1>(cb, cc, nf, nv);
+                pvq_search_chain<STEPS, TBH>(cf, c2v, zf, av, cbeg, cend, lg, bd, bi, have);
+                fetch_unit<0>(cbx, ccx, cf, c2v);
+                pvq_search_chain<STEPS, TBH>(nf, nv, zf, av, cbeg + 16 * TBH, cend, lg, bd, bi, have);
+            } else {
+                fetch_unit<0>(cbx, ccx, nf, nv);
+                pvq_search_chain<STEPS, TBH>(cf, c2v, zf, av, cbeg, cend, lg, bd, bi, have);
+#pragma unroll
+                for (int u = 0; u < TBH; ++u) {
+#pragma unroll
+                    for (int r = 0; r < STEPS; ++r) cf[u][r] = nf[u][r];
+#pragma unroll
+                    for (int r = 0; r < 4; ++r) c2v[u][r] = nv[u][r];
+                }
+            }
+#pragma unroll 1
+            for (int cb0 = cbeg + 16 * PVQF_TB; cb0 < cend; cb0 += 16) {
+                float lf[1][STEPS], lv[1][4];
+                pvq_search_fetch<STEPS, 1>(cb, cc, Ksz, cb0, l15, lg, lf, lv);
+                pvq_search_chain<STEPS, 1>(lf, lv, zf, av, cb0, cend, lg, bd, bi, have);
+            }
+            pvq_search_wave_best(bd, bi, g, wave, l15, lg, bestd, besti);
+        }
+    }
+};
 
 __device__ __forceinline__ int pvq_combine_waves(const float (&bestd)[PVQF_WAVES][PVQF_GMAX][16], const int (&besti)[PVQF_WAVES][PVQF_GMAX][16], int g, int vi) {
 #pragma clang fp contract(off)
@@ -211,18 +308,19 @@
     }
 }
 
+template <int NT, int STEPS> struct PvqfShared {
+    float zs[16][16 * NT + 1];
+    float zn2[PVQF_GMAX][16][4 * STEPS];
+    float asum[PVQF_GMAX][16];
+    float bestd[PVQF_WAVES][PVQF_GMAX][16];
+    int besti[PVQF_WAVES][PVQF_GMAX][16];
+    int code_s[PVQF_GMAX][16];
+};
+
 template <int NT, int STEPS, bool DEC>
-__global__ __launch_bounds__(64 * PVQF_WAVES) void pvq_fused_kernel(PvqFusedArgs a) {
-#pragma clang fp contract(off)
-    ESCX_SET_PRIO_SMALL();
-    constexpr int NP = 16 * NT, DT = 4 * STEPS, KC = NT;
-    extern __shared__ __attribute__((aligned(16))) float pvqf_part[];
-    __shared__ float zs[16][NP + 1];
-    __shared__ float zn2[PVQF_GMAX][16][DT];
-    __shared__ float asum[PVQF_GMAX][16];
-    __shared__ float bestd[PVQF_WAVES][PVQF_GMAX][16];
-    __shared__ int besti[PVQF_WAVES][PVQF_GMAX][16];
-    __shared__ int code_s[PVQF_GMAX][16];
+__device__ __forceinline__ void pvq_fused_stage(const PvqFusedArgs& a, float* part, PvqfShared<NT, STEPS>& sh) {
+#pragma clang fp contract(off)
+    constexpr int DT = 4 * STEPS, KC = NT;
     const int tid = threadIdx.x;
     const int lane = tid & 63, l15 = lane & 15, lg = lane >> 4;
     const int wave = __builtin_amdgcn_readfirstlane(tid >> 6);
@@ -238,22 +336,24 @@
 #endif
     PVQ_TS(0)
 
-    pvq_down_slice<NT, DEC>(a.enc, a.dec, a.wd, vecbase, live, lane, wave, a.Kq, a.k_per_z, a.splits, a.Hq, a.Wd, a.Cp, pvqf_part);
+    pvq_down_slice<NT, DEC>(a.enc, a.dec, a.wd, vecbase, live, lane, wave, a.Kq, a.k_per_z, a.splits, a.Hq, a.Wd, a.Cp, part);
     __syncthreads();
     PVQ_TS(1)
-    pvq_sum_slices<NT>(pvqf_part, a.splits, tid, zs);
-    __syncthreads();
-    pvq_normalise<NT, STEPS>(zs, tid, a.G, a.d, a.l2norm, zn2, asum);
+    PvqSearchAhead<STEPS> srch;
+    srch.init(a.Ksz, wave, l15, lg);
+    srch.start(a.cbn, a.c2);
+    pvq_sum_slices<NT>(part, a.splits, tid, sh.zs);
+    __syncthreads();
+    pvq_normalise<NT, STEPS>(sh.zs, tid, a.G, a.d, a.l2norm, sh.zn2, sh.asum);
     __syncthreads();
     PVQ_TS(2)
-    for (int g = 0; g < a.G; ++g)
-        pvq_search_group<STEPS>(a.cbn + (size_t)g * a.Ksz * DT, a.c2 + (size_t)g * a.Ksz, a.Ksz, g, wave, l15, lg, zn2, asum, bestd, besti);
+    srch.run(a.cbn, a.c2, a.Ksz, a.G, wave, l15, lg, sh.zn2, sh.asum, sh.bestd, sh.besti);
     __syncthreads();
     PVQ_TS(3)
     if (tid < 16 * a.G) {
         const int g = tid >> 4, vi = tid & 15;
-        const int i0 = pvq_combine_waves(bestd, besti, g, vi);
-        code_s[g][vi] = i0;
+        const int i0 = pvq_combine_waves(sh.bestd, sh.besti, g, vi);
+        sh.code_s[g][vi] = i0;
         const int mm = m0 + vi;
         if (mm < a.M) {
             const int bb = mm / a.Tq, tt = mm - bb * a.Tq;
@@ -261,7 +361,7 @@
             if (a.loss) {
                 const float* q = a.cbraw + ((size_t)g * a.Ksz + i0) * DT;
                 float e = 0.f;
-                for (int j = 0; j < a.d; ++j) { const float df = q[j] - zs[vi][g * DT + j]; e = __builtin_fmaf(df, df, e); }
+                for (int j = 0; j < a.d; ++j) { const float df = q[j] - sh.zs[vi][g * DT + j]; e = __builtin_fmaf(df, df, e); }
                 a.loss[(size_t)g * a.M + mm] = e * a.loss_scale;
             }
         }
@@ -276,7 +376,7 @@
         const int tabw = a.ov * a.Ksz;
         int cs[PVQF_GMAX];
 #pragma unroll
-        for (int g = 0; g < PVQF_GMAX; ++g) cs[g] = code_s[g < a.G ? g : 0][l15];
+        for (int g = 0; g < PVQF_GMAX; ++g) cs[g] = sh.code_s[g < a.G ? g : 0][l15];
         for (int nt0 = wave * UNR; nt0 < NTo; nt0 += PVQF_WAVES * UNR) {
             f32x4 tv[UNR], dv[UNR];
             size_t idx[UNR];
@@ -307,11 +407,30 @@
     for (int c = 0; c < KC; ++c) {
         const int k = 16 * c + 4 * lg, g = k / DT;
         zf[c] = zero4();
-        if (live && g < a.G) zf[c] = ld4(a.cbraw + ((size_t)g * a.Ksz + (size_t)code_s[g][l15]) * DT + (k - g * DT));
+        if (live && g < a.G) zf[c] = ld4(a.cbraw + ((size_t)g * a.Ksz + (size_t)sh.code_s[g][l15]) * DT + (k - g * DT));
     }
     pvq_up_mfma<NT, DEC>(zf, a.wup, a.dec, a.out, vecbase, live, wave, l15, lg, a.Kq, a.Hq, a.Wd, a.Cp);
     PVQ_TS(5)
 #undef PVQ_TS
+}
+
+template <int NT, int STEPS, bool DEC>
+__global__ __launch_bounds__(64 * PVQF_WAVES) void pvq_fused_kernel(PvqFusedArgs a) {
+    ESCX_SET_PRIO_SMALL();
+    extern __shared__ __attribute__((aligned(16))) float pvqf_part[];
+    __shared__ PvqfShared<NT, STEPS> sh;
+    pvq_fused_stage<NT, STEPS, DEC>(a, pvqf_part, sh);
+}
+
+struct PvqPairArgs { PvqFusedArgs s0, s1; };
+template <int NT, int STEPS>
+__global__ __launch_bounds__(64 * PVQF_WAVES) void pvq_fused_pair_kernel(PvqPairArgs a) {
+    ESCX_SET_PRIO_SMALL();
+    extern __shared__ __attribute__((aligned(16))) float pvqf_part[];
+    __shared__ PvqfShared<NT, STEPS> sh;
+    pvq_fused_stage<NT, STEPS, false>(a.s0, pvqf_part, sh);
+    __syncthreads();
+    pvq_fused_stage<NT, STEPS, true>(a.s1, pvqf_part, sh);
 }
 
 struct PvqTabAddArgs {
@@ -337,4 +456,34 @@
     st4(a.out + i * 4, v);
 }
 
-}
+struct PvqTabAdd2Args {
+    const long long* codes0; const long long* codes1; long long bstride;
+    const float* tab0; const float* gq0; const float* tab1; const float* gq1; float* out;
+    int G, Ksz, Tq, Hq, Wd, Cp, ov; long long n4;
+};
+__global__ __launch_bounds__(256) void pvq_tab_add2_kernel(PvqTabAdd2Args a) {
+    ESCX_SET_PRIO_SMALL();
+    const long long i = (long long)blockIdx.x * 256 + threadIdx.x;
+    if (i >= a.n4) return;
+    const int c4 = a.Cp >> 2;
+    const long long row = i / c4; const int c = (int)(i - row * c4) * 4;
+    const int w = (int)(row % a.Wd); const long long bh = row / a.Wd; const int h = (int)(bh % a.Hq); const int b = (int)(bh / a.Hq);
+    const int t = w / a.ov, o = w - t * a.ov;
+    const int gi = (((o * a.Hq + h) * a.Cp) + c) >> 2;
+    const int g0 = (int)a.gq0[gi], g1 = (int)a.gq1[gi];
+    f32x4 v0 = zero4(), v = zero4();
+    if (g0 >= 0) {
+        long long code = a.codes0[(size_t)b * a.bstride + (size_t)g0 * a.Tq + t];
+        code = code < 0 ? 0 : (code >= a.Ksz ? a.Ksz - 1 : code);
+        v0 = ld4(a.tab0 + ((size_t)h * a.ov * a.Ksz + (size_t)a.ov * code + o) * a.Cp + c);
+    }
+    if (g1 >= 0) {
+        long long code = a.codes1[(size_t)b * a.bstride + (size_t)g1 * a.Tq + t];
+        code = code < 0 ? 0 : (code >= a.Ksz ? a.Ksz - 1 : code);
+        v = ld4(a.tab1 + ((size_t)h * a.ov * a.Ksz + (size_t)a.ov * code + o) * a.Cp + c);
+    }
+    v += v0;
+    st4(a.out + i * 4, v);
+}
+
+}
diff --git a/efficient-speech-codec_amd/csrc/kernels_misc.hip b/efficient-speech-codec_amd/csrc/kernels_misc.hip
--- a/efficient-speech-codec_amd/csrc/kernels_misc.hip
+++ b/efficient-speech-codec_amd/csrc/kernels_misc.hip
@@ -107,6 +107,15 @@
     ESCX_LAUNCH(pvq_tab_add_kernel, dim3((unsigned)((a.n4 + 255) / 256)), dim3(256), 0, s, a);
 }
 
+#ifdef ESCX_PVQ_TRACE
+static unsigned long long* pvq_trace_slot() {
+    static unsigned long long* last = nullptr; static int n = 0;
+    unsigned long long* p = debug_trace_buffer();
+    if (p != last) { last = p; n = 0; }
+    return p ? p + (size_t)(n++ % 16) * 4096 * 8 : nullptr;
+}
+#endif
+
 int pvq_fused(const float* enc, const float* dec, int B, int Hq, int Wd, int Cp, int ov, const float* wd, int Np, int Kq, int splits, int bk,
               const float* cbn, const float* c2, const float* cbraw, int G, int Ksz, int d, int dt, const float* wup, const float* tab, const float* gq,
               float* out, long long* codes, long long bstride, float* loss, float loss_scale, int l2norm, hipStream_t s) {
@@ -115,12 +124,7 @@
     if (!pvq_geometry(Np, dt, G, Kq, Cp, splits, bk, &k_per_z) || Ksz < 1) return -1;
     PvqFusedArgs a{enc, dec, wd, cbn, c2, cbraw, wup, tab, gq, out, codes, bstride, loss, loss_scale, M, Tq, Hq, Wd, Cp, ov, Kq, k_per_z, splits, G, Ksz, d, l2norm, nullptr};
 #ifdef ESCX_PVQ_TRACE
-    {
-        static unsigned long long* last = nullptr; static int n = 0;
-        unsigned long long* p = debug_trace_buffer();
-        if (p != last) { last = p; n = 0; }
-        a.trace = p ? p + (size_t)(n++ % 16) * 4096 * 8 : nullptr;
-    }
+    a.trace = pvq_trace_slot();
 #endif
     const int NT = Np / 16, STEPS = dt / 4;
     if (NT == 6 && STEPS == 8) { launch_pvq_fused<6, 8>(a, s); return 0; }
@@ -129,6 +133,50 @@
     if (NT == 2 && STEPS == 2) { launch_pvq_fused<2, 2>(a, s); return 0; }
     if (NT == 1 && STEPS == 1) { launch_pvq_fused<1, 1>(a, s); return 0; }
     return -1;
+}
+
+template <int NT, int STEPS>
+static void launch_pvq_fused_pair(const PvqPairArgs& a, hipStream_t s) {
+    auto kern = pvq_fused_pair_kernel<NT, STEPS>;
+    constexpr int lds = pvqf_lds_floats<NT>() * (int)sizeof(float);
+    if constexpr (lds > 48 * 1024) {
+        static std::atomic<unsigned> done{0};
+        int dev = 0; (void)hipGetDevice(&dev);
+        const unsigned bit = 1u << (dev & 31);
+        if (!(done.load(std::memory_order_relaxed) & bit)) {
+            (void)hipFuncSetAttribute((const void*)kern, hipFuncAttributeMaxDynamicSharedMemorySize, lds);
+            done.fetch_or(bit, std::memory_order_relaxed);
+        }
+    }
+    ESCX_LAUNCH(kern, dim3((a.s0.M + 15) / 16), dim3(64 * PVQF_WAVES), lds, s, a);
+}
+
+int pvq_fused_pair(const float* enc, int B, int Hq, int Wd, int Cp, int ov, int Np, int Kq, int splits, int bk, int G, int Ksz, int d, int dt,
+                   const PvqPairStream& s0, const PvqPairStream& s1, float* out0, float* out1, long long bstride, int l2norm, hipStream_t s) {
+    const int Tq = Wd / ov, M = B * Tq;
+    int k_per_z = 0;
+    if (!pvq_geometry(Np, dt, G, Kq, Cp, splits, bk, &k_per_z) || Ksz < 1 || !out0 || (out1 && out1 != out0)) return -1;
+    PvqPairArgs a;
+    a.s0 = PvqFusedArgs{enc, nullptr, s0.wdf, s0.cbn, s0.c2, s0.cbraw, s0.wup, s0.tab, s0.gq, out0, s0.codes, bstride, s0.loss, s0.loss_scale,
+                        M, Tq, Hq, Wd, Cp, ov, Kq, k_per_z, splits, G, Ksz, d, l2norm, nullptr};
+    a.s1 = PvqFusedArgs{enc, out0, s1.wdf, s1.cbn, s1.c2, s1.cbraw, s1.wup, s1.tab, s1.gq, out1, s1.codes, bstride, s1.loss, s1.loss_scale,
+                        M, Tq, Hq, Wd, Cp, ov, Kq, k_per_z, splits, G, Ksz, d, l2norm, nullptr};
+#ifdef ESCX_PVQ_TRACE
+    a.s0.trace = pvq_trace_slot(); a.s1.trace = pvq_trace_slot();
+#endif
+    const int NT = Np / 16, STEPS = dt / 4;
+    if (NT == 6 && STEPS == 8) { launch_pvq_fused_pair<6, 8>(a, s); return 0; }
+    if (NT == 3 && STEPS == 4) { launch_pvq_fused_pair<3, 4>(a, s); return 0; }
+    if (NT == 3 && STEPS == 3) { launch_pvq_fused_pair<3, 3>(a, s); return 0; }
+    if (NT == 2 && STEPS == 2) { launch_pvq_fused_pair<2, 2>(a, s); return 0; }
+    if (NT == 1 && STEPS == 1) { launch_pvq_fused_pair<1, 1>(a, s); return 0; }
+    return -1;
+}
+
+void pvq_tab_add2(const long long* codes0, const long long* codes1, long long bstride, const float* tab0, const float* gq0, const float* tab1, const float* gq1,
+                  int G, int Ksz, int B, int Hq, int Wd, int Cp, int ov, float* out, hipStream_t s) {
+    PvqTabAdd2Args a{codes0, codes1, bstride, tab0, gq0, tab1, gq1, out, G, Ksz, Wd / ov, Hq, Wd, Cp, ov, (long long)B * Hq * Wd * (Cp / 4)};
+    ESCX_LAUNCH(pvq_tab_add2_kernel, dim3((unsigned)((a.n4 + 255) / 256)), dim3(256), 0, s, a);
 }
 
 int pvq_up(const long long* codes, long long bstride, const float* cbraw, int G, int Ksz, int dt, int B, int Hq, int Wd, int Cp, int ov,
diff --git a/efficient-speech-codec_amd/csrc/launchers.h b/efficient-speech-codec_amd/csrc/launchers.h
--- a/efficient-speech-codec_amd/csrc/launchers.h
+++ b/efficient-speech-codec_amd/csrc/launchers.h
@@ -86,6 +86,10 @@
 int pvq_fused(const float* enc, const float* dec, int B, int Hq, int Wd, int Cp, int ov, const float* wdf, int Np, int Kq, int splits, int bk,
               const float* cbn, const float* c2, const float* cbraw, int G, int Ksz, int d, int dt, const float* wup, const float* tab, const float* gq,
               float* out, long long* codes, long long bstride, float* loss, float loss_scale, int l2norm, hipStream_t s);
+struct PvqPairStream { const float* wdf; const float* cbn; const float* c2; const float* cbraw; const float* wup; const float* tab; const float* gq;
+                       long long* codes; float* loss; float loss_scale; };
+int pvq_fused_pair(const float* enc, int B, int Hq, int Wd, int Cp, int ov, int Np, int Kq, int splits, int bk, int G, int Ksz, int d, int dt,
+                   const PvqPairStream& s0, const PvqPairStream& s1, float* out0, float* out1, long long bstride, int l2norm, hipStream_t s);
 bool prvq_geometry_ok(int Np, int dt, int G, int Kq, int Cp, int splits, int bk);
 int prvq_fused(const float* enc, const long long* codes_in, int B, int Hq, int Wd, int Cp, int ov, const float* wdf, int Np, int Kq, int splits, int bk,
                const float* cbn, const float* c2, const float* cbraw, int G, int Ksz, int d, int dt, const float* wup,
@@ -96,6 +100,8 @@
                    float* zq, float* terms, long long lslot, float loss_scale, int l2norm, float* out, hipStream_t s);
 void pvq_tab_add(const long long* codes, long long bstride, const float* tab, const float* gq, int G, int Ksz, int B, int Hq, int Wd, int Cp, int ov,
                  const float* dec, float* out, hipStream_t s);
+void pvq_tab_add2(const long long* codes0, const long long* codes1, long long bstride, const float* tab0, const float* gq0, const float* tab1, const float* gq1,
+                  int G, int Ksz, int B, int Hq, int Wd, int Cp, int ov, float* out, hipStream_t s);
 int pvq_down_bk(int Cp);
 int pvq_up(const long long* codes, long long bstride, const float* cbraw, int G, int Ksz, int dt, int B, int Hq, int Wd, int Cp, int ov,
            const float* W, int Np, int Kp, const float* dec, float* out, hipStream_t s);
diff --git a/efficient-speech-codec_amd/esc/_native.py b/efficient-speech-codec_amd/esc/_native.py
--- a/efficient-speech-codec_amd/esc/_native.py
+++ b/efficient-speech-codec_amd/esc/_native.py
@@ -70,6 +70,8 @@
     "escx_transformer_layer": (c_int, [c_void_p, c_int, c_void_p, c_int, c_int, c_int, c_void_p, POINTER(c_int), c_void_p]),
     "escx_pvq_encode": (c_int, [c_void_p, c_int, c_void_p, c_void_p, c_int, c_int, c_void_p, c_int64, c_void_p]),
     "escx_pvq_decode": (c_int, [c_void_p, c_int, c_void_p, c_int64, c_void_p, c_int, c_int, c_void_p, c_void_p]),
+    "escx_pvq_encode_pair": (c_int, [c_void_p, c_void_p, c_int, c_int, c_void_p, c_int64, c_void_p, c_void_p]),
+    "escx_pvq_decode_pair": (c_int, [c_void_p, c_void_p, c_int64, c_int, c_int, c_void_p, c_void_p]),
     "escx_rvq_encode": (c_int, [c_void_p, c_void_p, c_int, c_int, c_int, c_void_p, c_void_p, c_void_p]),
     "escx_rvq_decode": (c_int, [c_void_p, c_void_p, c_int, c_int, c_int, c_void_p, c_void_p]),
     "escx_patch_deembed": (c_int, [c_void_p, c_void_p, c_int, c_int, c_void_p, c_void_p]),
diff --git a/include/escx.h b/include/escx.h
--- a/include/escx.h
+++ b/include/escx.h
@@ -100,6 +100,9 @@
                     int64_t* codes_dev, int64_t code_batch_stride, void* stream);
 int escx_pvq_decode(escx_handle h, int stream_id, const int64_t* codes_dev, int64_t code_batch_stride,
                     const float* dec_dev, int batch, int W, float* out_dev, void* stream);
+int escx_pvq_encode_pair(escx_handle h, const float* enc_dev, int batch, int W, int64_t* codes_dev, int64_t code_batch_stride,
+                         float* out_dev, void* stream);
+int escx_pvq_decode_pair(escx_handle h, const int64_t* codes_dev, int64_t code_batch_stride, int batch, int W, float* out_dev, void* stream);
 int escx_rvq_encode(escx_handle h, const float* tokens_dev, int batch, int W, int num_streams, int64_t* codes_dev, float* zq_out_dev, void* stream);
 int escx_rvq_decode(escx_handle h, const int64_t* codes_dev, int batch, int num_streams, int W, float* tokens_out_dev, void* stream);
 int escx_patch_deembed(escx_handle h, const float* tokens_dev, int batch, int W, float* spec_dev, void* stream);
```

Result: no change. 12660 (median of 4 runs) (+0.4%).
